# williamleif/GraphSAGE

Hardware: NVIDIA B200
Metric: seed_nodes_per_sec (higher is better)
Workload: dtype f32

## Files before the change

### graphsage_b200/_lib.py

```python
import ctypes
import os

import torch

_HERE = os.path.dirname(os.path.abspath(__file__))
LIB_PATH = os.path.join(_HERE, "csrc", "libgraphsage_b200.so")

ABI_VERSION = 2
GS_F32, GS_BF16 = 0, 1
ACT_NONE, ACT_RELU = 0, 1
COMBINE_ADD, COMBINE_CONCAT = 0, 1
MATH_FP32_SIMT, MATH_TF32X3, MATH_TF32, MATH_BF16 = 0, 1, 2, 3
MAX_SEGMENTS = 4

c_i32, c_i64, c_u64, c_vp = ctypes.c_int32, ctypes.c_int64, ctypes.c_uint64, ctypes.c_void_p


class Segment(ctypes.Structure):
    _fields_ = [("self_ids", c_vp), ("neigh_ids", c_vp), ("self_row0", c_i64), ("neigh_row0", c_i64),
                ("n", c_i64), ("k", c_i32), ("_pad", c_i32), ("out_row0", c_i64)]


MAX_SHARDS = 16


class ShardedTable(ctypes.Structure):
    _fields_ = [("base", c_vp * MAX_SHARDS), ("row_start", c_i64 * (MAX_SHARDS + 1)), ("n_shards", c_i32),
                ("my_shard", c_i32), ("n_global_rows", c_i64), ("zero_row", c_i64), ("remap", c_vp)]


class GemmPart(ctypes.Structure):
    _fields_ = [("A", c_vp), ("lda", c_i64), ("K", c_i32), ("B", c_vp), ("ldb", c_i64), ("N", c_i32)]


_SIGNATURES = {
    "gs_version": (c_i32, []),
    "gs_last_error_string": (ctypes.c_char_p, []),
    "gs_set_tuning": (c_i32, [ctypes.c_char_p, c_i32]),
    "gs_sample_padded": (c_i32, [c_vp, c_i64, c_i32, c_vp, c_i64, c_i32, c_vp, c_u64, c_u64, c_vp, c_vp, c_vp]),
    "gs_sample_padded_khop": (c_i32, [c_vp, c_i64, c_i32, c_vp, c_i64, ctypes.POINTER(c_i32), c_i32, c_u64, c_u64, c_vp,
                                      ctypes.POINTER(c_vp), c_vp]),
    "gs_build_padded_adj": (c_i32, [c_vp, c_vp, c_i64, c_i32, c_vp, c_u64, c_u64, c_vp, c_vp, c_vp]),
    "gs_sample_unigram": (c_i32, [c_vp, c_i64, c_i32, c_u64, c_u64, c_vp, c_vp, c_vp]),
    "gs_sample_csr": (c_i32, [c_vp, c_vp, c_i64, c_vp, c_i64, c_i32, c_i32, c_u64, c_u64, c_vp, c_i32, c_vp, c_vp]),
    "gs_perm_prefix_host": (c_i32, [c_u64, c_u64, c_i32, c_i32, ctypes.POINTER(c_i32)]),
    "gs_gather_rows": (c_i32, [c_vp, c_i32, c_i64, c_i32, c_i64, c_vp, c_i64, c_vp, c_i64, c_vp]),
    "gs_gather_mean": (c_i32, [c_vp, c_i32, c_i64, c_i32, c_i64, ctypes.POINTER(Segment), c_i32, c_i32, c_vp, c_vp,
                               c_i64, c_vp]),
    "gs_gather_mean_sharded": (c_i32, [ctypes.POINTER(ShardedTable), c_i32, c_i32, c_i64, ctypes.POINTER(Segment), c_i32,
                                       c_i32, c_i32, c_vp, c_vp, c_vp, c_i64, c_vp]),
    "gs_halo_begin": (c_i32, [c_vp, c_i64, c_vp, c_vp]),
    "gs_halo_claim": (c_i32, [ctypes.POINTER(ShardedTable), c_vp, c_i64, c_vp, c_vp, c_vp, c_i64, c_vp]),
    "gs_halo_fetch": (c_i32, [ctypes.POINTER(ShardedTable), c_i32, c_i64, c_vp, c_vp, c_i64, c_vp, c_i64, c_vp]),
    "gs_halo_translate": (c_i32, [ctypes.POINTER(ShardedTable), c_vp, c_i64, c_vp, c_vp, c_vp]),
    "gs_translate_ids": (c_i32, [ctypes.POINTER(ShardedTable), c_vp, c_i64, c_vp, c_vp]),
    "gs_gather_rows_sharded": (c_i32, [ctypes.POINTER(ShardedTable), c_i32, c_i32, c_i64, c_vp, c_i64, c_vp, c_i64, c_vp]),
    "gs_shard_alloc": (c_i32, [c_i64, ctypes.POINTER(c_vp)]),
    "gs_shard_free": (c_i32, [c_vp]),
    "gs_ipc_export": (c_i32, [c_vp, ctypes.c_char_p]),
    "gs_ipc_import": (c_i32, [ctypes.c_char_p, ctypes.POINTER(c_vp)]),
    "gs_ipc_close": (c_i32, [c_vp]),
    "gs_gather_rows_f32": (c_i32, [c_vp, c_i32, c_i64, c_i32, c_i64, c_vp, c_i64, c_i64, c_vp, c_i64, c_vp]),
    "gs_cast_rows_bf16": (c_i32, [c_vp, c_i64, c_i32, c_i64, c_vp, c_i64, c_vp]),
    "gs_rmat_degrees": (c_i32, [c_i32, c_i64, ctypes.c_double, ctypes.c_double, ctypes.c_double, ctypes.c_double,
                                ctypes.c_double, c_u64, c_u64, c_u64, c_u64, c_vp, c_vp]),
    "gs_rmat_fill": (c_i32, [c_i32, c_i64, ctypes.c_double, ctypes.c_double, ctypes.c_double, ctypes.c_double, c_u64, c_u64,
                             c_u64, c_u64, c_vp, c_vp, c_vp, c_i64, c_i64, c_vp]),
    "gs_segment_max": (c_i32, [c_vp, c_i64, c_i32, c_i32, c_i64, c_vp, c_i64, c_vp]),
    "gs_sage_gemm_workspace_bytes": (c_i64, [c_i64, ctypes.POINTER(GemmPart), c_i32, c_i32]),
    "gs_sage_gemm": (c_i32, [c_i64, ctypes.POINTER(GemmPart), c_i32, c_i32, c_vp, c_i32, c_i32, c_vp, c_i64, c_vp,
                             c_vp]),
    "gs_sage_gemm_pack": (c_i32, [ctypes.POINTER(GemmPart), c_i32, c_i32, c_vp, c_vp]),
    "gs_sage_gemm_prepacked": (c_i32, [c_i64, ctypes.POINTER(GemmPart), c_i32, c_i32, c_vp, c_i32, c_i32, c_vp, c_i64,
                                       c_vp, c_vp]),
    "gs_gather_mean_img_bytes": (c_i64, [c_i64, c_i32, c_i32]),
    "gs_gather_mean_img": (c_i32, [c_vp, c_i64, ctypes.POINTER(ShardedTable), c_i32, c_vp, c_i32, c_i64, ctypes.POINTER(Segment),
                                   c_i32, c_i32, c_i32, c_vp, c_vp]),
    "gs_sage_gemm_img": (c_i32, [c_i64, ctypes.POINTER(GemmPart), c_i32, c_i32, c_vp, c_i32, c_vp, c_i64, c_vp, c_vp, c_i32,
                                 c_vp]),
    "gs_sage_layer_small": (c_i32, [c_vp, c_i64, c_i32, c_i64, ctypes.POINTER(Segment), c_i32, ctypes.POINTER(GemmPart),
                                    c_i32, c_i32, c_vp, c_i32, c_i32, c_vp, c_i64, c_vp, c_u64, c_vp]),
    "gs_maxpool_mlp_workspace_bytes": (c_i64, [c_i32, c_i32]),
    "gs_maxpool_mlp_pack": (c_i32, [c_vp, c_i64, c_i32, c_i32, c_vp, c_vp]),
    "gs_maxpool_mlp_fused": (c_i32, [c_vp, c_i64, c_i32, c_i64, c_vp, c_i64, c_i64, c_i32, c_vp, c_vp, c_i32, c_vp, c_i64,
                                     c_vp]),
    "gs_meanpool_mlp_fused": (c_i32, [c_vp, c_i64, c_i32, c_i64, c_vp, c_i64, c_i64, c_i32, c_vp, c_vp, c_i32, c_vp, c_i64,
                                      c_vp]),
    "gs_pipeline_step": (c_i32, [c_vp, c_vp, c_i64, ctypes.POINTER(c_vp), c_i32, c_vp, c_vp, c_i64, c_vp, c_vp, c_vp, c_vp,
                                 c_vp, c_vp]),
    "gs_row_used": (c_i32, [c_vp, c_i32, c_i64, c_i32, c_i64, c_vp, c_vp]),
    "gs_lstm_seq": (c_i32, [c_vp, c_i64, c_vp, c_i32, c_vp, c_vp, c_i64, c_i64, c_i32, c_vp, c_i64, c_vp, c_vp, c_vp, c_vp]),
    "gs_l2_normalize_rows": (c_i32, [c_vp, c_i64, c_i32, c_i64, c_vp]),
    "gs_bump_counter": (c_i32, [c_vp, c_u64, c_vp]),
}

_lib = None


def lib():
    global _lib
    if _lib is None:
        if not os.path.exists(LIB_PATH):
            raise ImportError(
                "graphsage_b200: %s is missing - build it with `python -m graphsage_b200.build` "
                "(there is no CPU fallback)" % LIB_PATH)
        _lib = ctypes.CDLL(LIB_PATH)
        for name, (res, args) in _SIGNATURES.items():
            fn = getattr(_lib, name)
            fn.restype, fn.argtypes = res, args
        if _lib.gs_version() != ABI_VERSION:
            raise ImportError("graphsage_b200: %s has ABI version %d, this binding needs %d - rebuild it"
                              % (LIB_PATH, _lib.gs_version(), ABI_VERSION))
        for kv in os.environ.get("GS_TUNING", "").split(","):
            if "=" in kv:
                k, v = kv.split("=", 1)
                _lib.gs_set_tuning(k.strip().encode(), int(v))
    return _lib


def exported_symbols():
    return sorted(_SIGNATURES)


def check(rc):
    if rc != 0:
        msg = lib().gs_last_error_string().decode("utf-8", "replace")
        raise RuntimeError("libgraphsage_b200 error %d: %s" % (rc, msg))


def stream_ptr():
    return torch.cuda.current_stream().cuda_stream


def ptr(t):
    return 0 if t is None else t.data_ptr()


def require_cuda(*tensors):
    for t in tensors:
        if t is not None and not t.is_cuda:
            raise RuntimeError("graphsage_b200: tensor on %s - the hot path is CUDA-only (no CPU fallback)" % t.device)


def set_tuning(key, value):
    return lib().gs_set_tuning(key.encode(), int(value))


def perm_prefix_host(seed, counter, max_deg, k):
    buf = (c_i32 * max(k, 1))()
    check(lib().gs_perm_prefix_host(seed & (2**64 - 1), counter & (2**64 - 1), max_deg, k, buf))
    return list(buf[:k])
```

### graphsage_b200/csrc/api.cu

```cuda
#include <stdarg.h>

#include <map>
#include <set>
#include <utility>
#include <mutex>
#include <string>

#include "common.cuh"

namespace gs {

static thread_local char g_err[512] = "";

void set_error(const char* fmt, ...) {
  va_list ap;
  va_start(ap, fmt);
  vsnprintf(g_err, sizeof(g_err), fmt, ap);
  va_end(ap);
}

int32_t cuda_fail(cudaError_t e, const char* what) {
  set_error("CUDA error %d (%s) at %s", (int)e, cudaGetErrorString(e), what);
  return GS_ERR_CUDA;
}

static std::mutex g_mu;
static std::map<std::string, int32_t>& knobs() {
  static std::map<std::string, int32_t> m;
  return m;
}

int32_t tuning(const char* key, int32_t dflt) {
  std::lock_guard<std::mutex> l(g_mu);
  auto it = knobs().find(key);
  return it == knobs().end() ? dflt : it->second;
}

int sm_count() {
  static int n[64] = {0};
  int dev = 0;
  if (cudaGetDevice(&dev) != cudaSuccess || dev < 0 || dev >= 64) return 148;
  if (n[dev] == 0) {
    int v = 0;
    if (cudaDeviceGetAttribute(&v, cudaDevAttrMultiProcessorCount, dev) != cudaSuccess || v <= 0) v = 148;
    n[dev] = v;
  }
  return n[dev];
}

int32_t ensure_dyn_smem(const void* kernel, int bytes) {
  static std::mutex mu;
  static std::set<std::pair<int, const void*>> done;
  int dev = 0;
  GS_CUDA(cudaGetDevice(&dev));
  std::lock_guard<std::mutex> l(mu);
  if (done.count(std::make_pair(dev, kernel))) return GS_OK;
  GS_CUDA(cudaFuncSetAttribute(kernel, cudaFuncAttributeMaxDynamicSharedMemorySize, bytes));
  done.insert(std::make_pair(dev, kernel));
  return GS_OK;
}

}

extern "C" {

int32_t gs_version(void) { return GS_ABI_VERSION; }

const char* gs_last_error_string(void) { return gs::g_err; }

int32_t gs_set_tuning(const char* key, int32_t value) {
  if (!key) return 0;
  std::lock_guard<std::mutex> l(gs::g_mu);
  int32_t prev = 0;
  auto it = gs::knobs().find(key);
  if (it != gs::knobs().end()) prev = it->second;
  gs::knobs()[key] = value;
  return prev;
}

int32_t gs_perm_prefix_host(uint64_t seed, uint64_t counter, int32_t max_deg, int32_t k, int32_t* out_host) {
  GS_REQUIRE(out_host != nullptr || k == 0, "gs_perm_prefix_host: out_host is NULL");
  GS_REQUIRE(max_deg > 0 && k >= 0 && k <= max_deg, "gs_perm_prefix_host: need 0 <= k <= max_deg (k=%d, max_deg=%d)", k,
             max_deg);
  std::string buf((size_t)max_deg * sizeof(int32_t), '\0');
  int32_t* p = (int32_t*)&buf[0];
  for (int i = 0; i < max_deg; ++i) p[i] = i;
  for (int i = 0; i < k; ++i) {
    uint32_t r = gs::philox_draw(seed, counter, 0u, gs::kStreamPadded, i);
    int j = i + (int)gs::mulhi32(r, (uint32_t)(max_deg - i));
    int32_t t = p[i];
    p[i] = p[j];
    p[j] = t;
  }
  for (int i = 0; i < k; ++i) out_host[i] = p[i];
  return GS_OK;
}

int32_t gs_pipeline_step(const void* ids_host, void* ids_dev, int64_t ids_bytes, void* const* graph_execs_host,
                         int32_t n_graphs, const void* out_dev, void* out_host, int64_t out_bytes, void* h2d_stream,
                         void* compute_stream, void* copy_stream, void* ev_ids, void* ev_done, void* ev_drained) {
  GS_REQUIRE(ids_host && ids_dev && graph_execs_host && out_dev && out_host && ev_ids && ev_done && ev_drained &&
                 n_graphs >= 1,
             "gs_pipeline_step: NULL argument");
  cudaStream_t hs = (cudaStream_t)h2d_stream, cs = (cudaStream_t)compute_stream, ps = (cudaStream_t)copy_stream;
  GS_CUDA(cudaStreamWaitEvent(hs, (cudaEvent_t)ev_done, 0));
  GS_CUDA(cudaMemcpyAsync(ids_dev, ids_host, (size_t)ids_bytes, cudaMemcpyHostToDevice, hs));
  GS_CUDA(cudaEventRecord((cudaEvent_t)ev_ids, hs));
  GS_CUDA(cudaStreamWaitEvent(cs, (cudaEvent_t)ev_ids, 0));
  GS_CUDA(cudaStreamWaitEvent(cs, (cudaEvent_t)ev_drained, 0));
  for (int i = 0; i < n_graphs; ++i) GS_CUDA(cudaGraphLaunch((cudaGraphExec_t)graph_execs_host[i], cs));
  GS_CUDA(cudaEventRecord((cudaEvent_t)ev_done, cs));
  GS_CUDA(cudaStreamWaitEvent(ps, (cudaEvent_t)ev_done, 0));
  GS_CUDA(cudaMemcpyAsync(out_host, out_dev, (size_t)out_bytes, cudaMemcpyDeviceToHost, ps));
  GS_CUDA(cudaEventRecord((cudaEvent_t)ev_drained, ps));
  return GS_OK;
}

}
```

### graphsage_b200/csrc/common.cuh

```cuda
#pragma once
#include <cuda_runtime.h>
#include <stdint.h>
#include <stdio.h>
#include <string.h>

#include "../../include/graphsage_b200.h"

namespace gs {

void set_error(const char* fmt, ...);
int32_t cuda_fail(cudaError_t e, const char* what);
int32_t tuning(const char* key, int32_t dflt);
int32_t ensure_dyn_smem(const void* kernel, int bytes);

#define GS_REQUIRE(cond, ...)            \
  do {                                   \
    if (!(cond)) {                       \
      gs::set_error(__VA_ARGS__);        \
      return GS_ERR_INVALID_ARG;         \
    }                                    \
  } while (0)

#define GS_CUDA(expr)                                        \
  do {                                                       \
    cudaError_t _e = (expr);                                 \
    if (_e != cudaSuccess) return gs::cuda_fail(_e, #expr);  \
  } while (0)

inline int32_t launch_check(const char* what) {
  cudaError_t e = cudaGetLastError();
  if (e != cudaSuccess) return cuda_fail(e, what);
  return GS_OK;
}

int sm_count();

struct u32x4 { uint32_t x, y, z, w; };

__host__ __device__ inline uint32_t mulhi32(uint32_t a, uint32_t b) {
  return (uint32_t)(((uint64_t)a * (uint64_t)b) >> 32);
}

__host__ __device__ inline u32x4 philox4x32_10(u32x4 c, uint32_t k0, uint32_t k1) {
#pragma unroll
  for (int r = 0; r < 10; ++r) {
    uint64_t p0 = (uint64_t)0xD2511F53u * c.x;
    uint64_t p1 = (uint64_t)0xCD9E8D57u * c.z;
    u32x4 n;
    n.x = (uint32_t)(p1 >> 32) ^ c.y ^ k0;
    n.y = (uint32_t)p1;
    n.z = (uint32_t)(p0 >> 32) ^ c.w ^ k1;
    n.w = (uint32_t)p0;
    c = n;
    k0 += 0x9E3779B9u;
    k1 += 0xBB67AE85u;
  }
  return c;
}

__host__ __device__ inline uint32_t pick(const u32x4& v, int i) {
  return i == 0 ? v.x : i == 1 ? v.y : i == 2 ? v.z : v.w;
}

__host__ __device__ inline uint32_t philox_draw(uint64_t seed, uint64_t counter, uint32_t c2, uint32_t tag, int i) {
  u32x4 c{(uint32_t)counter, (uint32_t)(counter >> 32), c2, tag + (uint32_t)(i >> 2)};
  u32x4 r = philox4x32_10(c, (uint32_t)seed, (uint32_t)(seed >> 32));
  return pick(r, i & 3);
}

constexpr uint32_t kStreamPadded = 0u;
constexpr uint32_t kStreamCsr = 0x40000000u;
constexpr uint32_t kStreamUnigram = 0x20000000u;
constexpr uint32_t kStreamBuild = 0x10000000u;

#ifdef __CUDACC__
__device__ __forceinline__ uint32_t smem_u32(const void* p) { return (uint32_t)__cvta_generic_to_shared(p); }

__device__ __forceinline__ void mbar_init(uint64_t* bar, uint32_t count) {
  asm volatile("mbarrier.init.shared::cta.b64 [%0], %1;" ::"r"(smem_u32(bar)), "r"(count));
}
__device__ __forceinline__ void fence_mbar_init() { asm volatile("fence.mbarrier_init.release.cluster;" ::: "memory"); }
__device__ __forceinline__ void fence_proxy_async() { asm volatile("fence.proxy.async.shared::cta;" ::: "memory"); }

__device__ __forceinline__ void mbar_expect_tx(uint64_t* bar, uint32_t bytes) {
  asm volatile("mbarrier.arrive.expect_tx.shared::cta.b64 _, [%0], %1;" ::"r"(smem_u32(bar)), "r"(bytes) : "memory");
}
__device__ __forceinline__ void mbar_arrive(uint64_t* bar) {
  asm volatile("mbarrier.arrive.shared::cta.b64 _, [%0];" ::"r"(smem_u32(bar)) : "memory");
}
__device__ __forceinline__ bool mbar_try_wait(uint64_t* bar, uint32_t parity) {
  uint32_t ok;
  asm volatile(
      "{\n\t.reg .pred p;\n\t"
      "mbarrier.try_wait.parity.shared::cta.b64 p, [%1], %2;\n\t"
      "selp.b32 %0, 1, 0, p;\n\t}"
      : "=r"(ok)
      : "r"(smem_u32(bar)), "r"(parity)
      : "memory");
  return ok != 0;
}
__device__ __forceinline__ void mbar_wait(uint64_t* bar, uint32_t parity) {
  while (!mbar_try_wait(bar, parity)) {
  }
}

__device__ __forceinline__ void bulk_g2s(void* smem_dst, const void* gsrc, uint32_t bytes, uint64_t* bar) {
  asm volatile("cp.async.bulk.shared::cluster.global.mbarrier::complete_tx::bytes [%0], [%1], %2, [%3];" ::"r"(
                   smem_u32(smem_dst)),
               "l"(gsrc), "r"(bytes), "r"(smem_u32(bar))
               : "memory");
}
__device__ __forceinline__ void bulk_s2g(void* gdst, const void* smem_src, uint32_t bytes) {
  asm volatile("cp.async.bulk.global.shared::cta.bulk_group [%0], [%1], %2;" ::"l"(gdst), "r"(smem_u32(smem_src)),
               "r"(bytes)
               : "memory");
}
__device__ __forceinline__ void bulk_commit() { asm volatile("cp.async.bulk.commit_group;" ::: "memory"); }
template <int N>
__device__ __forceinline__ void bulk_wait_read() {
  asm volatile("cp.async.bulk.wait_group.read %0;" ::"n"(N) : "memory");
}
template <int N>
__device__ __forceinline__ void bulk_wait() {
  asm volatile("cp.async.bulk.wait_group %0;" ::"n"(N) : "memory");
}

__device__ __forceinline__ float4 ldg_nc_f4(const float4* p) {
  float4 r;
  asm volatile("ld.global.nc.L1::no_allocate.v4.f32 {%0,%1,%2,%3}, [%4];"
               : "=f"(r.x), "=f"(r.y), "=f"(r.z), "=f"(r.w)
               : "l"(p));
  return r;
}
#endif

}
```

### graphsage_b200/csrc/gather.cu

```cuda
#include "common.cuh"

namespace gs {

struct SegTable {
  gs_segment s[GS_MAX_SEGMENTS];
  int32_t n_segments;
  int64_t total_rows;
};

__device__ __forceinline__ int find_segment(const SegTable& t, int64_t r, int64_t& local) {
  int si = 0;
  int64_t base = 0;
#pragma unroll
  for (int q = 0; q < GS_MAX_SEGMENTS - 1; ++q) {
    if (q < t.n_segments - 1 && r >= base + t.s[q].n) {
      base += t.s[q].n;
      si = q + 1;
    }
  }
  local = r - base;
  return si;
}

__device__ __forceinline__ int64_t clamp_row(int64_t id, int64_t n_rows) {
  return (id < 0 || id >= n_rows) ? n_rows - 1 : id;
}

__device__ __forceinline__ float4 mask_tail(float4 v, int col0, int F) {
  if (col0 + 1 >= F) v.y = 0.f;
  if (col0 + 2 >= F) v.z = 0.f;
  if (col0 + 3 >= F) v.w = 0.f;
  return v;
}

template <int kUnroll>
__global__ void __launch_bounds__(256) gather_mean_ldg_kernel(const float* __restrict__ src, int64_t n_src_rows, int F,
                                                              int64_t pitch, const __grid_constant__ SegTable tab, int include_self,
                                                              float* __restrict__ out_self,
                                                              float* __restrict__ out_mean, int64_t out_pitch) {
  const int ncol4 = (int)(out_pitch >> 2);
  for (int64_t r = blockIdx.x; r < tab.total_rows; r += gridDim.x) {
    int64_t i;
    const gs_segment& sg = tab.s[find_segment(tab, r, i)];
    const int k = sg.k;
    const int64_t orow = sg.out_row0 + i;
    const int64_t srow = clamp_row(sg.self_ids ? (int64_t)sg.self_ids[i] : sg.self_row0 + i, n_src_rows);
    for (int c = threadIdx.x; c < ncol4; c += blockDim.x) {
      const int col0 = c * 4;
      float4 acc = make_float4(0.f, 0.f, 0.f, 0.f);
      float4 sv = acc;
      if (col0 < F) {
        int j = 0;
        for (; j + kUnroll <= k; j += kUnroll) {
          float4 v[kUnroll];
#pragma unroll
          for (int u = 0; u < kUnroll; ++u) {
            int64_t nr = clamp_row(sg.neigh_ids ? (int64_t)sg.neigh_ids[i * k + j + u] : sg.neigh_row0 + i * k + j + u,
                                   n_src_rows);
            v[u] = ldg_nc_f4(reinterpret_cast<const float4*>(src + nr * pitch) + c);
          }
#pragma unroll
          for (int u = 0; u < kUnroll; ++u) {
            acc.x += v[u].x; acc.y += v[u].y; acc.z += v[u].z; acc.w += v[u].w;
          }
        }
        for (; j < k; ++j) {
          int64_t nr = clamp_row(sg.neigh_ids ? (int64_t)sg.neigh_ids[i * k + j] : sg.neigh_row0 + i * k + j, n_src_rows);
          float4 v = ldg_nc_f4(reinterpret_cast<const float4*>(src + nr * pitch) + c);
          acc.x += v.x; acc.y += v.y; acc.z += v.z; acc.w += v.w;
        }
        if (include_self || out_self) sv = ldg_nc_f4(reinterpret_cast<const float4*>(src + srow * pitch) + c);
        float div = (float)(k + (include_self ? 1 : 0));
        if (include_self) { acc.x += sv.x; acc.y += sv.y; acc.z += sv.z; acc.w += sv.w; }
        acc.x /= div; acc.y /= div; acc.z /= div; acc.w /= div;
        acc = mask_tail(acc, col0, F);
        sv = mask_tail(sv, col0, F);
      }
      reinterpret_cast<float4*>(out_mean + orow * out_pitch)[c] = acc;
      if (out_self) reinterpret_cast<float4*>(out_self + orow * out_pitch)[c] = sv;
    }
  }
}

__global__ void __launch_bounds__(256) gather_mean_scalar_kernel(const float* __restrict__ src, int64_t n_src_rows, int F,
                                                                 int64_t pitch, const __grid_constant__ SegTable tab, int include_self,
                                                                 float* __restrict__ out_self,
                                                                 float* __restrict__ out_mean, int64_t out_pitch) {
  for (int64_t r = blockIdx.x; r < tab.total_rows; r += gridDim.x) {
    int64_t i;
    const gs_segment& sg = tab.s[find_segment(tab, r, i)];
    const int k = sg.k;
    const int64_t orow = sg.out_row0 + i;
    const int64_t srow = clamp_row(sg.self_ids ? (int64_t)sg.self_ids[i] : sg.self_row0 + i, n_src_rows);
    for (int c = threadIdx.x; c < (int)out_pitch; c += blockDim.x) {
      float acc = 0.f, sv = 0.f;
      if (c < F) {
        for (int j = 0; j < k; ++j) {
          int64_t nr = clamp_row(sg.neigh_ids ? (int64_t)sg.neigh_ids[i * k + j] : sg.neigh_row0 + i * k + j, n_src_rows);
          acc += src[nr * pitch + c];
        }
        sv = src[srow * pitch + c];
        if (include_self) acc += sv;
        acc /= (float)(k + (include_self ? 1 : 0));
      }
      out_mean[orow * out_pitch + c] = acc;
      if (out_self) out_self[orow * out_pitch + c] = sv;
    }
  }
}

__global__ void __launch_bounds__(192) gather_mean_tma_kernel(const float* __restrict__ src, int64_t n_src_rows, int F,
                                                              int64_t pitch, const __grid_constant__ SegTable tab, int include_self,
                                                              float* __restrict__ out_self,
                                                              float* __restrict__ out_mean, int64_t out_pitch,
                                                              int row_bytes) {
  extern __shared__ __align__(128) unsigned char smem[];
  __shared__ __align__(8) uint64_t bar;
  if (threadIdx.x == 0) {
    mbar_init(&bar, 1);
    fence_mbar_init();
  }
  __syncthreads();
  const int ncol4 = (int)(out_pitch >> 2);
  const int row_f4 = row_bytes >> 4;
  uint32_t phase = 0;
  for (int64_t r = blockIdx.x; r < tab.total_rows; r += gridDim.x) {
    int64_t i;
    const gs_segment& sg = tab.s[find_segment(tab, r, i)];
    const int k = sg.k;
    const int64_t orow = sg.out_row0 + i;
    if (threadIdx.x < 32) {
      if (threadIdx.x == 0) mbar_expect_tx(&bar, (uint32_t)((k + 1) * row_bytes));
      __syncwarp();
      for (int j = threadIdx.x; j <= k; j += 32) {
        int64_t id;
        if (j < k) id = sg.neigh_ids ? (int64_t)sg.neigh_ids[i * k + j] : sg.neigh_row0 + i * k + j;
        else id = sg.self_ids ? (int64_t)sg.self_ids[i] : sg.self_row0 + i;
        id = clamp_row(id, n_src_rows);
        bulk_g2s(smem + (size_t)j * row_bytes, src + id * pitch, (uint32_t)row_bytes, &bar);
      }
    }
    mbar_wait(&bar, phase);
    phase ^= 1u;
    const float4* rows = reinterpret_cast<const float4*>(smem);
    for (int c = threadIdx.x; c < ncol4; c += blockDim.x) {
      const int col0 = c * 4;
      float4 acc = make_float4(0.f, 0.f, 0.f, 0.f);
      float4 sv = acc;
      if (col0 < F) {
#pragma unroll 5
        for (int j = 0; j < k; ++j) {
          float4 v = rows[j * row_f4 + c];
          acc.x += v.x; acc.y += v.y; acc.z += v.z; acc.w += v.w;
        }
        sv = rows[k * row_f4 + c];
        float div = (float)(k + (include_self ? 1 : 0));
        if (include_self) { acc.x += sv.x; acc.y += sv.y; acc.z += sv.z; acc.w += sv.w; }
        acc.x /= div; acc.y /= div; acc.z /= div; acc.w /= div;
        acc = mask_tail(acc, col0, F);
        sv = mask_tail(sv, col0, F);
      }
      reinterpret_cast<float4*>(out_mean + orow * out_pitch)[c] = acc;
      if (out_self) reinterpret_cast<float4*>(out_self + orow * out_pitch)[c] = sv;
    }
    __syncthreads();
  }
}

struct DenseRows {
  const float* src;
  int64_t n_rows, pitch;
  __device__ __forceinline__ const float* row(int64_t id) const { return src + clamp_row(id, n_rows) * pitch; }
};

struct ShardTab {
  const float* base[GS_MAX_SHARDS];
  int64_t row_start[GS_MAX_SHARDS + 1];
  int32_t n_shards, my_shard;
  int64_t n_global_rows;
  int64_t zero_row;
  const int32_t* remap;
};

struct ShardRows {
  ShardTab t;
  int64_t pitch;
  int32_t locators;
  const float* staging;
  __device__ __forceinline__ const float* row(int64_t id) const {
    const float* mine = t.base[t.my_shard];
    if (locators) {
      if (id >= 0) return mine + id * pitch;
      if (locators == 2) return staging + (-id - 1) * pitch;
      id = -id - 1;
    } else if (id < 0 || id >= t.n_global_rows - 1) {
      return mine + t.zero_row * pitch;
    } else if (t.remap) {
      const int32_t s = __ldg(t.remap + id);
      if (s >= 0) return mine + (int64_t)s * pitch;
    } else if (id >= t.row_start[t.my_shard] && id < t.row_start[t.my_shard + 1]) {
      return mine + (id - t.row_start[t.my_shard]) * pitch;
    }
    int o = 0;
#pragma unroll
    for (int q = 1; q < GS_MAX_SHARDS; ++q)
      if (q < t.n_shards && id >= t.row_start[q]) o = q;
    return t.base[o] + (id - t.row_start[o]) * pitch;
  }
};

constexpr int kGroupRows = 13;

struct GatherImg {
  unsigned char* base;
  int32_t kblocks, n_mtiles;
  int32_t want_self;
};

__device__ __forceinline__ void gather_img_store(const GatherImg& im, int part, int64_t orow, int c, float4 v) {
  const int kb = c >> 3, chunk = c & 7;
  const int64_t mt = orow >> 7;
  const int r = (int)(orow & 127);
  unsigned char* dst = im.base + ((((int64_t)part * im.n_mtiles + mt) * im.kblocks + kb) * 2) * 16384 +
                       (uint32_t)(r * 128 + ((chunk ^ (r & 7)) << 4));
  uint4 hi, lo;
  hi.x = __float_as_uint(v.x) & 0xFFFFE000u; hi.y = __float_as_uint(v.y) & 0xFFFFE000u;
  hi.z = __float_as_uint(v.z) & 0xFFFFE000u; hi.w = __float_as_uint(v.w) & 0xFFFFE000u;
  lo.x = __float_as_uint(v.x - __uint_as_float(hi.x)) & 0xFFFFE000u; lo.y = __float_as_uint(v.y - __uint_as_float(hi.y)) & 0xFFFFE000u;
  lo.z = __float_as_uint(v.z - __uint_as_float(hi.z)) & 0xFFFFE000u; lo.w = __float_as_uint(v.w - __uint_as_float(hi.w)) & 0xFFFFE000u;
  *reinterpret_cast<uint4*>(dst) = hi;
  *reinterpret_cast<uint4*>(dst + 16384) = lo;
}

template <class Rows>
__global__ void __launch_bounds__(192) gather_mean_tma2_kernel(const __grid_constant__ Rows rows_of, int F,
                                                               const __grid_constant__ SegTable tab,
                                                               int include_self, float* __restrict__ out_self,
                                                               float* __restrict__ out_mean, int64_t out_pitch,
                                                               int row_bytes, const __grid_constant__ GatherImg img) {
  extern __shared__ __align__(128) unsigned char smem[];
  __shared__ __align__(8) uint64_t bar[2];
  if (threadIdx.x == 0) {
    mbar_init(&bar[0], 1);
    mbar_init(&bar[1], 1);
    fence_mbar_init();
  }
  __syncthreads();
  const int ncol4 = (int)(out_pitch >> 2);
  const int row_f4 = row_bytes >> 4;
  const size_t buf_bytes = (size_t)kGroupRows * row_bytes;

  int64_t r_issue = blockIdx.x;
  int g_issue = 0;
  auto issue = [&](int buf) -> bool {
    if (r_issue >= tab.total_rows) return false;
    int64_t i;
    const gs_segment& sg = tab.s[find_segment(tab, r_issue, i)];
    const int k = sg.k;
    const int rows_total = k + 1;
    const int first = g_issue * kGroupRows;
    const int cnt = min(kGroupRows, rows_total - first);
    if (threadIdx.x < 32) {
      if (threadIdx.x == 0) mbar_expect_tx(&bar[buf], (uint32_t)(cnt * row_bytes));
      __syncwarp();
      for (int j = threadIdx.x; j < cnt; j += 32) {
        const int jj = first + j;
        int64_t id;
        if (jj < k) id = sg.neigh_ids ? (int64_t)sg.neigh_ids[i * k + jj] : sg.neigh_row0 + i * k + jj;
        else id = sg.self_ids ? (int64_t)sg.self_ids[i] : sg.self_row0 + i;
        bulk_g2s(smem + buf * buf_bytes + (size_t)j * row_bytes, rows_of.row(id), (uint32_t)row_bytes, &bar[buf]);
      }
    }
    if (first + cnt >= rows_total) { r_issue += gridDim.x; g_issue = 0; } else { ++g_issue; }
    return true;
  };

  uint32_t phase[2] = {0u, 0u};
  int buf = 0;
  bool have = issue(0);
  int64_t r = blockIdx.x;
  int g = 0;
  float4 acc[2];
  acc[0] = acc[1] = make_float4(0.f, 0.f, 0.f, 0.f);
  while (have) {
    const bool have_next = issue(buf ^ 1);
    int64_t i;
    const gs_segment& sg = tab.s[find_segment(tab, r, i)];
    const int k = sg.k;
    const int rows_total = k + 1;
    const int first = g * kGroupRows;
    const int cnt = min(kGroupRows, rows_total - first);
    const bool last = first + cnt >= rows_total;
    mbar_wait(&bar[buf], phase[buf]);
    phase[buf] ^= 1u;
    const float4* rows = reinterpret_cast<const float4*>(smem + buf * buf_bytes);
    const int nn = last ? cnt - 1 : cnt;
#pragma unroll
    for (int q = 0; q < 2; ++q) {
      const int c = threadIdx.x + q * blockDim.x;
      if (c < ncol4 && c * 4 < F) {
        float4 a = acc[q];
        for (int j = 0; j < nn; ++j) {
          float4 v = rows[j * row_f4 + c];
          a.x += v.x; a.y += v.y; a.z += v.z; a.w += v.w;
        }
        acc[q] = a;
      }
    }
    if (last) {
      const int64_t orow = sg.out_row0 + i;
      const int ncol_img = img.base ? img.kblocks * 8 : 0;
#pragma unroll
      for (int q = 0; q < 2; ++q) {
        const int c = threadIdx.x + q * blockDim.x;
        if (c < ncol4 || c < ncol_img) {
          float4 a = make_float4(0.f, 0.f, 0.f, 0.f), sv = a;
          if (c < ncol4 && c * 4 < F) {
            a = acc[q];
            sv = rows[(cnt - 1) * row_f4 + c];
            const float div = (float)(k + (include_self ? 1 : 0));
            if (include_self) { a.x += sv.x; a.y += sv.y; a.z += sv.z; a.w += sv.w; }
            a.x /= div; a.y /= div; a.z /= div; a.w /= div;
            a = mask_tail(a, c * 4, F);
            sv = mask_tail(sv, c * 4, F);
          }
          if (c < ncol4) {
            if (out_mean) reinterpret_cast<float4*>(out_mean + orow * out_pitch)[c] = a;
            if (out_self) reinterpret_cast<float4*>(out_self + orow * out_pitch)[c] = sv;
          }
          if (c < ncol_img) {
            if (img.want_self) gather_img_store(img, 0, orow, c, sv);
            gather_img_store(img, img.want_self ? 1 : 0, orow, c, a);
          }
          if (c < ncol4) acc[q] = make_float4(0.f, 0.f, 0.f, 0.f);
        }
      }
      r += gridDim.x;
      g = 0;
    } else {
      ++g;
    }
    __syncthreads();
    buf ^= 1;
    have = have_next;
  }
}

__global__ void __launch_bounds__(192) gather_mean_bf16_tma2_kernel(const uint16_t* __restrict__ src, int64_t n_src_rows, int F,
                                                                    int64_t pitch, const __grid_constant__ SegTable tab,
                                                                    int include_self, float* __restrict__ out_self,
                                                                    float* __restrict__ out_mean, int64_t out_pitch,
                                                                    int row_bytes) {
  extern __shared__ __align__(128) unsigned char smem[];
  __shared__ __align__(8) uint64_t bar[2];
  if (threadIdx.x == 0) {
    mbar_init(&bar[0], 1);
    mbar_init(&bar[1], 1);
    fence_mbar_init();
  }
  __syncthreads();
  const int ncol8 = (int)(out_pitch >> 3);
  const int row_u4 = row_bytes >> 4;
  const size_t buf_bytes = (size_t)kGroupRows * row_bytes;
  int64_t r_issue = blockIdx.x;
  int g_issue = 0;
  auto issue = [&](int buf) -> bool {
    if (r_issue >= tab.total_rows) return false;
    int64_t i;
    const gs_segment& sg = tab.s[find_segment(tab, r_issue, i)];
    const int k = sg.k;
    const int rows_total = k + 1;
    const int first = g_issue * kGroupRows;
    const int cnt = min(kGroupRows, rows_total - first);
    if (threadIdx.x < 32) {
      if (threadIdx.x == 0) mbar_expect_tx(&bar[buf], (uint32_t)(cnt * row_bytes));
      __syncwarp();
      for (int j = threadIdx.x; j < cnt; j += 32) {
        const int jj = first + j;
        int64_t id;
        if (jj < k) id = sg.neigh_ids ? (int64_t)sg.neigh_ids[i * k + jj] : sg.neigh_row0 + i * k + jj;
        else id = sg.self_ids ? (int64_t)sg.self_ids[i] : sg.self_row0 + i;
        id = clamp_row(id, n_src_rows);
        bulk_g2s(smem + buf * buf_bytes + (size_t)j * row_bytes, src + id * pitch, (uint32_t)row_bytes, &bar[buf]);
      }
    }
    if (first + cnt >= rows_total) { r_issue += gridDim.x; g_issue = 0; } else { ++g_issue; }
    return true;
  };
  auto widen = [](uint4 u, float (&v)[8]) {
    const uint32_t w[4] = {u.x, u.y, u.z, u.w};
#pragma unroll
    for (int e = 0; e < 4; ++e) {
      v[2 * e] = __uint_as_float(w[e] << 16);
      v[2 * e + 1] = __uint_as_float(w[e] & 0xffff0000u);
    }
  };
  uint32_t phase[2] = {0u, 0u};
  int buf = 0;
  bool have = issue(0);
  int64_t r = blockIdx.x;
  int g = 0;
  float acc[8];
#pragma unroll
  for (int e = 0; e < 8; ++e) acc[e] = 0.f;
  const int c = threadIdx.x;
  while (have) {
    const bool have_next = issue(buf ^ 1);
    int64_t i;
    const gs_segment& sg = tab.s[find_segment(tab, r, i)];
    const int k = sg.k;
    const int rows_total = k + 1;
    const int first = g * kGroupRows;
    const int cnt = min(kGroupRows, rows_total - first);
    const bool last = first + cnt >= rows_total;
    mbar_wait(&bar[buf], phase[buf]);
    phase[buf] ^= 1u;
    const uint4* rows = reinterpret_cast<const uint4*>(smem + buf * buf_bytes);
    const int nn = last ? cnt - 1 : cnt;
    if (c < ncol8 && c * 8 < F) {
      for (int j = 0; j < nn; ++j) {
        float v[8];
        widen(rows[j * row_u4 + c], v);
#pragma unroll
        for (int e = 0; e < 8; ++e) acc[e] += v[e];
      }
    }
    if (last) {
      const int64_t orow = sg.out_row0 + i;
      if (c < ncol8) {
        float a[8], sv[8];
#pragma unroll
        for (int e = 0; e < 8; ++e) { a[e] = 0.f; sv[e] = 0.f; }
        if (c * 8 < F) {
          widen(rows[(cnt - 1) * row_u4 + c], sv);
          const float div = (float)(k + (include_self ? 1 : 0));
#pragma unroll
          for (int e = 0; e < 8; ++e) {
            float t = acc[e];
            if (include_self) t += sv[e];
            a[e] = (c * 8 + e < F) ? t / div : 0.f;
            if (c * 8 + e >= F) sv[e] = 0.f;
          }
        }
        float4* om = reinterpret_cast<float4*>(out_mean + orow * out_pitch) + 2 * c;
        om[0] = make_float4(a[0], a[1], a[2], a[3]);
        om[1] = make_float4(a[4], a[5], a[6], a[7]);
        if (out_self) {
          float4* os = reinterpret_cast<float4*>(out_self + orow * out_pitch) + 2 * c;
          os[0] = make_float4(sv[0], sv[1], sv[2], sv[3]);
          os[1] = make_float4(sv[4], sv[5], sv[6], sv[7]);
        }
#pragma unroll
        for (int e = 0; e < 8; ++e) acc[e] = 0.f;
      }
      r += gridDim.x;
      g = 0;
    } else {
      ++g;
    }
    __syncthreads();
    buf ^= 1;
    have = have_next;
  }
}

__global__ void __launch_bounds__(32) gather_rows_tma_kernel(const unsigned char* __restrict__ src, int64_t n_rows,
                                                             int64_t pitch_bytes, const int32_t* __restrict__ ids,
                                                             int64_t n, unsigned char* __restrict__ out,
                                                             int64_t out_pitch_bytes, int row_bytes) {
  extern __shared__ __align__(128) unsigned char smem[];
  __shared__ __align__(8) uint64_t bar;
  const int lane = threadIdx.x;
  if (lane == 0) {
    mbar_init(&bar, 1);
    fence_mbar_init();
  }
  __syncwarp();
  uint32_t phase = 0;
  for (int64_t base = (int64_t)blockIdx.x * 32; base < n; base += (int64_t)gridDim.x * 32) {
    int cnt = (int)((n - base) < 32 ? (n - base) : 32);
    if (lane == 0) mbar_expect_tx(&bar, (uint32_t)(cnt * row_bytes));
    __syncwarp();
    if (lane < cnt) {
      int64_t id = clamp_row(ids[base + lane], n_rows);
      bulk_g2s(smem + (size_t)lane * row_bytes, src + id * pitch_bytes, (uint32_t)row_bytes, &bar);
    }
    mbar_wait(&bar, phase);
    phase ^= 1u;
    if (lane < cnt) bulk_s2g(out + (base + lane) * out_pitch_bytes, smem + (size_t)lane * row_bytes, (uint32_t)row_bytes);
    bulk_commit();
    bulk_wait_read<0>();
    __syncwarp();
  }
  bulk_wait<0>();
}

template <typename T>
__global__ void __launch_bounds__(256) gather_rows_simple_kernel(const T* __restrict__ src, int64_t n_rows, int F,
                                                                 int64_t pitch, const int32_t* __restrict__ ids,
                                                                 int64_t n, T* __restrict__ out, int64_t out_pitch) {
  const int lane = threadIdx.x & 31;
  const int64_t warp = ((int64_t)blockIdx.x * blockDim.x + threadIdx.x) >> 5;
  const int64_t nwarps = ((int64_t)gridDim.x * blockDim.x) >> 5;
  for (int64_t i = warp; i < n; i += nwarps) {
    int64_t id = clamp_row(ids[i], n_rows);
    for (int c = lane; c < F; c += 32) out[i * out_pitch + c] = src[id * pitch + c];
  }
}

template <typename T>
__global__ void __launch_bounds__(256) gather_rows_to_f32_kernel(const T* __restrict__ src, int64_t n_rows, int F,
                                                                 int64_t pitch, const int32_t* __restrict__ ids, int64_t row0,
                                                                 int64_t n, float* __restrict__ out, int64_t out_pitch) {
  const int lane = threadIdx.x & 31;
  const int64_t warp = ((int64_t)blockIdx.x * blockDim.x + threadIdx.x) >> 5;
  const int64_t nwarps = ((int64_t)gridDim.x * blockDim.x) >> 5;
  for (int64_t i = warp; i < n; i += nwarps) {
    const int64_t id = clamp_row(ids ? (int64_t)ids[i] : row0 + i, n_rows);
    for (int c = lane; c < (int)out_pitch; c += 32) {
      float v = 0.f;
      if (c < F) {
        if constexpr (sizeof(T) == 2) v = __uint_as_float(((uint32_t)src[id * pitch + c]) << 16);
        else v = src[id * pitch + c];
      }
      out[i * out_pitch + c] = v;
    }
  }
}

__global__ void __launch_bounds__(256) gather_rows_bf16_to_f32_vec_kernel(const uint16_t* __restrict__ src, int64_t n_rows, int F,
                                                                          int64_t pitch, const int32_t* __restrict__ ids,
                                                                          int64_t row0, int64_t n, float* __restrict__ out,
                                                                          int64_t out_pitch) {
  const int lane = threadIdx.x & 31;
  const int64_t warp = ((int64_t)blockIdx.x * blockDim.x + threadIdx.x) >> 5;
  const int64_t nwarps = ((int64_t)gridDim.x * blockDim.x) >> 5;
  const int chunks = (int)(out_pitch >> 3);
  for (int64_t i = warp; i < n; i += nwarps) {
    const int64_t id = clamp_row(ids ? (int64_t)ids[i] : row0 + i, n_rows);
    const uint4* rp = reinterpret_cast<const uint4*>(src + id * pitch);
    float4* op = reinterpret_cast<float4*>(out + i * out_pitch);
    for (int c = lane; c < chunks; c += 32) {
      uint4 u = make_uint4(0u, 0u, 0u, 0u);
      if (c * 8 < F) u = __ldg(rp + c);
      const uint32_t w[4] = {u.x, u.y, u.z, u.w};
      float v[8];
#pragma unroll
      for (int e = 0; e < 4; ++e) {
        v[2 * e] = (c * 8 + 2 * e < F) ? __uint_as_float(w[e] << 16) : 0.f;
        v[2 * e + 1] = (c * 8 + 2 * e + 1 < F) ? __uint_as_float(w[e] & 0xffff0000u) : 0.f;
      }
      op[2 * c] = make_float4(v[0], v[1], v[2], v[3]);
      op[2 * c + 1] = make_float4(v[4], v[5], v[6], v[7]);
    }
  }
}

__device__ __forceinline__ uint32_t f32_to_bf16_rne(float x) {
  const uint32_t u = __float_as_uint(x);
  if ((u & 0x7fffffffu) > 0x7f800000u) return (u >> 16) | 0x40u;
  return (u + 0x7fffu + ((u >> 16) & 1u)) >> 16;
}

__global__ void __launch_bounds__(256) cast_rows_bf16_kernel(const float* __restrict__ x, int64_t n, int F, int64_t ldx,
                                                             uint16_t* __restrict__ out, int64_t out_pitch) {
  const int chunks = (int)(out_pitch >> 3);
  const int64_t total = n * chunks;
  for (int64_t q = (int64_t)blockIdx.x * blockDim.x + threadIdx.x; q < total; q += (int64_t)gridDim.x * blockDim.x) {
    const int64_t i = q / chunks;
    const int c = (int)(q - i * chunks) * 8;
    const float* xp = x + i * ldx + c;
    uint32_t h[8];
#pragma unroll
    for (int e = 0; e < 8; ++e) h[e] = (c + e < F) ? f32_to_bf16_rne(xp[e]) : 0u;
    uint4 o;
    o.x = h[0] | (h[1] << 16); o.y = h[2] | (h[3] << 16); o.z = h[4] | (h[5] << 16); o.w = h[6] | (h[7] << 16);
    *reinterpret_cast<uint4*>(out + i * out_pitch + c) = o;
  }
}

__global__ void __launch_bounds__(256) cast_rows_bf16_scalar_kernel(const float* __restrict__ x, int64_t n, int F, int64_t ldx,
                                                                    uint16_t* __restrict__ out, int64_t out_pitch) {
  const int64_t total = n * out_pitch;
  for (int64_t q = (int64_t)blockIdx.x * blockDim.x + threadIdx.x; q < total; q += (int64_t)gridDim.x * blockDim.x) {
    const int64_t i = q / out_pitch;
    const int c = (int)(q - i * out_pitch);
    out[q] = c < F ? (uint16_t)f32_to_bf16_rne(x[i * ldx + c]) : (uint16_t)0;
  }
}

__global__ void bump_counter_kernel(unsigned long long* counter, unsigned long long inc) { *counter += inc; }

__global__ void __launch_bounds__(256) segment_max_kernel(const float* __restrict__ x, int64_t n, int k, int C,
                                                          int64_t ldx, float* __restrict__ out, int64_t ldo) {
  for (int64_t i = blockIdx.x; i < n; i += gridDim.x) {
    for (int c = threadIdx.x; c < C; c += blockDim.x) {
      float m = x[(i * k) * ldx + c];
      for (int j = 1; j < k; ++j) m = fmaxf(m, x[(i * k + j) * ldx + c]);
      out[i * ldo + c] = m;
    }
  }
}

__global__ void __launch_bounds__(256) l2_normalize_kernel(float* __restrict__ x, int64_t n, int C, int64_t ldx) {
  const int lane = threadIdx.x & 31;
  const int64_t warp = ((int64_t)blockIdx.x * blockDim.x + threadIdx.x) >> 5;
  const int64_t nwarps = ((int64_t)gridDim.x * blockDim.x) >> 5;
  for (int64_t i = warp; i < n; i += nwarps) {
    float ss = 0.f;
    for (int c = lane; c < C; c += 32) {
      float v = x[i * ldx + c];
      ss += v * v;
    }
#pragma unroll
    for (int o = 16; o > 0; o >>= 1) ss += __shfl_xor_sync(0xffffffffu, ss, o);
    float inv = 1.0f / sqrtf(fmaxf(ss, 1e-12f));
    for (int c = lane; c < C; c += 32) x[i * ldx + c] *= inv;
  }
}

__global__ void __launch_bounds__(256) translate_ids_kernel(const int32_t* __restrict__ remap, int64_t n_global_rows,
                                                            int32_t zero_row, const int32_t* __restrict__ ids, int64_t n,
                                                            int32_t* __restrict__ out) {
  for (int64_t i = (int64_t)blockIdx.x * blockDim.x + threadIdx.x; i < n; i += (int64_t)gridDim.x * blockDim.x) {
    const int32_t id = ids[i];
    int32_t loc;
    if (id < 0 || id >= n_global_rows - 1) loc = zero_row;
    else {
      loc = __ldg(remap + id);
      if (loc < 0) loc = -id - 1;
    }
    out[i] = loc;
  }
}

__device__ __forceinline__ bool halo_is_local(const ShardTab& t, int32_t id, int32_t& loc) {
  if (id < 0 || id >= t.n_global_rows - 1) { loc = (int32_t)t.zero_row; return true; }
  if (t.remap) {
    loc = __ldg(t.remap + id);
    return loc >= 0;
  }
  if (id >= t.row_start[t.my_shard] && id < t.row_start[t.my_shard + 1]) { loc = (int32_t)(id - t.row_start[t.my_shard]); return true; }
  return false;
}

__global__ void __launch_bounds__(256) halo_claim_kernel(const __grid_constant__ ShardTab t, const int32_t* __restrict__ ids,
                                                         int64_t n, int32_t* __restrict__ claim, int32_t* __restrict__ count,
                                                         int32_t* __restrict__ stage_ids, int64_t capacity) {
  for (int64_t i = (int64_t)blockIdx.x * blockDim.x + threadIdx.x; i < n; i += (int64_t)gridDim.x * blockDim.x) {
    const int32_t id = ids[i];
    int32_t loc;
    if (halo_is_local(t, id, loc)) continue;
    if (atomicCAS(claim + id, -1, -2) == -1) {
      const int32_t idx = atomicAdd(count, 1);
      if (idx < capacity) stage_ids[idx] = id;
      claim[id] = idx;
    }
  }
}

__global__ void __launch_bounds__(256) halo_translate_kernel(const __grid_constant__ ShardTab t, const int32_t* __restrict__ ids,
                                                             int64_t n, const int32_t* __restrict__ claim,
                                                             int32_t* __restrict__ out) {
  for (int64_t i = (int64_t)blockIdx.x * blockDim.x + threadIdx.x; i < n; i += (int64_t)gridDim.x * blockDim.x) {
    const int32_t id = ids[i];
    int32_t loc;
    if (!halo_is_local(t, id, loc)) loc = -claim[id] - 1;
    out[i] = loc;
  }
}

constexpr int kHaloLoads = 5;
__global__ void __launch_bounds__(256) halo_fetch_kernel(const __grid_constant__ ShardRows sr, int row_f4,
                                                         const int32_t* __restrict__ stage_ids, const int32_t* __restrict__ count,
                                                         int64_t capacity, float* __restrict__ staging, int64_t staging_pitch) {
  const int lane = threadIdx.x & 31;
  const int64_t warp = ((int64_t)blockIdx.x * blockDim.x + threadIdx.x) >> 5;
  const int64_t nwarps = ((int64_t)gridDim.x * blockDim.x) >> 5;
  int64_t n = *count;
  if (n > capacity) n = capacity;
  for (int64_t i = warp; i < n; i += nwarps) {
    const float4* src = reinterpret_cast<const float4*>(sr.row(stage_ids[i]));
    float4* dst = reinterpret_cast<float4*>(staging + i * staging_pitch);
    for (int c0 = lane; c0 < row_f4; c0 += 32 * kHaloLoads) {
      float4 v[kHaloLoads];
#pragma unroll
      for (int u = 0; u < kHaloLoads; ++u)
        if (c0 + 32 * u < row_f4) v[u] = ldg_nc_f4(src + c0 + 32 * u);
#pragma unroll
      for (int u = 0; u < kHaloLoads; ++u)
        if (c0 + 32 * u < row_f4) dst[c0 + 32 * u] = v[u];
    }
  }
}

template <int kUnroll>
__global__ void __launch_bounds__(256) gather_mean_sharded_kernel(const __grid_constant__ ShardRows st, int F,
                                                                  const __grid_constant__ SegTable tab, int include_self,
                                                                  float* __restrict__ out_self,
                                                                  float* __restrict__ out_mean, int64_t out_pitch) {
  const int ncol4 = (int)(out_pitch >> 2);
  for (int64_t r = blockIdx.x; r < tab.total_rows; r += gridDim.x) {
    int64_t i;
    const gs_segment& sg = tab.s[find_segment(tab, r, i)];
    const int k = sg.k;
    const int64_t orow = sg.out_row0 + i;
    const float* srow = st.row(sg.self_ids ? (int64_t)sg.self_ids[i] : sg.self_row0 + i);
    for (int c = threadIdx.x; c < ncol4; c += blockDim.x) {
      const int col0 = c * 4;
      float4 acc = make_float4(0.f, 0.f, 0.f, 0.f);
      float4 sv = acc;
      if (col0 < F) {
        int j = 0;
        for (; j + kUnroll <= k; j += kUnroll) {
          float4 v[kUnroll];
#pragma unroll
          for (int u = 0; u < kUnroll; ++u) {
            const float* p = st.row(sg.neigh_ids ? (int64_t)sg.neigh_ids[i * k + j + u] : sg.neigh_row0 + i * k + j + u);
            v[u] = ldg_nc_f4(reinterpret_cast<const float4*>(p) + c);
          }
#pragma unroll
          for (int u = 0; u < kUnroll; ++u) {
            acc.x += v[u].x; acc.y += v[u].y; acc.z += v[u].z; acc.w += v[u].w;
          }
        }
        for (; j < k; ++j) {
          const float* p = st.row(sg.neigh_ids ? (int64_t)sg.neigh_ids[i * k + j] : sg.neigh_row0 + i * k + j);
          float4 v = ldg_nc_f4(reinterpret_cast<const float4*>(p) + c);
          acc.x += v.x; acc.y += v.y; acc.z += v.z; acc.w += v.w;
        }
        if (include_self || out_self) sv = ldg_nc_f4(reinterpret_cast<const float4*>(srow) + c);
        float div = (float)(k + (include_self ? 1 : 0));
        if (include_self) { acc.x += sv.x; acc.y += sv.y; acc.z += sv.z; acc.w += sv.w; }
        acc.x /= div; acc.y /= div; acc.z /= div; acc.w /= div;
        acc = mask_tail(acc, col0, F);
        sv = mask_tail(sv, col0, F);
      }
      reinterpret_cast<float4*>(out_mean + orow * out_pitch)[c] = acc;
      if (out_self) reinterpret_cast<float4*>(out_self + orow * out_pitch)[c] = sv;
    }
  }
}

__global__ void __launch_bounds__(256) gather_rows_sharded_kernel(const __grid_constant__ ShardRows st, int F,
                                                                  const int32_t* __restrict__ ids, int64_t n,
                                                                  float* __restrict__ out, int64_t out_pitch) {
  const int lane = threadIdx.x & 31;
  const int64_t warp = ((int64_t)blockIdx.x * blockDim.x + threadIdx.x) >> 5;
  const int64_t nwarps = ((int64_t)gridDim.x * blockDim.x) >> 5;
  const int ncol4 = (int)(out_pitch >> 2);
  for (int64_t i = warp; i < n; i += nwarps) {
    const float* p = st.row(ids[i]);
    for (int c = lane; c < ncol4; c += 32) {
      float4 v = make_float4(0.f, 0.f, 0.f, 0.f);
      if (c * 4 < F) v = mask_tail(ldg_nc_f4(reinterpret_cast<const float4*>(p) + c), c * 4, F);
      reinterpret_cast<float4*>(out + i * out_pitch)[c] = v;
    }
  }
}

static inline bool aligned16(const void* p) { return (reinterpret_cast<uintptr_t>(p) & 15u) == 0; }

}


namespace gs {
template <class Rows>
static int32_t launch_gather_tma2(const Rows& rows_of, int F, const SegTable& tab, int include_self, float* out_self, float* out_mean,
                                  int64_t out_pitch, const GatherImg& img, cudaStream_t st) {
  const int32_t rc_attr = ensure_dyn_smem((const void*)gather_mean_tma2_kernel<Rows>, 200 * 1024);
  if (rc_attr != GS_OK) return rc_attr;
  const int ncol4 = (int)(out_pitch / 4);
  const int row_bytes = ((F + 3) / 4) * 16;
  const size_t smem2 = (size_t)2 * kGroupRows * row_bytes;
  int threads = ((ncol4 + 31) / 32) * 32;
  if (threads > 160) threads = 160;
  if (threads < 32) threads = 32;
  int per_sm = (int)((224 * 1024) / (smem2 + 1024));
  if (per_sm < 1) per_sm = 1;
  int lim = tuning("gather_ctas_per_sm", 8);
  if (per_sm > lim) per_sm = lim;
  int64_t blocks = tab.total_rows;
  int64_t cap = (int64_t)sm_count() * per_sm;
  if (blocks > cap) blocks = cap;
  gather_mean_tma2_kernel<Rows><<<(unsigned)blocks, threads, smem2, st>>>(rows_of, F, tab, include_self, out_self, out_mean,
                                                                          out_pitch, row_bytes, img);
  return launch_check("gather_mean_tma2_kernel");
}
}

extern "C" {

int32_t gs_gather_rows(const void* feats, int32_t dtype, int64_t n_rows, int32_t F, int64_t pitch, const int32_t* ids,
                       int64_t n, void* out, int64_t out_pitch, void* stream) {
  GS_REQUIRE(n >= 0 && F >= 0, "gs_gather_rows: negative size");
  if (n == 0 || F == 0) return GS_OK;
  GS_REQUIRE(feats && ids && out, "gs_gather_rows: NULL pointer");
  GS_REQUIRE(dtype == GS_F32 || dtype == GS_BF16, "gs_gather_rows: dtype %d", dtype);
  GS_REQUIRE(n_rows > 0 && pitch >= F && out_pitch >= F, "gs_gather_rows: pitch < F");
  const int es = dtype == GS_F32 ? 4 : 2;
  cudaStream_t st = (cudaStream_t)stream;
  const int row_bytes = ((F * es + 15) / 16) * 16;
  const bool tma_ok = gs::aligned16(feats) && gs::aligned16(out) && (pitch * es) % 16 == 0 && (out_pitch * es) % 16 == 0 &&
                      row_bytes <= pitch * es && row_bytes <= out_pitch * es && row_bytes * 32 <= 200 * 1024;
  if (tma_ok && gs::tuning("gather_variant", 2) != 0) {
    size_t smem = (size_t)row_bytes * 32;
    {
      const int32_t rc_attr = gs::ensure_dyn_smem((const void*)gs::gather_rows_tma_kernel, 200 * 1024);
      if (rc_attr != GS_OK) return rc_attr;
    }
    int per_sm = (int)((220 * 1024) / (smem + 1024));
    if (per_sm < 1) per_sm = 1;
    if (per_sm > 16) per_sm = 16;
    int64_t blocks = (n + 31) / 32;
    int64_t cap = (int64_t)gs::sm_count() * per_sm;
    if (blocks > cap) blocks = cap;
    gs::gather_rows_tma_kernel<<<(unsigned)blocks, 32, smem, st>>>((const unsigned char*)feats, n_rows, pitch * es, ids, n,
                                                                   (unsigned char*)out, out_pitch * es, row_bytes);
    return gs::launch_check("gather_rows_tma_kernel");
  }
  int64_t blocks = (n + 7) / 8;
  int64_t cap = (int64_t)gs::sm_count() * 8;
  if (blocks > cap) blocks = cap;
  if (dtype == GS_F32)
    gs::gather_rows_simple_kernel<float><<<(unsigned)blocks, 256, 0, st>>>((const float*)feats, n_rows, F, pitch, ids, n,
                                                                           (float*)out, out_pitch);
  else
    gs::gather_rows_simple_kernel<uint16_t><<<(unsigned)blocks, 256, 0, st>>>((const uint16_t*)feats, n_rows, F, pitch, ids,
                                                                              n, (uint16_t*)out, out_pitch);
  return gs::launch_check("gather_rows_simple_kernel");
}

int32_t gs_gather_mean(const void* src, int32_t dtype, int64_t n_src_rows, int32_t F, int64_t pitch,
                       const gs_segment* segments_host, int32_t n_segments, int32_t include_self, void* out_self,
                       void* out_mean, int64_t out_pitch, void* stream) {
  GS_REQUIRE(dtype == GS_F32 || dtype == GS_BF16, "gs_gather_mean: dtype %d (GS_F32 or GS_BF16)", dtype);
  GS_REQUIRE(n_segments >= 0 && n_segments <= GS_MAX_SEGMENTS, "gs_gather_mean: n_segments=%d (max %d)", n_segments,
             GS_MAX_SEGMENTS);
  GS_REQUIRE(segments_host || n_segments == 0, "gs_gather_mean: segments_host is NULL");
  gs::SegTable tab;
  memset(&tab, 0, sizeof(tab));
  tab.n_segments = n_segments;
  int kmax = 0;
  for (int s = 0; s < n_segments; ++s) {
    tab.s[s] = segments_host[s];
    GS_REQUIRE(tab.s[s].n >= 0 && tab.s[s].k >= 1, "gs_gather_mean: segment %d has n=%lld k=%d", s, (long long)tab.s[s].n,
               tab.s[s].k);
    tab.total_rows += tab.s[s].n;
    if (tab.s[s].k > kmax) kmax = tab.s[s].k;
  }
  if (tab.total_rows == 0) return GS_OK;
  GS_REQUIRE(src && out_mean, "gs_gather_mean: NULL pointer");
  GS_REQUIRE(F > 0 && pitch >= F && out_pitch >= F && n_src_rows > 0, "gs_gather_mean: bad F/pitch");
  cudaStream_t st = (cudaStream_t)stream;
  if (dtype == GS_BF16) {
    const int64_t f8 = ((int64_t)F + 7) / 8 * 8;
    if (!(gs::aligned16(src) && gs::aligned16(out_mean) && (!out_self || gs::aligned16(out_self)) && pitch % 8 == 0 &&
          out_pitch % 8 == 0 && f8 <= pitch && f8 <= out_pitch && f8 / 8 <= 192)) {
      gs::set_error("gs_gather_mean(GS_BF16): needs 16-byte aligned rows (pitch %% 8 == 0), out_pitch %% 8 == 0 and F <= 1536");
      return GS_ERR_UNSUPPORTED;
    }
    const int32_t rc_attr = gs::ensure_dyn_smem((const void*)gs::gather_mean_bf16_tma2_kernel, 200 * 1024);
    if (rc_attr != GS_OK) return rc_attr;
    const int row_bytes = (int)(f8 * 2);
    const size_t smem2 = (size_t)2 * gs::kGroupRows * row_bytes;
    const int ncol8 = (int)(out_pitch / 8);
    int threads = ((ncol8 + 31) / 32) * 32;
    if (threads < 32) threads = 32;
    GS_REQUIRE(threads <= 192, "gs_gather_mean(GS_BF16): out_pitch too wide");
    int per_sm = (int)((224 * 1024) / (smem2 + 1024));
    if (per_sm < 1) per_sm = 1;
    int lim = gs::tuning("gather_ctas_per_sm", 8);
    if (per_sm > lim) per_sm = lim;
    int64_t blocks = tab.total_rows;
    int64_t cap = (int64_t)gs::sm_count() * per_sm;
    if (blocks > cap) blocks = cap;
    gs::gather_mean_bf16_tma2_kernel<<<(unsigned)blocks, threads, smem2, st>>>((const uint16_t*)src, n_src_rows, F, pitch, tab,
                                                                              include_self, (float*)out_self, (float*)out_mean,
                                                                              out_pitch, row_bytes);
    return gs::launch_check("gather_mean_bf16_tma2_kernel");
  }
  const float* fsrc = (const float*)src;
  const bool vec_ok = gs::aligned16(src) && gs::aligned16(out_mean) && (!out_self || gs::aligned16(out_self)) &&
                      pitch % 4 == 0 && out_pitch % 4 == 0 && ((F + 3) / 4) * 4 <= pitch;
  if (!vec_ok) {
    int64_t blocks = tab.total_rows;
    int64_t cap = (int64_t)gs::sm_count() * 8;
    if (blocks > cap) blocks = cap;
    gs::gather_mean_scalar_kernel<<<(unsigned)blocks, 256, 0, st>>>(fsrc, n_src_rows, F, pitch, tab, include_self,
                                                                    (float*)out_self, (float*)out_mean, out_pitch);
    return gs::launch_check("gather_mean_scalar_kernel");
  }
  const int ncol4 = (int)(out_pitch / 4);
  const int row_bytes = ((F + 3) / 4) * 16;
  const size_t smem = (size_t)row_bytes * (kmax + 1);
  const int variant = gs::tuning("gather_variant", 2);
  if (variant == 2 && ncol4 <= 2 * 160) {
    const gs::DenseRows rows_of{fsrc, n_src_rows, pitch};
    gs::GatherImg img;
    memset(&img, 0, sizeof(img));
    return gs::launch_gather_tma2(rows_of, F, tab, include_self, (float*)out_self, (float*)out_mean, out_pitch, img, st);
  }
  if (variant >= 1 && smem <= 200 * 1024) {
    {
      const int32_t rc_attr = gs::ensure_dyn_smem((const void*)gs::gather_mean_tma_kernel, 200 * 1024);
      if (rc_attr != GS_OK) return rc_attr;
    }
    int threads = ((ncol4 + 31) / 32) * 32;
    if (threads > 192) threads = 192;
    if (threads < 32) threads = 32;
    int per_sm = (int)((224 * 1024) / (smem + 1024));
    if (per_sm < 1) per_sm = 1;
    int lim = gs::tuning("gather_ctas_per_sm", 8);
    if (per_sm > lim) per_sm = lim;
    int64_t blocks = tab.total_rows;
    int64_t cap = (int64_t)gs::sm_count() * per_sm;
    if (blocks > cap) blocks = cap;
    gs::gather_mean_tma_kernel<<<(unsigned)blocks, threads, smem, st>>>(fsrc, n_src_rows, F, pitch, tab, include_self,
                                                                        (float*)out_self, (float*)out_mean, out_pitch,
                                                                        row_bytes);
    return gs::launch_check("gather_mean_tma_kernel");
  }
  int threads = ((ncol4 + 31) / 32) * 32;
  if (threads > 256) threads = 256;
  int64_t blocks = tab.total_rows;
  int64_t cap = (int64_t)gs::sm_count() * gs::tuning("gather_ctas_per_sm", 8);
  if (blocks > cap) blocks = cap;
  gs::gather_mean_ldg_kernel<5><<<(unsigned)blocks, threads, 0, st>>>(fsrc, n_src_rows, F, pitch, tab, include_self,
                                                                      (float*)out_self, (float*)out_mean, out_pitch);
  return gs::launch_check("gather_mean_ldg_kernel");
}

int32_t gs_gather_rows_f32(const void* feats, int32_t dtype, int64_t n_rows, int32_t F, int64_t pitch, const int32_t* ids,
                           int64_t row0, int64_t n, float* out, int64_t out_pitch, void* stream) {
  GS_REQUIRE(n >= 0 && F >= 0, "gs_gather_rows_f32: negative size");
  if (n == 0 || out_pitch == 0) return GS_OK;
  GS_REQUIRE(feats && out, "gs_gather_rows_f32: NULL pointer");
  GS_REQUIRE(dtype == GS_F32 || dtype == GS_BF16, "gs_gather_rows_f32: dtype %d", dtype);
  GS_REQUIRE(n_rows > 0 && pitch >= F && out_pitch >= F, "gs_gather_rows_f32: pitch < F");
  int64_t blocks = (n + 7) / 8;
  int64_t cap = (int64_t)gs::sm_count() * 8;
  if (blocks > cap) blocks = cap;
  if (dtype == GS_F32)
    gs::gather_rows_to_f32_kernel<float><<<(unsigned)blocks, 256, 0, (cudaStream_t)stream>>>(
        (const float*)feats, n_rows, F, pitch, ids, row0, n, out, out_pitch);
  else if (pitch % 8 == 0 && out_pitch % 8 == 0 && gs::aligned16(feats) && gs::aligned16(out) && out_pitch <= pitch)
    gs::gather_rows_bf16_to_f32_vec_kernel<<<(unsigned)blocks, 256, 0, (cudaStream_t)stream>>>(
        (const uint16_t*)feats, n_rows, F, pitch, ids, row0, n, out, out_pitch);
  else
    gs::gather_rows_to_f32_kernel<uint16_t><<<(unsigned)blocks, 256, 0, (cudaStream_t)stream>>>(
        (const uint16_t*)feats, n_rows, F, pitch, ids, row0, n, out, out_pitch);
  return gs::launch_check("gather_rows_to_f32_kernel");
}

int32_t gs_cast_rows_bf16(const float* x, int64_t n, int32_t F, int64_t ldx, void* out_bf16, int64_t out_pitch,
                          void* stream) {
  GS_REQUIRE(n >= 0 && F >= 0 && ldx >= F && out_pitch >= F, "gs_cast_rows_bf16: bad sizes");
  if (n == 0 || out_pitch == 0) return GS_OK;
  GS_REQUIRE(x && out_bf16, "gs_cast_rows_bf16: NULL pointer");
  const bool vec = out_pitch % 8 == 0 && gs::aligned16(out_bf16) && ldx >= ((F + 7) / 8) * 8;
  int64_t blocks = ((vec ? n * (out_pitch / 8) : n * out_pitch) + 255) / 256;
  int64_t cap = (int64_t)gs::sm_count() * 8;
  if (blocks > cap) blocks = cap;
  if (vec)
    gs::cast_rows_bf16_kernel<<<(unsigned)blocks, 256, 0, (cudaStream_t)stream>>>(x, n, F, ldx, (uint16_t*)out_bf16, out_pitch);
  else
    gs::cast_rows_bf16_scalar_kernel<<<(unsigned)blocks, 256, 0, (cudaStream_t)stream>>>(x, n, F, ldx, (uint16_t*)out_bf16,
                                                                                         out_pitch);
  return gs::launch_check("cast_rows_bf16_kernel");
}

int32_t gs_bump_counter(uint64_t* counter_dev, uint64_t inc, void* stream) {
  GS_REQUIRE(counter_dev != nullptr, "gs_bump_counter: NULL counter");
  gs::bump_counter_kernel<<<1, 1, 0, (cudaStream_t)stream>>>((unsigned long long*)counter_dev, (unsigned long long)inc);
  return gs::launch_check("bump_counter_kernel");
}

int32_t gs_segment_max(const float* x, int64_t n, int32_t k, int32_t C, int64_t ldx, float* out, int64_t ldo,
                       void* stream) {
  GS_REQUIRE(n >= 0 && k >= 1 && C >= 0, "gs_segment_max: bad sizes");
  if (n == 0 || C == 0) return GS_OK;
  GS_REQUIRE(x && out, "gs_segment_max: NULL pointer");
  int64_t blocks = n;
  int64_t cap = (int64_t)gs::sm_count() * 8;
  if (blocks > cap) blocks = cap;
  gs::segment_max_kernel<<<(unsigned)blocks, 256, 0, (cudaStream_t)stream>>>(x, n, k, C, ldx, out, ldo);
  return gs::launch_check("segment_max_kernel");
}

int32_t gs_l2_normalize_rows(float* x, int64_t n, int32_t C, int64_t ldx, void* stream) {
  GS_REQUIRE(n >= 0 && C >= 0, "gs_l2_normalize_rows: bad sizes");
  if (n == 0 || C == 0) return GS_OK;
  GS_REQUIRE(x, "gs_l2_normalize_rows: NULL pointer");
  int64_t blocks = (n + 7) / 8;
  int64_t cap = (int64_t)gs::sm_count() * 8;
  if (blocks > cap) blocks = cap;
  gs::l2_normalize_kernel<<<(unsigned)blocks, 256, 0, (cudaStream_t)stream>>>(x, n, C, ldx);
  return gs::launch_check("l2_normalize_kernel");
}

}

static int32_t fill_shard_tab(const gs_sharded_table* t, gs::ShardRows& sr, int64_t pitch, const char* who) {
  GS_REQUIRE(t != nullptr, "%s: table is NULL", who);
  GS_REQUIRE(t->n_shards >= 1 && t->n_shards <= GS_MAX_SHARDS, "%s: n_shards=%d (max %d)", who, t->n_shards, GS_MAX_SHARDS);
  GS_REQUIRE(t->my_shard >= 0 && t->my_shard < t->n_shards, "%s: my_shard=%d", who, t->my_shard);
  GS_REQUIRE(t->n_global_rows > 0 && t->row_start[0] == 0 && t->row_start[t->n_shards] == t->n_global_rows - 1,
             "%s: row_start must run from 0 to n_global_rows - 1", who);
  for (int i = 0; i < t->n_shards; ++i)
    GS_REQUIRE(t->row_start[i] <= t->row_start[i + 1], "%s: row_start must be non-decreasing (shard %d)", who, i);
  GS_REQUIRE(t->zero_row >= 0, "%s: zero_row < 0", who);
  GS_REQUIRE(pitch % 4 == 0, "%s: pitch must be a multiple of 4 floats", who);
  memset(&sr, 0, sizeof(sr));
  gs::ShardTab& st = sr.t;
  for (int i = 0; i < t->n_shards; ++i) {
    GS_REQUIRE(t->base[i] != nullptr && gs::aligned16(t->base[i]), "%s: shard %d pointer NULL or not 16-byte aligned", who, i);
    st.base[i] = (const float*)t->base[i];
  }
  for (int i = 0; i <= t->n_shards; ++i) st.row_start[i] = t->row_start[i];
  for (int i = t->n_shards + 1; i <= GS_MAX_SHARDS; ++i) st.row_start[i] = t->row_start[t->n_shards];
  st.n_shards = t->n_shards;
  st.my_shard = t->my_shard;
  st.n_global_rows = t->n_global_rows;
  st.zero_row = t->zero_row;
  st.remap = t->remap;
  sr.pitch = pitch;
  return GS_OK;
}

extern "C" {

int32_t gs_translate_ids(const gs_sharded_table* table_host, const int32_t* ids, int64_t n, int32_t* out, void* stream) {
  GS_REQUIRE(table_host && table_host->remap, "gs_translate_ids: the table has no remap (no replicas)");
  GS_REQUIRE(n >= 0, "gs_translate_ids: n < 0");
  if (n == 0) return GS_OK;
  GS_REQUIRE(ids && out, "gs_translate_ids: NULL pointer");
  GS_REQUIRE(table_host->zero_row >= 0 && table_host->zero_row < 0x7fffffffLL, "gs_translate_ids: zero_row out of range");
  int64_t blocks = (n + 255) / 256;
  int64_t cap = (int64_t)gs::sm_count() * 8;
  if (blocks > cap) blocks = cap;
  gs::translate_ids_kernel<<<(unsigned)blocks, 256, 0, (cudaStream_t)stream>>>(table_host->remap, table_host->n_global_rows,
                                                                                (int32_t)table_host->zero_row, ids, n, out);
  return gs::launch_check("translate_ids_kernel");
}

int64_t gs_gather_mean_img_bytes(int64_t rows, int32_t F, int32_t want_self) {
  if (rows < 0 || F < 1) return -1;
  const int64_t n_mtiles = (rows + 127) / 128, kblocks = (F + 31) / 32;
  return (want_self ? 2 : 1) * n_mtiles * kblocks * 2 * 16384;
}

int32_t gs_gather_mean_img(const void* src, int64_t n_src_rows, const gs_sharded_table* table_host, int32_t ids_are_locators,
                           const void* staging, int32_t F, int64_t pitch, const gs_segment* segments_host, int32_t n_segments,
                           int32_t include_self, int32_t want_self, void* images, void* stream) {
  GS_REQUIRE((src != nullptr) != (table_host != nullptr), "gs_gather_mean_img: pass either a dense table or a sharded one");
  GS_REQUIRE(n_segments >= 0 && n_segments <= GS_MAX_SEGMENTS && (segments_host || n_segments == 0),
             "gs_gather_mean_img: bad segments");
  gs::SegTable tab;
  memset(&tab, 0, sizeof(tab));
  tab.n_segments = n_segments;
  int64_t rows = 0;
  for (int s = 0; s < n_segments; ++s) {
    tab.s[s] = segments_host[s];
    GS_REQUIRE(tab.s[s].n >= 0 && tab.s[s].k >= 1, "gs_gather_mean_img: segment %d has n=%lld k=%d", s, (long long)tab.s[s].n,
               tab.s[s].k);
    tab.total_rows += tab.s[s].n;
    if (tab.s[s].out_row0 + tab.s[s].n > rows) rows = tab.s[s].out_row0 + tab.s[s].n;
  }
  if (tab.total_rows == 0) return GS_OK;
  GS_REQUIRE(images && (reinterpret_cast<uintptr_t>(images) & 1023u) == 0, "gs_gather_mean_img: images must be 1024-byte aligned");
  const int64_t out_pitch = ((int64_t)F + 7) / 8 * 8;
  const int ncol4 = (int)(out_pitch / 4);
  if (ncol4 > 2 * 160 || F < 1 || pitch % 4 != 0 || pitch < ((F + 3) / 4) * 4 || gs::tuning("gather_variant", 2) != 2) {
    gs::set_error("gs_gather_mean_img: needs F <= 1280, 16-byte row pitch and the bulk-copy gather (F=%d pitch=%lld)", F, (long long)pitch);
    return GS_ERR_UNSUPPORTED;
  }
  gs::GatherImg img;
  img.base = (unsigned char*)images;
  img.kblocks = (F + 31) / 32;
  img.n_mtiles = (int32_t)((rows + 127) / 128);
  img.want_self = want_self ? 1 : 0;
  if (src) {
    GS_REQUIRE(gs::aligned16(src) && n_src_rows > 0, "gs_gather_mean_img: table must be 16-byte aligned");
    const gs::DenseRows rows_of{(const float*)src, n_src_rows, pitch};
    return gs::launch_gather_tma2(rows_of, F, tab, include_self, nullptr, nullptr, out_pitch, img, (cudaStream_t)stream);
  }
  gs::ShardRows sr;
  int32_t rc = fill_shard_tab(table_host, sr, pitch, "gs_gather_mean_img");
  if (rc != GS_OK) return rc;
  GS_REQUIRE(ids_are_locators >= 0 && ids_are_locators <= 2 && (ids_are_locators != 2 || staging != nullptr),
             "gs_gather_mean_img: ids_are_locators = 2 needs the staging buffer");
  sr.locators = ids_are_locators;
  sr.staging = (const float*)staging;
  return gs::launch_gather_tma2(sr, F, tab, include_self, nullptr, nullptr, out_pitch, img, (cudaStream_t)stream);
}

int32_t gs_halo_begin(int32_t* claim, int64_t n_global_rows, int32_t* count, void* stream) {
  GS_REQUIRE(claim && count && n_global_rows > 0, "gs_halo_begin: bad arguments");
  GS_CUDA(cudaMemsetAsync(claim, 0xff, (size_t)n_global_rows * 4, (cudaStream_t)stream));
  GS_CUDA(cudaMemsetAsync(count, 0, 4, (cudaStream_t)stream));
  return GS_OK;
}

int32_t gs_halo_claim(const gs_sharded_table* table_host, const int32_t* ids, int64_t n, int32_t* claim, int32_t* count,
                      int32_t* stage_ids, int64_t capacity, void* stream) {
  gs::ShardRows sr;
  int32_t rc = fill_shard_tab(table_host, sr, 4, "gs_halo_claim");
  if (rc != GS_OK) return rc;
  GS_REQUIRE(n >= 0 && capacity >= 0, "gs_halo_claim: negative size");
  if (n == 0) return GS_OK;
  GS_REQUIRE(ids && claim && count && stage_ids, "gs_halo_claim: NULL pointer");
  int64_t blocks = (n + 255) / 256;
  int64_t cap = (int64_t)gs::sm_count() * 8;
  if (blocks > cap) blocks = cap;
  gs::halo_claim_kernel<<<(unsigned)blocks, 256, 0, (cudaStream_t)stream>>>(sr.t, ids, n, claim, count, stage_ids, capacity);
  return gs::launch_check("halo_claim_kernel");
}

int32_t gs_halo_translate(const gs_sharded_table* table_host, const int32_t* ids, int64_t n, const int32_t* claim, int32_t* out,
                          void* stream) {
  gs::ShardRows sr;
  int32_t rc = fill_shard_tab(table_host, sr, 4, "gs_halo_translate");
  if (rc != GS_OK) return rc;
  GS_REQUIRE(n >= 0, "gs_halo_translate: n < 0");
  if (n == 0) return GS_OK;
  GS_REQUIRE(ids && claim && out, "gs_halo_translate: NULL pointer");
  int64_t blocks = (n + 255) / 256;
  int64_t cap = (int64_t)gs::sm_count() * 8;
  if (blocks > cap) blocks = cap;
  gs::halo_translate_kernel<<<(unsigned)blocks, 256, 0, (cudaStream_t)stream>>>(sr.t, ids, n, claim, out);
  return gs::launch_check("halo_translate_kernel");
}

int32_t gs_halo_fetch(const gs_sharded_table* table_host, int32_t F, int64_t pitch, const int32_t* stage_ids,
                      const int32_t* count, int64_t capacity, float* staging, int64_t staging_pitch, void* stream) {
  gs::ShardRows sr;
  int32_t rc = fill_shard_tab(table_host, sr, pitch, "gs_halo_fetch");
  if (rc != GS_OK) return rc;
  if (capacity == 0) return GS_OK;
  GS_REQUIRE(stage_ids && count && staging && gs::aligned16(staging) && staging_pitch % 4 == 0 && F > 0 &&
                 pitch >= ((F + 3) / 4) * 4 && staging_pitch >= ((F + 3) / 4) * 4,
             "gs_halo_fetch: bad arguments");
  sr.locators = 0;
  sr.staging = nullptr;
  sr.t.remap = nullptr;
  const int blocks = gs::sm_count() * gs::tuning("halo_fetch_ctas_per_sm", 2);
  gs::halo_fetch_kernel<<<(unsigned)blocks, 256, 0, (cudaStream_t)stream>>>(sr, (F + 3) / 4, stage_ids, count, capacity, staging,
                                                                            staging_pitch);
  return gs::launch_check("halo_fetch_kernel");
}

int32_t gs_gather_mean_sharded(const gs_sharded_table* table_host, int32_t dtype, int32_t F, int64_t pitch,
                               const gs_segment* segments_host, int32_t n_segments, int32_t include_self,
                               int32_t ids_are_locators, const void* staging, void* out_self, void* out_mean,
                               int64_t out_pitch, void* stream) {
  GS_REQUIRE(dtype == GS_F32, "gs_gather_mean_sharded: only GS_F32 (dtype=%d)", dtype);
  GS_REQUIRE(n_segments >= 0 && n_segments <= GS_MAX_SEGMENTS && (segments_host || n_segments == 0),
             "gs_gather_mean_sharded: bad segments");
  gs::ShardRows sr;
  int32_t rc = fill_shard_tab(table_host, sr, pitch, "gs_gather_mean_sharded");
  if (rc != GS_OK) return rc;
  GS_REQUIRE(ids_are_locators >= 0 && ids_are_locators <= 2 && (ids_are_locators != 2 || staging != nullptr),
             "gs_gather_mean_sharded: ids_are_locators = 2 needs the staging buffer");
  sr.locators = ids_are_locators;
  sr.staging = (const float*)staging;
  gs::SegTable tab;
  memset(&tab, 0, sizeof(tab));
  tab.n_segments = n_segments;
  for (int s = 0; s < n_segments; ++s) {
    tab.s[s] = segments_host[s];
    GS_REQUIRE(tab.s[s].n >= 0 && tab.s[s].k >= 1, "gs_gather_mean_sharded: segment %d has n=%lld k=%d", s,
               (long long)tab.s[s].n, tab.s[s].k);
    tab.total_rows += tab.s[s].n;
  }
  if (tab.total_rows == 0) return GS_OK;
  GS_REQUIRE(out_mean && gs::aligned16(out_mean) && (!out_self || gs::aligned16(out_self)) && out_pitch % 4 == 0 &&
                 F > 0 && pitch >= ((F + 3) / 4) * 4 && out_pitch >= F,
             "gs_gather_mean_sharded: bad output / pitch");
  const int ncol4 = (int)(out_pitch / 4);
  if (gs::tuning("gather_variant", 2) != 0 && ncol4 <= 2 * 160) {
    gs::GatherImg img;
    memset(&img, 0, sizeof(img));
    return gs::launch_gather_tma2(sr, F, tab, include_self, (float*)out_self, (float*)out_mean, out_pitch, img,
                                  (cudaStream_t)stream);
  }
  int threads = ((ncol4 + 31) / 32) * 32;
  if (threads > 256) threads = 256;
  int64_t blocks = tab.total_rows;
  int64_t cap = (int64_t)gs::sm_count() * gs::tuning("gather_ctas_per_sm", 8);
  if (blocks > cap) blocks = cap;
  gs::gather_mean_sharded_kernel<5><<<(unsigned)blocks, threads, 0, (cudaStream_t)stream>>>(
      sr, F, tab, include_self, (float*)out_self, (float*)out_mean, out_pitch);
  return gs::launch_check("gather_mean_sharded_kernel");
}

int32_t gs_gather_rows_sharded(const gs_sharded_table* table_host, int32_t dtype, int32_t F, int64_t pitch,
                               const int32_t* ids, int64_t n, void* out, int64_t out_pitch, void* stream) {
  GS_REQUIRE(dtype == GS_F32, "gs_gather_rows_sharded: only GS_F32 (dtype=%d)", dtype);
  gs::ShardRows sr;
  int32_t rc = fill_shard_tab(table_host, sr, pitch, "gs_gather_rows_sharded");
  if (rc != GS_OK) return rc;
  if (n == 0) return GS_OK;
  GS_REQUIRE(ids && out && gs::aligned16(out) && out_pitch % 4 == 0 && F > 0 && pitch >= ((F + 3) / 4) * 4 && out_pitch >= F,
             "gs_gather_rows_sharded: bad arguments");
  int64_t blocks = (n + 7) / 8;
  int64_t cap = (int64_t)gs::sm_count() * 8;
  if (blocks > cap) blocks = cap;
  gs::gather_rows_sharded_kernel<<<(unsigned)blocks, 256, 0, (cudaStream_t)stream>>>(sr, F, ids, n, (float*)out, out_pitch);
  return gs::launch_check("gather_rows_sharded_kernel");
}

int32_t gs_shard_alloc(int64_t bytes, void** dev_ptr_out) {
  GS_REQUIRE(bytes > 0 && dev_ptr_out, "gs_shard_alloc: bad arguments");
  GS_CUDA(cudaMalloc(dev_ptr_out, (size_t)bytes));
  return GS_OK;
}

int32_t gs_shard_free(void* dev_ptr) {
  if (dev_ptr) GS_CUDA(cudaFree(dev_ptr));
  return GS_OK;
}

int32_t gs_ipc_export(const void* dev_ptr, uint8_t* handle64_out_host) {
  GS_REQUIRE(dev_ptr && handle64_out_host, "gs_ipc_export: NULL argument");
  static_assert(sizeof(cudaIpcMemHandle_t) == 64, "cudaIpcMemHandle_t is 64 bytes");
  cudaIpcMemHandle_t h;
  GS_CUDA(cudaIpcGetMemHandle(&h, const_cast<void*>(dev_ptr)));
  memcpy(handle64_out_host, &h, 64);
  return GS_OK;
}

int32_t gs_ipc_import(const uint8_t* handle64_host, void** dev_ptr_out) {
  GS_REQUIRE(handle64_host && dev_ptr_out, "gs_ipc_import: NULL argument");
  cudaIpcMemHandle_t h;
  memcpy(&h, handle64_host, 64);
  GS_CUDA(cudaIpcOpenMemHandle(dev_ptr_out, h, cudaIpcMemLazyEnablePeerAccess));
  return GS_OK;
}

int32_t gs_ipc_close(void* dev_ptr) {
  if (dev_ptr) GS_CUDA(cudaIpcCloseMemHandle(dev_ptr));
  return GS_OK;
}

}
```

### graphsage_b200/csrc/gemm_tc.cu

```cuda
#include "tc_common.cuh"

namespace gs {

constexpr int TC_PRODUCER_WARPS = 8;
constexpr int TC_THREADS = (TC_PRODUCER_WARPS + 2) * 32;

struct TcPart {
  const float* A;
  int64_t lda;
  int32_t K;
  int32_t N;
  int32_t kblocks;
  int32_t ntiles;
  int64_t img_off;
  const float* B;
  int64_t ldb;
};

struct TcParams {
  TcPart p[2];
  int32_t n_parts;
  int32_t combine;
  int64_t M;
  const float* bias;
  int32_t act;
  float* out;
  int64_t ldo;
  int32_t tiles_n0;
  int32_t issue_elect;
  const unsigned char* a_img;
  int32_t a_mtiles;
  int32_t a_part0;
};

template <int MODE>
__global__ void __launch_bounds__(256) pack_b_kernel(TcParams prm, unsigned char* __restrict__ ws) {
  constexpr int BK = MODE == 2 ? 64 : 32;
  constexpr int EPC = MODE == 2 ? 8 : 4;
  constexpr int NIMG = MODE == 0 ? 2 : 1;
  int unit = blockIdx.x;
  int pi = 0;
  if (prm.n_parts == 2 && unit >= prm.p[0].ntiles * prm.p[0].kblocks) {
    unit -= prm.p[0].ntiles * prm.p[0].kblocks;
    pi = 1;
  }
  const TcPart& P = prm.p[pi];
  const int nt = unit / P.kblocks, kb = unit % P.kblocks;
  unsigned char* img = ws + P.img_off + ((int64_t)(nt * P.kblocks + kb) * NIMG) * TC_TILE_BYTES;
  for (int q = threadIdx.x; q < 128 * 8; q += blockDim.x) {
    const int c = q >> 7, n = q & 127;
    const int gn = nt * TC_BN + n;
    const int k0 = kb * BK + c * EPC;
    float w[EPC];
#pragma unroll
    for (int e = 0; e < EPC; ++e) w[e] = (gn < P.N && k0 + e < P.K) ? P.B[(int64_t)(k0 + e) * P.ldb + gn] : 0.f;
    const uint32_t off = sw128_off(n, c);
    if constexpr (MODE == 2) {
      __nv_bfloat162 h[4];
#pragma unroll
      for (int e = 0; e < 4; ++e) h[e] = __floats2bfloat162_rn(w[2 * e], w[2 * e + 1]);
      *reinterpret_cast<uint4*>(img + off) = *reinterpret_cast<uint4*>(h);
    } else {
      uint4 hi;
      hi.x = tf32_mask(w[0]); hi.y = tf32_mask(w[1]); hi.z = tf32_mask(w[2]); hi.w = tf32_mask(w[3]);
      *reinterpret_cast<uint4*>(img + off) = hi;
      if constexpr (MODE == 0) {
        uint4 lo;
        lo.x = tf32_mask(w[0] - __uint_as_float(hi.x)); lo.y = tf32_mask(w[1] - __uint_as_float(hi.y));
        lo.z = tf32_mask(w[2] - __uint_as_float(hi.z)); lo.w = tf32_mask(w[3] - __uint_as_float(hi.w));
        *reinterpret_cast<uint4*>(img + TC_TILE_BYTES + off) = lo;
      }
    }
  }
}

__device__ unsigned long long g_tc_dbg[32];
__device__ __forceinline__ void dbg_stamp(int slot) {
  if (blockIdx.x == 0 && blockIdx.y == 0) {
    unsigned long long t;
    asm volatile("mov.u64 %0, %%globaltimer;" : "=l"(t));
    g_tc_dbg[slot] = t;
  }
}

template <int MODE, bool ASYNC = false>
struct TcCfg {
  static constexpr int BK = MODE == 2 ? 64 : 32;
  static constexpr int UK = MODE == 2 ? 16 : 8;
  static constexpr int NIMG = MODE == 0 ? 2 : 1;
  static constexpr int IMG_BYTES = NIMG * TC_TILE_BYTES;
  static constexpr int SA = MODE == 0 ? 2 : 3;
  static constexpr int NB = ASYNC ? (MODE == 0 ? 2 : 4) : (MODE == 0 ? 4 : 8);
  static constexpr int RAW_BYTES = TC_BM * BK * 4;
  static constexpr int RAW_SLOTS = ASYNC ? (MODE == 2 ? 3 : 4) : 0;
  static constexpr int B_OFF = SA * IMG_BYTES;
  static constexpr int RAW_OFF = B_OFF + NB * IMG_BYTES;
  static constexpr int SMEM_BYTES = RAW_OFF + RAW_SLOTS * RAW_BYTES + 1024;
};


template <int MODE>
__device__ __forceinline__ void load_a_chunk(const TcPart& P, int64_t M, int64_t grow, int gcol, bool vec, float (&v)[8]) {
  constexpr int EPC = MODE == 2 ? 8 : 4;
#pragma unroll
  for (int e = 0; e < 8; ++e) v[e] = 0.f;
  if (grow >= M) return;
  const float* src = P.A + grow * P.lda + gcol;
  if (vec && gcol + EPC <= P.K) {
    float4 a = ldg_nc_f4(reinterpret_cast<const float4*>(src));
    v[0] = a.x; v[1] = a.y; v[2] = a.z; v[3] = a.w;
    if constexpr (EPC == 8) {
      float4 b = ldg_nc_f4(reinterpret_cast<const float4*>(src) + 1);
      v[4] = b.x; v[5] = b.y; v[6] = b.z; v[7] = b.w;
    }
  } else {
#pragma unroll
    for (int e = 0; e < EPC; ++e)
      if (gcol + e < P.K) v[e] = __ldg(src + e);
  }
}

template <int MODE>
__device__ __forceinline__ void store_a_chunk(unsigned char* a_img, int row, int c, const float (&v)[8]) {
  const uint32_t off = sw128_off(row, c);
  if constexpr (MODE == 2) {
    __nv_bfloat162 h[4];
#pragma unroll
    for (int e = 0; e < 4; ++e) h[e] = __floats2bfloat162_rn(v[2 * e], v[2 * e + 1]);
    *reinterpret_cast<uint4*>(a_img + off) = *reinterpret_cast<uint4*>(h);
  } else {
    uint4 hi;
    hi.x = tf32_mask(v[0]); hi.y = tf32_mask(v[1]); hi.z = tf32_mask(v[2]); hi.w = tf32_mask(v[3]);
    *reinterpret_cast<uint4*>(a_img + off) = hi;
    if constexpr (MODE == 0) {
      uint4 lo;
      lo.x = tf32_mask(v[0] - __uint_as_float(hi.x)); lo.y = tf32_mask(v[1] - __uint_as_float(hi.y));
      lo.z = tf32_mask(v[2] - __uint_as_float(hi.z)); lo.w = tf32_mask(v[3] - __uint_as_float(hi.w));
      *reinterpret_cast<uint4*>(a_img + TC_TILE_BYTES + off) = lo;
    }
  }
}

template <int MODE, bool ASYNC>
__global__ void __launch_bounds__(TC_THREADS, 1) sage_gemm_tc_kernel(const __grid_constant__ TcParams prm,
                                                                     const unsigned char* __restrict__ ws) {
  using C = TcCfg<MODE, ASYNC>;
  extern __shared__ unsigned char smem_raw[];
  __shared__ __align__(8) uint64_t full_a[C::SA], empty_a[C::SA], full_b[C::NB], empty_b[C::NB], accum_bar;
  __shared__ uint32_t tmem_base_smem;

  unsigned char* smem = reinterpret_cast<unsigned char*>((reinterpret_cast<uintptr_t>(smem_raw) + 1023) & ~(uintptr_t)1023);
  const int warp = threadIdx.x >> 5, lane = threadIdx.x & 31;
  if (threadIdx.x == 0) dbg_stamp(0);

  const int64_t m0 = (int64_t)blockIdx.x * TC_BM;
  int part_lo = 0, part_hi = prm.n_parts, ntile = blockIdx.y, col_off = 0;
  if (prm.combine == GS_COMBINE_CONCAT && prm.n_parts == 2) {
    if ((int)blockIdx.y < prm.tiles_n0) part_hi = 1;
    else { part_lo = 1; ntile = blockIdx.y - prm.tiles_n0; col_off = prm.p[0].N; }
  }
  const int N = prm.p[part_lo].N;
  int total_it = 0;
  for (int pi = part_lo; pi < part_hi; ++pi) total_it += prm.p[pi].kblocks;

  if (threadIdx.x == 0) {
    for (int s = 0; s < C::SA; ++s) {
      mbar_init(&full_a[s], ASYNC ? TC_PRODUCER_WARPS : TC_PRODUCER_WARPS / 2);
      mbar_init(&empty_a[s], 1);
    }
    for (int s = 0; s < C::NB; ++s) {
      mbar_init(&full_b[s], 1);
      mbar_init(&empty_b[s], 1);
    }
    mbar_init(&accum_bar, 1);
    fence_mbar_init();
  }
  if (warp == TC_PRODUCER_WARPS) {
    tmem_alloc(&tmem_base_smem, TC_BN);
    tmem_relinquish();
  }
  tc_fence_before();
  __syncthreads();
  tc_fence_after();
  const uint32_t tmem_acc = tmem_base_smem;
  if (threadIdx.x == 0) dbg_stamp(1);

  if (warp < TC_PRODUCER_WARPS) {
    if constexpr (ASYNC) {
      constexpr int EPC = MODE == 2 ? 8 : 4;
      constexpr int CPT = 4;
      constexpr int RAW_PER_CHUNK = EPC / 4;
      unsigned char* raw = smem + C::RAW_OFF;
      const int tid = threadIdx.x;
      auto locate = [&](int it, int& pi, int& kb) {
        pi = part_lo; kb = it;
        while (kb >= prm.p[pi].kblocks) { kb -= prm.p[pi].kblocks; ++pi; }
      };
      auto issue = [&](int it) {
        if (it < total_it) {
          int pi, kb;
          locate(it, pi, kb);
          const TcPart& P = prm.p[pi];
          unsigned char* slot = raw + (size_t)(it % C::RAW_SLOTS) * C::RAW_BYTES;
#pragma unroll
          for (int i = 0; i < CPT; ++i) {
            const int q = tid + 256 * i;
            const int row = q >> 3, c = q & 7;
            const int64_t grow = m0 + row;
#pragma unroll
            for (int h = 0; h < RAW_PER_CHUNK; ++h) {
              const int gcol = kb * C::BK + c * EPC + h * 4;
              int nbytes = 0;
              if (grow < prm.M && gcol < P.K) nbytes = min(4, P.K - gcol) * 4;
              const float* src = nbytes ? (P.A + grow * P.lda + gcol) : P.A;
              cp_async16(slot + (size_t)(q * RAW_PER_CHUNK + h) * 16, src, nbytes);
            }
          }
        }
        cp_async_commit();
      };
#pragma unroll
      for (int j = 0; j < C::RAW_SLOTS - 1; ++j) issue(j);
      for (int it = 0; it < total_it; ++it) {
        issue(it + C::RAW_SLOTS - 1);
        cp_async_wait<C::RAW_SLOTS - 1>();
        const unsigned char* slot = raw + (size_t)(it % C::RAW_SLOTS) * C::RAW_BYTES;
        float v[CPT][8];
#pragma unroll
        for (int i = 0; i < CPT; ++i) {
          const int q = tid + 256 * i;
#pragma unroll
          for (int h = 0; h < RAW_PER_CHUNK; ++h) {
            const float4 f = *reinterpret_cast<const float4*>(slot + (size_t)(q * RAW_PER_CHUNK + h) * 16);
            v[i][h * 4 + 0] = f.x; v[i][h * 4 + 1] = f.y; v[i][h * 4 + 2] = f.z; v[i][h * 4 + 3] = f.w;
          }
        }
        const int s = it % C::SA;
        const uint32_t ph = (uint32_t)(it / C::SA) & 1u;
        mbar_wait(&empty_a[s], ph ^ 1u);
        unsigned char* a_img = smem + (size_t)s * C::IMG_BYTES;
#pragma unroll
        for (int i = 0; i < CPT; ++i) {
          const int q = tid + 256 * i;
          store_a_chunk<MODE>(a_img, q >> 3, q & 7, v[i]);
        }
        fence_proxy_async();
        __syncwarp();
        if (lane == 0) mbar_arrive(&full_a[s]);
      }
    } else {
    const int group = warp >> 2;
    const int tg = threadIdx.x & 127;
    const int c = tg & 7, r0 = tg >> 3;
    float cur[8][8];
    auto locate = [&](int it, int& pi, int& kb) {
      pi = part_lo; kb = it;
      while (kb >= prm.p[pi].kblocks) { kb -= prm.p[pi].kblocks; ++pi; }
    };
    auto fetch = [&](int it, float (&dst)[8][8]) {
      int pi, kb;
      locate(it, pi, kb);
      const TcPart& P = prm.p[pi];
      const bool vec = ((P.lda & 3) == 0) && ((reinterpret_cast<uintptr_t>(P.A) & 15u) == 0);
      const int gcol = kb * C::BK + c * (MODE == 2 ? 8 : 4);
#pragma unroll
      for (int i = 0; i < 8; ++i) load_a_chunk<MODE>(P, prm.M, m0 + r0 + 16 * i, gcol, vec, dst[i]);
    };
    int it = group;
    if (it < total_it) fetch(it, cur);
    for (; it < total_it; it += 2) {
      const int s = it % C::SA;
      const uint32_t ph = (uint32_t)(it / C::SA) & 1u;
      float nxt[8][8];
      const bool more = it + 2 < total_it;
      if (more) fetch(it + 2, nxt);
      mbar_wait(&empty_a[s], ph ^ 1u);
      unsigned char* a_img = smem + (size_t)s * C::IMG_BYTES;
#pragma unroll
      for (int i = 0; i < 8; ++i) store_a_chunk<MODE>(a_img, r0 + 16 * i, c, cur[i]);
      fence_proxy_async();
      __syncwarp();
      if (lane == 0) mbar_arrive(&full_a[s]);
      if (threadIdx.x == 0 && it == 0) dbg_stamp(2);
      if (threadIdx.x == 0 && it + 2 >= total_it) dbg_stamp(3);
      if (more) {
#pragma unroll
        for (int i = 0; i < 8; ++i)
#pragma unroll
          for (int e = 0; e < 8; ++e) cur[i][e] = nxt[i][e];
      }
    }
    }
    if (threadIdx.x == 0) dbg_stamp(4);
    mbar_wait(&accum_bar, 0);
    tc_fence_after();
    if (threadIdx.x == 0) dbg_stamp(5);
    const int q = warp & 3;
    const int half = warp >> 2;
    const int64_t grow = m0 + q * 32 + lane;
#pragma unroll
    for (int cb = 0; cb < 2; ++cb) {
      const int col0 = half * 64 + cb * 32;
      uint32_t r[32];
      tmem_ld_32x32(tmem_acc + ((uint32_t)(q * 32) << 16) + (uint32_t)col0, r);
      tmem_ld_wait();
      if (grow < prm.M) {
        const int gn0 = ntile * TC_BN + col0;
        float* dst = prm.out + grow * prm.ldo + col_off + gn0;
        const bool vec = ((reinterpret_cast<uintptr_t>(dst) & 15u) == 0) && gn0 + 32 <= N;
#pragma unroll
        for (int j = 0; j < 32; j += 4) {
          float v[4];
#pragma unroll
          for (int e = 0; e < 4; ++e) {
            v[e] = __uint_as_float(r[j + e]);
            if (prm.bias && gn0 + j + e < N) v[e] += prm.bias[col_off + gn0 + j + e];
            if (prm.act == GS_ACT_RELU) v[e] = fmaxf(v[e], 0.f);
          }
          if (vec) {
            *reinterpret_cast<float4*>(dst + j) = make_float4(v[0], v[1], v[2], v[3]);
          } else {
#pragma unroll
            for (int e = 0; e < 4; ++e)
              if (gn0 + j + e < N) dst[j + e] = v[e];
          }
        }
      }
    }
    tc_fence_before();
    if (threadIdx.x == 0) dbg_stamp(6);
  } else if (warp == TC_PRODUCER_WARPS) {
    constexpr uint32_t idesc = make_idesc(MODE == 2 ? 1u : 2u, TC_BM, TC_BN);
    for (int it = 0; it < total_it; ++it) {
      const int s = it % C::SA, sb = it % C::NB;
      mbar_wait(&full_a[s], (uint32_t)(it / C::SA) & 1u);
      if (lane == 0 && it == 0) dbg_stamp(8);
      mbar_wait(&full_b[sb], (uint32_t)(it / C::NB) & 1u);
      tc_fence_after();
      if (lane == 0 && it == 0) dbg_stamp(9);
      if (lane == 0 && it == 1) dbg_stamp(10);
      if (lane == 0 && it == 8) dbg_stamp(11);
      if (lane == 0 && it == total_it - 1) dbg_stamp(12);
      const uint32_t a_base = smem_u32(smem + (size_t)s * C::IMG_BYTES);
      const uint32_t b_base = smem_u32(smem + C::B_OFF + (size_t)sb * C::IMG_BYTES);
      const uint64_t a_hi = make_smem_desc(a_base), b_hi = make_smem_desc(b_base);
      if (prm.issue_elect) {
#pragma unroll
        for (int k = 0; k < C::BK / C::UK; ++k) {
          const uint64_t koff = (uint64_t)((k * 32) >> 4);
          const uint32_t acc = (it > 0 || k > 0) ? 1u : 0u;
          umma_ss_elect<MODE == 2>(tmem_acc, a_hi + koff, b_hi + koff, idesc, acc);
          if constexpr (MODE == 0) {
            const uint64_t a_lo = make_smem_desc(a_base + TC_TILE_BYTES), b_lo = make_smem_desc(b_base + TC_TILE_BYTES);
            umma_ss_elect<false>(tmem_acc, a_hi + koff, b_lo + koff, idesc, 1u);
            umma_ss_elect<false>(tmem_acc, a_lo + koff, b_hi + koff, idesc, 1u);
          }
        }
        umma_commit_elect(&empty_a[s]);
        umma_commit_elect(&empty_b[sb]);
        if (it == total_it - 1) umma_commit_elect(&accum_bar);
        if (lane == 0 && it == total_it - 1) dbg_stamp(13);
      } else if (lane == 0) {
#pragma unroll
        for (int k = 0; k < C::BK / C::UK; ++k) {
          const uint64_t koff = (uint64_t)((k * 32) >> 4);
          const uint32_t acc = (it > 0 || k > 0) ? 1u : 0u;
          umma_ss<MODE == 2>(tmem_acc, a_hi + koff, b_hi + koff, idesc, acc);
          if constexpr (MODE == 0) {
            const uint64_t a_lo = make_smem_desc(a_base + TC_TILE_BYTES), b_lo = make_smem_desc(b_base + TC_TILE_BYTES);
            umma_ss<false>(tmem_acc, a_hi + koff, b_lo + koff, idesc, 1u);
            umma_ss<false>(tmem_acc, a_lo + koff, b_hi + koff, idesc, 1u);
          }
        }
        umma_commit(&empty_a[s]);
        umma_commit(&empty_b[sb]);
        if (it == total_it - 1) umma_commit(&accum_bar);
        if (it == total_it - 1) dbg_stamp(13);
      }
      __syncwarp();
    }
  } else {
    if (lane == 0) {
      int it = 0;
      for (int pi = part_lo; pi < part_hi; ++pi) {
        const TcPart& P = prm.p[pi];
        const unsigned char* base = ws + P.img_off + (int64_t)ntile * P.kblocks * C::NIMG * TC_TILE_BYTES;
        for (int kb = 0; kb < P.kblocks; ++kb, ++it) {
          const int sb = it % C::NB;
          const uint32_t ph = (uint32_t)(it / C::NB) & 1u;
          mbar_wait(&empty_b[sb], ph ^ 1u);
          mbar_expect_tx(&full_b[sb], C::IMG_BYTES);
          bulk_g2s(smem + C::B_OFF + (size_t)sb * C::IMG_BYTES, base + (int64_t)kb * C::IMG_BYTES, C::IMG_BYTES,
                   &full_b[sb]);
        }
      }
    }
    __syncwarp();
  }
  __syncthreads();
  if (threadIdx.x == 0) dbg_stamp(7);
  if (warp == TC_PRODUCER_WARPS) {
    tc_fence_after();
    tmem_dealloc(tmem_acc, TC_BN);
  }
}

constexpr int TCI_THREADS = 256;
constexpr int TCI_IMG = 2 * TC_TILE_BYTES;
constexpr int TCI_SA = 3, TCI_NB = 3;
constexpr int TCI_SMEM = (TCI_SA + TCI_NB) * TCI_IMG + 1024;

__global__ void __launch_bounds__(TCI_THREADS, 1) sage_gemm_tc_img_kernel(const __grid_constant__ TcParams prm,
                                                                          const unsigned char* __restrict__ ws) {
  extern __shared__ unsigned char smem_raw[];
  __shared__ __align__(8) uint64_t full_a[TCI_SA], empty_a[TCI_SA], full_b[TCI_NB], empty_b[TCI_NB], accum_bar;
  __shared__ uint32_t tmem_base_smem;
  unsigned char* smem = reinterpret_cast<unsigned char*>((reinterpret_cast<uintptr_t>(smem_raw) + 1023) & ~(uintptr_t)1023);
  unsigned char* a_ring = smem;
  unsigned char* b_ring = smem + TCI_SA * TCI_IMG;
  const int warp = threadIdx.x >> 5, lane = threadIdx.x & 31;

  const int64_t m0 = (int64_t)blockIdx.x * TC_BM;
  int part_lo = 0, part_hi = prm.n_parts, ntile = blockIdx.y, col_off = 0;
  if (prm.combine == GS_COMBINE_CONCAT && prm.n_parts == 2) {
    if ((int)blockIdx.y < prm.tiles_n0) part_hi = 1;
    else { part_lo = 1; ntile = blockIdx.y - prm.tiles_n0; col_off = prm.p[0].N; }
  }
  const int N = prm.p[part_lo].N;
  int total_it = 0;
  for (int pi = part_lo; pi < part_hi; ++pi) total_it += prm.p[pi].kblocks;

  if (threadIdx.x == 0) {
    for (int s = 0; s < TCI_SA; ++s) { mbar_init(&full_a[s], 1); mbar_init(&empty_a[s], 1); }
    for (int s = 0; s < TCI_NB; ++s) { mbar_init(&full_b[s], 1); mbar_init(&empty_b[s], 1); }
    mbar_init(&accum_bar, 1);
    fence_mbar_init();
  }
  if (warp == 2) {
    tmem_alloc(&tmem_base_smem, TC_BN);
    tmem_relinquish();
  }
  tc_fence_before();
  __syncthreads();
  tc_fence_after();
  const uint32_t tmem_acc = tmem_base_smem;

  if (warp == 0) {
    if (lane == 0) {
      int it = 0;
      for (int pi = part_lo; pi < part_hi; ++pi) {
        const TcPart& P = prm.p[pi];
        const unsigned char* base = prm.a_img + (((int64_t)(prm.a_part0 + pi) * prm.a_mtiles + blockIdx.x) * P.kblocks) * TCI_IMG;
        for (int kb = 0; kb < P.kblocks; ++kb, ++it) {
          const int sa = it % TCI_SA;
          mbar_wait(&empty_a[sa], ((uint32_t)(it / TCI_SA) & 1u) ^ 1u);
          mbar_expect_tx(&full_a[sa], TCI_IMG);
          bulk_g2s(a_ring + (size_t)sa * TCI_IMG, base + (int64_t)kb * TCI_IMG, TCI_IMG, &full_a[sa]);
        }
      }
    }
    __syncwarp();
  } else if (warp == 1) {
    if (lane == 0) {
      int it = 0;
      for (int pi = part_lo; pi < part_hi; ++pi) {
        const TcPart& P = prm.p[pi];
        const unsigned char* base = ws + P.img_off + (int64_t)ntile * P.kblocks * TCI_IMG;
        for (int kb = 0; kb < P.kblocks; ++kb, ++it) {
          const int sb = it % TCI_NB;
          mbar_wait(&empty_b[sb], ((uint32_t)(it / TCI_NB) & 1u) ^ 1u);
          mbar_expect_tx(&full_b[sb], TCI_IMG);
          bulk_g2s(b_ring + (size_t)sb * TCI_IMG, base + (int64_t)kb * TCI_IMG, TCI_IMG, &full_b[sb]);
        }
      }
    }
    __syncwarp();
  } else if (warp == 2) {
    constexpr uint32_t idesc = make_idesc(2u, TC_BM, TC_BN);
    for (int it = 0; it < total_it; ++it) {
      const int sa = it % TCI_SA, sb = it % TCI_NB;
      mbar_wait_uniform(&full_a[sa], (uint32_t)(it / TCI_SA) & 1u);
      mbar_wait_uniform(&full_b[sb], (uint32_t)(it / TCI_NB) & 1u);
      tc_fence_after();
      const uint32_t a_base = smem_u32(a_ring + (size_t)sa * TCI_IMG), b_base = smem_u32(b_ring + (size_t)sb * TCI_IMG);
      const uint64_t a_hi = make_smem_desc(a_base), b_hi = make_smem_desc(b_base);
      const uint64_t a_lo = make_smem_desc(a_base + TC_TILE_BYTES), b_lo = make_smem_desc(b_base + TC_TILE_BYTES);
#pragma unroll
      for (int k = 0; k < 4; ++k) {
        const uint64_t koff = (uint64_t)((k * 32) >> 4);
        umma_ss_elect<false>(tmem_acc, a_hi + koff, b_hi + koff, idesc, (it > 0 || k > 0) ? 1u : 0u);
        umma_ss_elect<false>(tmem_acc, a_hi + koff, b_lo + koff, idesc, 1u);
        umma_ss_elect<false>(tmem_acc, a_lo + koff, b_hi + koff, idesc, 1u);
      }
      umma_commit_elect(&empty_a[sa]);
      umma_commit_elect(&empty_b[sb]);
      if (it == total_it - 1) umma_commit_elect(&accum_bar);
    }
  } else if (warp >= 4) {
    mbar_wait(&accum_bar, 0);
    tc_fence_after();
    const int q = warp & 3;
    const int64_t grow = m0 + q * 32 + lane;
#pragma unroll 1
    for (int cb = 0; cb < 4; ++cb) {
      const int col0 = cb * 32;
      uint32_t r[32];
      tmem_ld_32x32(tmem_acc + ((uint32_t)(q * 32) << 16) + (uint32_t)col0, r);
      tmem_ld_wait();
      if (grow < prm.M) {
        const int gn0 = ntile * TC_BN + col0;
        float* dst = prm.out + grow * prm.ldo + col_off + gn0;
        const bool vec = ((reinterpret_cast<uintptr_t>(dst) & 15u) == 0) && gn0 + 32 <= N;
#pragma unroll
        for (int j = 0; j < 32; j += 4) {
          float v[4];
#pragma unroll
          for (int e = 0; e < 4; ++e) {
            v[e] = __uint_as_float(r[j + e]);
            if (prm.bias && gn0 + j + e < N) v[e] += prm.bias[col_off + gn0 + j + e];
            if (prm.act == GS_ACT_RELU) v[e] = fmaxf(v[e], 0.f);
          }
          if (vec) {
            *reinterpret_cast<float4*>(dst + j) = make_float4(v[0], v[1], v[2], v[3]);
          } else {
#pragma unroll
            for (int e = 0; e < 4; ++e)
              if (gn0 + j + e < N) dst[j + e] = v[e];
          }
        }
      }
    }
    tc_fence_before();
  }
  __syncthreads();
  if (warp == 2) {
    tc_fence_after();
    tmem_dealloc(tmem_acc, TC_BN);
  }
}

static int mode_of(int32_t math) { return math == GS_MATH_TF32X3 ? 0 : math == GS_MATH_TF32 ? 1 : 2; }

static void fill_parts(TcParams& prm, int64_t M, const gs_gemm_part* parts, int32_t n_parts, int mode) {
  const int BK = mode == 2 ? 64 : 32;
  const int nimg = mode == 0 ? 2 : 1;
  memset(&prm, 0, sizeof(prm));
  prm.n_parts = n_parts;
  prm.M = M;
  int64_t off = 0;
  for (int i = 0; i < n_parts; ++i) {
    TcPart& P = prm.p[i];
    P.A = parts[i].A; P.lda = parts[i].lda; P.K = parts[i].K; P.N = parts[i].N;
    P.B = parts[i].B; P.ldb = parts[i].ldb;
    P.kblocks = (P.K + BK - 1) / BK;
    P.ntiles = (P.N + TC_BN - 1) / TC_BN;
    P.img_off = off;
    off += (int64_t)P.kblocks * P.ntiles * nimg * TC_TILE_BYTES;
  }
  prm.tiles_n0 = prm.p[0].ntiles;
  prm.issue_elect = tuning("mma_issue", 1) != 0;
}

int64_t sage_gemm_tc_workspace(int64_t M, const gs_gemm_part* parts, int32_t n_parts, int32_t math) {
  TcParams prm;
  fill_parts(prm, M, parts, n_parts, mode_of(math));
  const TcPart& L = prm.p[n_parts - 1];
  const int nimg = mode_of(math) == 0 ? 2 : 1;
  return L.img_off + (int64_t)L.kblocks * L.ntiles * nimg * TC_TILE_BYTES;
}

template <int MODE>
static int32_t launch_pack(const TcParams& prm, unsigned char* ws, cudaStream_t st) {
  int units = prm.p[0].ntiles * prm.p[0].kblocks + (prm.n_parts == 2 ? prm.p[1].ntiles * prm.p[1].kblocks : 0);
  pack_b_kernel<MODE><<<units, 256, 0, st>>>(prm, ws);
  return launch_check("pack_b_kernel");
}

template <int MODE, bool ASYNC>
static int32_t launch_tc_impl(const TcParams& prm, const unsigned char* ws, cudaStream_t st) {
  using C = TcCfg<MODE, ASYNC>;
  {
    const int32_t rc_attr = ensure_dyn_smem((const void*)sage_gemm_tc_kernel<MODE, ASYNC>, C::SMEM_BYTES);
    if (rc_attr != GS_OK) return rc_attr;
  }
  int tiles_n = prm.p[0].ntiles;
  if (prm.combine == GS_COMBINE_CONCAT && prm.n_parts == 2) tiles_n += prm.p[1].ntiles;
  dim3 grid((unsigned)((prm.M + TC_BM - 1) / TC_BM), (unsigned)tiles_n);
  sage_gemm_tc_kernel<MODE, ASYNC><<<grid, TC_THREADS, C::SMEM_BYTES, st>>>(prm, ws);
  return launch_check("sage_gemm_tc_kernel");
}

template <int MODE>
static int32_t launch_tc(const TcParams& prm, const unsigned char* ws, cudaStream_t st) {
  bool aligned = true;
  for (int i = 0; i < prm.n_parts; ++i)
    aligned = aligned && (prm.p[i].lda % 4 == 0) && ((reinterpret_cast<uintptr_t>(prm.p[i].A) & 15u) == 0);
  if (aligned && tuning("gemm_async", 0)) return launch_tc_impl<MODE, true>(prm, ws, st);
  return launch_tc_impl<MODE, false>(prm, ws, st);
}

int32_t tc_debug_read(unsigned long long* out_host, int n) {
  if (n > 32) n = 32;
  GS_CUDA(cudaDeviceSynchronize());
  GS_CUDA(cudaMemcpyFromSymbol(out_host, g_tc_dbg, sizeof(unsigned long long) * n));
  return GS_OK;
}

int32_t sage_gemm_tc_pack(const gs_gemm_part* parts, int32_t n_parts, int32_t math, void* workspace, cudaStream_t st) {
  GS_REQUIRE(workspace != nullptr && (reinterpret_cast<uintptr_t>(workspace) & 127u) == 0,
             "gs_sage_gemm_pack: workspace must be non-NULL and 128-byte aligned");
  const int mode = mode_of(math);
  TcParams prm;
  fill_parts(prm, 0, parts, n_parts, mode);
  unsigned char* ws = (unsigned char*)workspace;
  if (mode == 0) return launch_pack<0>(prm, ws, st);
  if (mode == 1) return launch_pack<1>(prm, ws, st);
  return launch_pack<2>(prm, ws, st);
}

int32_t sage_gemm_tc_img(int64_t M, const gs_gemm_part* parts, int32_t n_parts, int32_t combine, const float* bias, int32_t act,
                         float* out, int64_t ldo, const void* workspace, const void* a_images, int32_t a_part0,
                         cudaStream_t st) {
  GS_REQUIRE(workspace != nullptr && (reinterpret_cast<uintptr_t>(workspace) & 127u) == 0,
             "gs_sage_gemm_img: packed weights missing or not 128-byte aligned");
  GS_REQUIRE(a_images != nullptr && (reinterpret_cast<uintptr_t>(a_images) & 1023u) == 0,
             "gs_sage_gemm_img: A images missing or not 1024-byte aligned");
  TcParams prm;
  fill_parts(prm, M, parts, n_parts, 0);
  for (int i = 1; i < n_parts; ++i)
    GS_REQUIRE(prm.p[i].K == prm.p[0].K, "gs_sage_gemm_img: every part must have the K of the gathered rows");
  prm.combine = combine; prm.bias = bias; prm.act = act; prm.out = out; prm.ldo = ldo;
  prm.a_img = (const unsigned char*)a_images;
  prm.a_mtiles = (int32_t)((M + TC_BM - 1) / TC_BM);
  prm.a_part0 = a_part0;
  const int32_t rc_attr = ensure_dyn_smem((const void*)sage_gemm_tc_img_kernel, TCI_SMEM);
  if (rc_attr != GS_OK) return rc_attr;
  int tiles_n = prm.p[0].ntiles;
  if (combine == GS_COMBINE_CONCAT && n_parts == 2) tiles_n += prm.p[1].ntiles;
  dim3 grid((unsigned)prm.a_mtiles, (unsigned)tiles_n);
  sage_gemm_tc_img_kernel<<<grid, TCI_THREADS, TCI_SMEM, st>>>(prm, (const unsigned char*)workspace);
  return launch_check("sage_gemm_tc_img_kernel");
}

int32_t sage_gemm_tc(int64_t M, const gs_gemm_part* parts, int32_t n_parts, int32_t combine, const float* bias,
                     int32_t act, int32_t math, float* out, int64_t ldo, const void* workspace, cudaStream_t st) {
  GS_REQUIRE(workspace != nullptr, "gs_sage_gemm: tensor-core math modes need the workspace (gs_sage_gemm_workspace_bytes)");
  GS_REQUIRE((reinterpret_cast<uintptr_t>(workspace) & 127u) == 0, "gs_sage_gemm: workspace must be 128-byte aligned");
  const int mode = mode_of(math);
  TcParams prm;
  fill_parts(prm, M, parts, n_parts, mode);
  prm.combine = combine;
  prm.bias = bias;
  prm.act = act;
  prm.out = out;
  prm.ldo = ldo;
  const unsigned char* ws = (const unsigned char*)workspace;
  if (mode == 0) return launch_tc<0>(prm, ws, st);
  if (mode == 1) return launch_tc<1>(prm, ws, st);
  return launch_tc<2>(prm, ws, st);
}

}
```

### graphsage_b200/csrc/layer_small.cu

```cuda
#include "common.cuh"

namespace gs {

constexpr int LS_ROWS = 4;
constexpr int LS_THREADS = 512;

struct LsParams {
  const float* src;
  int64_t n_src_rows, pitch;
  int32_t F;
  gs_segment seg;
  int32_t include_self;
  gs_gemm_part p[2];
  int32_t n_parts, combine;
  const float* bias;
  int32_t act, l2norm;
  float* out;
  int64_t ldo;
  uint64_t* counter_dev;
  uint64_t counter_inc;
  int32_t vec;
};

__device__ __forceinline__ int64_t ls_clamp(int64_t id, int64_t n) { return (id < 0 || id >= n) ? n - 1 : id; }

__global__ void __launch_bounds__(LS_THREADS) sage_layer_small_kernel(const __grid_constant__ LsParams prm) {
  extern __shared__ float sm[];
  const int F = prm.F;
  float* xs = sm;
  float* xm = sm + LS_ROWS * F;
  const gs_segment& sg = prm.seg;
  const int k = sg.k;
  const int64_t row0 = (int64_t)blockIdx.x * LS_ROWS;
  if (prm.vec) {
    const int f4 = F >> 2;
    for (int p = threadIdx.x; p < f4 * LS_ROWS; p += LS_THREADS) {
      const int r = p / f4, c4 = p - r * f4;
      const int64_t i = row0 + r;
      float4 acc = make_float4(0.f, 0.f, 0.f, 0.f), sv = acc;
      if (i < sg.n) {
        const int64_t srow = ls_clamp(sg.self_ids ? (int64_t)sg.self_ids[i] : sg.self_row0 + i, prm.n_src_rows);
        sv = ldg_nc_f4(reinterpret_cast<const float4*>(prm.src + srow * prm.pitch) + c4);
        for (int j0 = 0; j0 < k; j0 += 5) {
          float4 v[5];
#pragma unroll
          for (int u = 0; u < 5; ++u) {
            v[u] = make_float4(0.f, 0.f, 0.f, 0.f);
            if (j0 + u < k) {
              const int64_t nr = ls_clamp(sg.neigh_ids ? (int64_t)sg.neigh_ids[i * k + j0 + u] : sg.neigh_row0 + i * k + j0 + u,
                                          prm.n_src_rows);
              v[u] = ldg_nc_f4(reinterpret_cast<const float4*>(prm.src + nr * prm.pitch) + c4);
            }
          }
#pragma unroll
          for (int u = 0; u < 5; ++u) { acc.x += v[u].x; acc.y += v[u].y; acc.z += v[u].z; acc.w += v[u].w; }
        }
        const float div = (float)(k + (prm.include_self ? 1 : 0));
        if (prm.include_self) { acc.x += sv.x; acc.y += sv.y; acc.z += sv.z; acc.w += sv.w; }
        acc.x /= div; acc.y /= div; acc.z /= div; acc.w /= div;
      }
      reinterpret_cast<float4*>(xs + r * F)[c4] = sv;
      reinterpret_cast<float4*>(xm + r * F)[c4] = acc;
    }
  } else
  for (int c = threadIdx.x; c < F; c += LS_THREADS) {
    float acc[LS_ROWS], sv[LS_ROWS];
#pragma unroll
    for (int r = 0; r < LS_ROWS; ++r) {
      acc[r] = 0.f;
      const int64_t i = row0 + r;
      sv[r] = 0.f;
      if (i < sg.n) {
        const int64_t srow = ls_clamp(sg.self_ids ? (int64_t)sg.self_ids[i] : sg.self_row0 + i, prm.n_src_rows);
        sv[r] = prm.src[srow * prm.pitch + c];
      }
    }
    for (int j0 = 0; j0 < k; j0 += 5) {
      float v[LS_ROWS][5];
#pragma unroll
      for (int r = 0; r < LS_ROWS; ++r) {
        const int64_t i = row0 + r;
#pragma unroll
        for (int u = 0; u < 5; ++u) {
          v[r][u] = 0.f;
          if (i < sg.n && j0 + u < k) {
            const int64_t nr = ls_clamp(sg.neigh_ids ? (int64_t)sg.neigh_ids[i * k + j0 + u] : sg.neigh_row0 + i * k + j0 + u,
                                        prm.n_src_rows);
            v[r][u] = prm.src[nr * prm.pitch + c];
          }
        }
      }
#pragma unroll
      for (int r = 0; r < LS_ROWS; ++r)
#pragma unroll
        for (int u = 0; u < 5; ++u) acc[r] += v[r][u];
    }
#pragma unroll
    for (int r = 0; r < LS_ROWS; ++r) {
      float a = acc[r];
      if (prm.include_self) a += sv[r];
      a /= (float)(k + (prm.include_self ? 1 : 0));
      xs[r * F + c] = sv[r];
      xm[r * F + c] = (row0 + r < sg.n) ? a : 0.f;
    }
  }
  __syncthreads();
  const int N0 = prm.p[0].N;
  const int ntot = (prm.n_parts == 2 && prm.combine == GS_COMBINE_CONCAT) ? N0 + prm.p[1].N : N0;
  const int ncolp = (ntot + 31) & ~31;
  const int ncgp = prm.vec ? ((((ntot + 3) >> 2) + 31) & ~31) : 0;
  const int nslices = prm.vec ? (ncgp <= LS_THREADS ? LS_THREADS / ncgp : 1) : (ncolp <= LS_THREADS ? LS_THREADS / ncolp : 1);
  float* part = xm + LS_ROWS * F;
  float* red = part + nslices * LS_ROWS * ncolp;
  if (prm.vec) {
    const int ncg = ntot >> 2;
    const int sl = threadIdx.x / ncgp;
    const int cg0 = threadIdx.x - sl * ncgp;
    for (int cg = cg0; cg < ncg && sl < nslices; cg += (nslices == 1 ? LS_THREADS : ncgp)) {
      const int col = cg * 4;
      float4 acc[LS_ROWS];
#pragma unroll
      for (int r = 0; r < LS_ROWS; ++r) acc[r] = make_float4(0.f, 0.f, 0.f, 0.f);
      for (int pi = 0; pi < prm.n_parts; ++pi) {
        int c = col;
        if (prm.n_parts == 2 && prm.combine == GS_COMBINE_CONCAT) {
          if ((pi == 0) != (col < N0)) continue;
          if (pi == 1) c = col - N0;
        }
        const gs_gemm_part& P = prm.p[pi];
        const float* x = (prm.n_parts == 1 || pi == 1) ? xm : xs;
        const float* w = P.B + c;
        const int kchunk = (((P.K + nslices - 1) / nslices) + 3) & ~3;
        const int kbeg = sl * kchunk, kend = min(P.K, kbeg + kchunk);
        float4 wn[4];
        if (kbeg < kend) {
#pragma unroll
          for (int u = 0; u < 4; ++u) wn[u] = __ldg(reinterpret_cast<const float4*>(w + (int64_t)(kbeg + u) * P.ldb));
        }
        for (int kk = kbeg; kk < kend; kk += 4) {
          float4 wv[4];
#pragma unroll
          for (int u = 0; u < 4; ++u) wv[u] = wn[u];
          if (kk + 4 < kend) {
#pragma unroll
            for (int u = 0; u < 4; ++u) wn[u] = __ldg(reinterpret_cast<const float4*>(w + (int64_t)(kk + 4 + u) * P.ldb));
          }
#pragma unroll
          for (int r = 0; r < LS_ROWS; ++r) {
            const float4 xv = *reinterpret_cast<const float4*>(x + r * F + kk);
            acc[r].x = fmaf(xv.x, wv[0].x, acc[r].x); acc[r].y = fmaf(xv.x, wv[0].y, acc[r].y);
            acc[r].z = fmaf(xv.x, wv[0].z, acc[r].z); acc[r].w = fmaf(xv.x, wv[0].w, acc[r].w);
            acc[r].x = fmaf(xv.y, wv[1].x, acc[r].x); acc[r].y = fmaf(xv.y, wv[1].y, acc[r].y);
            acc[r].z = fmaf(xv.y, wv[1].z, acc[r].z); acc[r].w = fmaf(xv.y, wv[1].w, acc[r].w);
            acc[r].x = fmaf(xv.z, wv[2].x, acc[r].x); acc[r].y = fmaf(xv.z, wv[2].y, acc[r].y);
            acc[r].z = fmaf(xv.z, wv[2].z, acc[r].z); acc[r].w = fmaf(xv.z, wv[2].w, acc[r].w);
            acc[r].x = fmaf(xv.w, wv[3].x, acc[r].x); acc[r].y = fmaf(xv.w, wv[3].y, acc[r].y);
            acc[r].z = fmaf(xv.w, wv[3].z, acc[r].z); acc[r].w = fmaf(xv.w, wv[3].w, acc[r].w);
          }
        }
      }
#pragma unroll
      for (int r = 0; r < LS_ROWS; ++r) *reinterpret_cast<float4*>(part + (sl * LS_ROWS + r) * ncolp + col) = acc[r];
      if (nslices > 1) break;
    }
  }
  const int slice = prm.vec ? nslices : (nslices == 1 ? 0 : threadIdx.x / ncolp);
  const int col_step = nslices == 1 ? LS_THREADS : ncolp;
  for (int col = (nslices == 1 ? threadIdx.x : threadIdx.x % ncolp); col < ntot && slice < nslices; col += col_step) {
    float acc[LS_ROWS];
#pragma unroll
    for (int r = 0; r < LS_ROWS; ++r) acc[r] = 0.f;
    for (int pi = 0; pi < prm.n_parts; ++pi) {
      int c = col;
      if (prm.n_parts == 2 && prm.combine == GS_COMBINE_CONCAT) {
        if ((pi == 0) != (col < N0)) continue;
        if (pi == 1) c = col - N0;
      }
      const gs_gemm_part& P = prm.p[pi];
      const float* x = (prm.n_parts == 1 || pi == 1) ? xm : xs;
      const float* w = P.B + c;
      const int kchunk = (((P.K + nslices - 1) / nslices) + 7) & ~7;
      const int kbeg = slice * kchunk, kend = min(P.K, kbeg + kchunk);
      int kk = kbeg;
      for (; kk + 8 <= kend; kk += 8) {
        float wv[8];
#pragma unroll
        for (int u = 0; u < 8; ++u) wv[u] = __ldg(w + (int64_t)(kk + u) * P.ldb);
#pragma unroll
        for (int u = 0; u < 8; ++u)
#pragma unroll
          for (int r = 0; r < LS_ROWS; ++r) acc[r] = fmaf(x[r * F + kk + u], wv[u], acc[r]);
      }
      for (; kk < kend; ++kk) {
        const float wv = __ldg(w + (int64_t)kk * P.ldb);
#pragma unroll
        for (int r = 0; r < LS_ROWS; ++r) acc[r] = fmaf(x[r * F + kk], wv, acc[r]);
      }
    }
#pragma unroll
    for (int r = 0; r < LS_ROWS; ++r) part[(slice * LS_ROWS + r) * ncolp + col] = acc[r];
    if (nslices > 1) break;
  }
  __syncthreads();
  float ss[LS_ROWS];
#pragma unroll
  for (int r = 0; r < LS_ROWS; ++r) ss[r] = 0.f;
  for (int col = threadIdx.x; col < ntot; col += LS_THREADS) {
#pragma unroll
    for (int r = 0; r < LS_ROWS; ++r) {
      float v = 0.f;
      for (int s2 = 0; s2 < nslices; ++s2) v += part[(s2 * LS_ROWS + r) * ncolp + col];
      if (prm.bias) v += prm.bias[col];
      if (prm.act == GS_ACT_RELU) v = fmaxf(v, 0.f);
      ss[r] += v * v;
      part[r * ncolp + col] = v;
    }
  }
  float inv[LS_ROWS];
#pragma unroll
  for (int r = 0; r < LS_ROWS; ++r) inv[r] = 1.f;
  if (prm.l2norm) {
#pragma unroll
    for (int r = 0; r < LS_ROWS; ++r) {
      float t = ss[r];
#pragma unroll
      for (int o = 16; o > 0; o >>= 1) t += __shfl_xor_sync(0xffffffffu, t, o);
      if ((threadIdx.x & 31) == 0) red[r * 16 + (threadIdx.x >> 5)] = t;
    }
    __syncthreads();
#pragma unroll
    for (int r = 0; r < LS_ROWS; ++r) {
      float tot = 0.f;
#pragma unroll
      for (int w = 0; w < LS_THREADS / 32; ++w) tot += red[r * 16 + w];
      inv[r] = 1.0f / sqrtf(fmaxf(tot, 1e-12f));
    }
  }
  for (int col = threadIdx.x; col < ntot; col += LS_THREADS) {
#pragma unroll
    for (int r = 0; r < LS_ROWS; ++r)
      if (row0 + r < sg.n) prm.out[(sg.out_row0 + row0 + r) * prm.ldo + col] = part[r * ncolp + col] * inv[r];
  }
  if (prm.counter_dev != nullptr && blockIdx.x == 0 && threadIdx.x == 0) *prm.counter_dev += prm.counter_inc;
}

}

extern "C" int32_t gs_sage_layer_small(const float* src, int64_t n_src_rows, int32_t F, int64_t pitch,
                                       const gs_segment* segment_host, int32_t include_self,
                                       const gs_gemm_part* parts_host, int32_t n_parts, int32_t combine, const float* bias,
                                       int32_t act, int32_t l2_normalize, float* out, int64_t ldo, uint64_t* counter_dev,
                                       uint64_t counter_inc, void* stream) {
  GS_REQUIRE(src && segment_host && parts_host && out, "gs_sage_layer_small: NULL pointer");
  GS_REQUIRE(n_parts == 1 || n_parts == 2, "gs_sage_layer_small: n_parts=%d", n_parts);
  GS_REQUIRE(F >= 1 && F <= 2048 && pitch >= F && n_src_rows > 0, "gs_sage_layer_small: F=%d (max 2048) / pitch", F);
  GS_REQUIRE(segment_host->k >= 1 && segment_host->n >= 0, "gs_sage_layer_small: bad segment");
  GS_REQUIRE(combine == GS_COMBINE_ADD || combine == GS_COMBINE_CONCAT, "gs_sage_layer_small: combine=%d", combine);
  GS_REQUIRE(act == GS_ACT_NONE || act == GS_ACT_RELU, "gs_sage_layer_small: act=%d", act);
  gs::LsParams prm;
  memset(&prm, 0, sizeof(prm));
  int ntot = 0;
  for (int i = 0; i < n_parts; ++i) {
    GS_REQUIRE(parts_host[i].B && parts_host[i].K == F && parts_host[i].N >= 1 && parts_host[i].ldb >= parts_host[i].N,
               "gs_sage_layer_small: part %d must have K == F (%d) and a valid B", i, F);
    prm.p[i] = parts_host[i];
  }
  if (n_parts == 2 && combine == GS_COMBINE_ADD)
    GS_REQUIRE(parts_host[0].N == parts_host[1].N, "gs_sage_layer_small: ADD needs equal N");
  ntot = parts_host[0].N + ((n_parts == 2 && combine == GS_COMBINE_CONCAT) ? parts_host[1].N : 0);
  GS_REQUIRE(ntot <= 1024 && ldo >= ntot, "gs_sage_layer_small: output width %d (max 1024) / ldo", ntot);
  if (segment_host->n == 0) return GS_OK;
  prm.src = src; prm.n_src_rows = n_src_rows; prm.pitch = pitch; prm.F = F;
  prm.seg = *segment_host; prm.include_self = include_self;
  prm.n_parts = n_parts; prm.combine = combine; prm.bias = bias; prm.act = act; prm.l2norm = l2_normalize;
  prm.out = out; prm.ldo = ldo; prm.counter_dev = counter_dev; prm.counter_inc = counter_inc;
  bool vec = (F % 4 == 0) && (pitch % 4 == 0) && ((reinterpret_cast<uintptr_t>(src) & 15u) == 0) && (ntot % 4 == 0) &&
             (parts_host[0].N % 4 == 0);
  for (int i = 0; i < n_parts; ++i)
    vec = vec && (parts_host[i].ldb % 4 == 0) && ((reinterpret_cast<uintptr_t>(parts_host[i].B) & 15u) == 0);
  prm.vec = vec ? 1 : 0;
  const int ncolp = (ntot + 31) & ~31;
  const int ncgp = (((ntot + 3) / 4) + 31) & ~31;
  const int nslices = vec ? (ncgp <= gs::LS_THREADS ? gs::LS_THREADS / ncgp : 1)
                          : (ncolp <= gs::LS_THREADS ? gs::LS_THREADS / ncolp : 1);
  const size_t smem = (size_t)(2 * gs::LS_ROWS * F + nslices * gs::LS_ROWS * ncolp + gs::LS_ROWS * 16) * sizeof(float);
  GS_REQUIRE(smem <= 200 * 1024, "gs_sage_layer_small: needs %zu bytes of shared memory", smem);
  {
    const int32_t rc_attr = gs::ensure_dyn_smem((const void*)gs::sage_layer_small_kernel, 200 * 1024);
    if (rc_attr != GS_OK) return rc_attr;
  }
  unsigned blocks = (unsigned)((segment_host->n + gs::LS_ROWS - 1) / gs::LS_ROWS);
  gs::sage_layer_small_kernel<<<blocks, gs::LS_THREADS, smem, (cudaStream_t)stream>>>(prm);
  return gs::launch_check("sage_layer_small_kernel");
}
```

### graphsage_b200/csrc/maxpool_tc.cu

```cuda
#include <cuda.h>

#include "tc_common.cuh"

namespace gs {

constexpr int MP_KCOLS = 32;
constexpr int MP_IMG = TC_BM * 64;
constexpr int MP_MAX_KB = 20;
constexpr int MP_RING = 26;
constexpr int MP_PROD_WARPS = 4;
constexpr int MP_THREADS = (MP_PROD_WARPS + 6) * 32;
constexpr int MP_STAGE_LD = 129;
constexpr int MP_SMEM = MP_RING * MP_IMG + 32 * MP_STAGE_LD * 4 + 1024;

struct MpParams {
  const __nv_bfloat16* table;
  int64_t n_rows, pitch;
  int32_t K, kblocks;
  const int32_t* row_ids;
  int64_t row0;
  int64_t n_groups;
  int32_t k, G;
  int64_t n_tiles;
  int32_t hidden, n_slices;
  const unsigned char* wimg;
  const float* bias;
  int32_t pool_mean;
  float* out;
  int64_t ldo;
  int32_t issue_elect;
  int32_t n_stages;
  int32_t kb_t;
  const uint32_t* wrows;
  int32_t dbg;
};

__host__ __device__ __forceinline__ uint32_t sw64_off(int r, int c) { return (uint32_t)(r * 64 + ((c ^ ((r >> 1) & 3)) << 4)); }

__device__ __forceinline__ uint64_t make_smem_desc64(uint32_t saddr) {
  uint64_t d = 0;
  d |= (uint64_t)((saddr & 0x3FFFFu) >> 4);
  d |= (uint64_t)1 << 16;
  d |= (uint64_t)(512 >> 4) << 32;
  d |= (uint64_t)1 << 46;
  d |= (uint64_t)4 << 61;
  return d;
}

__global__ void __launch_bounds__(256) maxpool_pack_kernel(const float* __restrict__ W, int64_t ldw, int K, int hidden,
                                                           int kblocks, unsigned char* __restrict__ img) {
  const int slice = blockIdx.x / kblocks, kb = blockIdx.x % kblocks;
  unsigned char* dst = img + ((int64_t)slice * kblocks + kb) * MP_IMG;
  for (int q = threadIdx.x; q < 128 * 4; q += blockDim.x) {
    const int c = q >> 7, n = q & 127;
    const int gn = slice * 128 + n, k0 = kb * MP_KCOLS + c * 8;
    __nv_bfloat162 h[4];
#pragma unroll
    for (int e = 0; e < 4; ++e) {
      float a = (gn < hidden && k0 + 2 * e < K) ? W[(int64_t)(k0 + 2 * e) * ldw + gn] : 0.f;
      float b = (gn < hidden && k0 + 2 * e + 1 < K) ? W[(int64_t)(k0 + 2 * e + 1) * ldw + gn] : 0.f;
      h[e] = __floats2bfloat162_rn(a, b);
    }
    *reinterpret_cast<uint4*>(dst + sw64_off(n, c)) = *reinterpret_cast<uint4*>(h);
  }
}

__device__ unsigned long long g_mp_dbg[128];
__device__ __forceinline__ void mp_stamp(uint32_t tcount, int slot) {
  if (blockIdx.x == 0 && tcount < 12) {
    unsigned long long t;
    asm volatile("mov.u64 %0, %%globaltimer;" : "=l"(t));
    g_mp_dbg[tcount * 8 + slot] = t;
  }
}

#ifdef GS_K4_EPI_PROBE
#define MP_EPI_T(var) const long long var = clock64()
#define MP_EPI_ACC(slot, a, b) \
  do {                         \
    if (blockIdx.x == 0 && et == 0) g_mp_dbg[100 + (slot)] += (unsigned long long)((b) - (a)); \
  } while (0)
#else
#define MP_EPI_T(var) \
  do {                \
  } while (0)
#define MP_EPI_ACC(slot, a, b) \
  do {                         \
  } while (0)
#endif


template <int MP_SA, int CL = 1>
__device__ __forceinline__ void mp_mma_role(const MpParams& prm, int lane, int kblocks, int64_t tile0, int64_t tile_step,
                                            uint32_t tmem_base, uint64_t* full_a, uint64_t* empty_a, uint64_t* acc_full,
                                            uint64_t* acc_empty, uint64_t& b_full, unsigned char* a_ring,
                                            unsigned char* b_res) {
  constexpr uint32_t idesc = make_idesc(1u, TC_BM, TC_BN);
  mbar_wait(&b_full, 0);
  uint32_t it = 0, tcount = 0;
  for (int64_t t = tile0; t < prm.n_tiles; t += tile_step, ++tcount) {
    const uint32_t buf = tcount & 1u;
    if (lane == 0) mp_stamp(tcount, 2);
    mbar_wait(&acc_empty[buf], ((tcount >> 1) & 1u) ^ 1u);
    tc_fence_after();
    if (lane == 0) mp_stamp(tcount, 3);
    const uint32_t tmem_acc = tmem_base + buf * 128u;
    for (int kb = 0; kb < kblocks; ++kb, ++it) {
      const int s = it % MP_SA;
      mbar_wait(&full_a[s], (it / MP_SA) & 1u);
      tc_fence_after();
      const uint64_t adesc = make_smem_desc64(smem_u32(a_ring + (size_t)s * MP_IMG));
      const uint64_t bdesc = make_smem_desc64(smem_u32(b_res + (size_t)kb * MP_IMG));
      if (prm.issue_elect) {
#pragma unroll
        for (int k2 = 0; k2 < 2; ++k2)
          umma_ss_elect<true>(tmem_acc, adesc + (uint64_t)(k2 * 2), bdesc + (uint64_t)(k2 * 2), idesc,
                              (kb > 0 || k2 > 0) ? 1u : 0u);
        if constexpr (CL > 1)
          umma_commit_elect_multicast(&empty_a[s], (uint16_t)((1u << CL) - 1u));
        else
          umma_commit_elect(&empty_a[s]);
        if (kb == kblocks - 1) umma_commit_elect(&acc_full[buf]);
        if (lane == 0 && kb == kblocks - 1) mp_stamp(tcount, 4);
      } else if (lane == 0) {
#pragma unroll
        for (int k2 = 0; k2 < 2; ++k2)
          umma_ss<true>(tmem_acc, adesc + (uint64_t)(k2 * 2), bdesc + (uint64_t)(k2 * 2), idesc, (kb > 0 || k2 > 0) ? 1u : 0u);
        umma_commit(&empty_a[s]);
        if (kb == kblocks - 1) umma_commit(&acc_full[buf]);
        if (kb == kblocks - 1) mp_stamp(tcount, 4);
      }
      __syncwarp();
    }
  }
}

__device__ __forceinline__ void mp_weights_role(const MpParams& prm, int lane, int slice, int kblocks, uint64_t& b_full,
                                                unsigned char* b_res) {
  if (lane == 0) {
    mbar_expect_tx(&b_full, (uint32_t)(kblocks * MP_IMG));
    const unsigned char* src = prm.wimg + (int64_t)slice * kblocks * MP_IMG;
    for (int kb = 0; kb < kblocks; ++kb)
      bulk_g2s(b_res + (size_t)kb * MP_IMG, src + (int64_t)kb * MP_IMG, MP_IMG, &b_full);
  }
  __syncwarp();
}

__device__ __forceinline__ void mp_epilogue_role(const MpParams& prm, int et, int warp, int lane, int slice, int64_t tile0,
                                                 int64_t tile_step, uint32_t tmem_base, uint64_t* acc_full,
                                                 uint64_t* acc_empty, float* stage, float* bias_s) {
  const int q = warp & 3;
  const int row = q * 32 + lane;
  const int k = prm.k, G = prm.G;
  bias_s[et] = prm.bias ? prm.bias[slice * 128 + et] : 0.f;
  named_bar_sync(1, 128);
  uint32_t tcount = 0;
  for (int64_t t = tile0; t < prm.n_tiles; t += tile_step, ++tcount) {
    const uint32_t buf = tcount & 1u;
    if (et == 0) mp_stamp(tcount, 5);
    mbar_wait(&acc_full[buf], (tcount >> 1) & 1u);
    tc_fence_after();
    if (et == 0) mp_stamp(tcount, 6);
    const uint32_t tmem_acc = tmem_base + buf * 128u + ((uint32_t)(q * 32) << 16);
#pragma unroll 1
    for (int cb = 0; cb < 4; ++cb) {
      uint32_t r[32];
      MP_EPI_T(e0);
      tmem_ld_32x32(tmem_acc + (uint32_t)(cb * 32), r);
      tmem_ld_wait();
      MP_EPI_T(e1);
      const int hcol0 = slice * 128 + cb * 32;
#pragma unroll
      for (int j = 0; j < 32; ++j) stage[j * MP_STAGE_LD + row] = __uint_as_float(r[j]);
      MP_EPI_T(e2);
      named_bar_sync(1, 128);
      MP_EPI_T(e3);
      {
        const int cc = et & 31;
        for (int g = et >> 5; g < G; g += 4) {
          const int64_t gg = t * G + g;
          if (gg < prm.n_groups) {
            const float* p = stage + cc * MP_STAGE_LD + g * k;
            const float b = bias_s[cb * 32 + cc];
            float res;
            if (prm.pool_mean) {
              float sacc = 0.f;
              for (int j = 0; j < k; ++j) sacc += fmaxf(p[j] + b, 0.f);
              res = sacc / (float)k;
            } else {
              float m = -3.0e38f;
              int j = 0;
              for (; j + 8 <= k; j += 8) {
                float v[8];
#pragma unroll
                for (int u = 0; u < 8; ++u) v[u] = p[j + u];
                m = fmaxf(m, fmaxf(fmaxf(fmaxf(v[0], v[1]), fmaxf(v[2], v[3])), fmaxf(fmaxf(v[4], v[5]), fmaxf(v[6], v[7]))));
              }
              for (; j < k; ++j) m = fmaxf(m, p[j]);
              res = fmaxf(m + b, 0.f);
            }
            prm.out[gg * prm.ldo + hcol0 + cc] = res;
          }
        }
      }
      MP_EPI_T(e4);
      named_bar_sync(1, 128);
      MP_EPI_T(e5);
      MP_EPI_ACC(0, e0, e1);
      MP_EPI_ACC(1, e1, e2);
      MP_EPI_ACC(2, e2, e3);
      MP_EPI_ACC(3, e3, e4);
      MP_EPI_ACC(4, e4, e5);
      MP_EPI_ACC(5, 0, 1);
    }
    tc_fence_before();
    __syncwarp();
    if (lane == 0) mbar_arrive(&acc_empty[buf]);
    if (et == 0) mp_stamp(tcount, 7);
  }
}

template <int MP_SA, int MP_INFLIGHT, bool kAsyncArrive = false>
__global__ void __launch_bounds__(MP_THREADS, 1) maxpool_mlp_kernel(const __grid_constant__ MpParams prm) {
  static_assert(MP_INFLIGHT + 2 <= MP_SA, "a stage must be free while MP_INFLIGHT copies fly and one is consumed");
  extern __shared__ unsigned char smem_raw[];
  __shared__ __align__(8) uint64_t full_a[MP_SA], empty_a[MP_SA], acc_full[2], acc_empty[2], b_full;
  __shared__ uint32_t tmem_base_smem;
  __shared__ float bias_s[128];
  unsigned char* smem = reinterpret_cast<unsigned char*>((reinterpret_cast<uintptr_t>(smem_raw) + 1023) & ~(uintptr_t)1023);
  unsigned char* b_res = smem;
  unsigned char* a_ring = smem + (MP_RING - MP_SA) * MP_IMG;
  float* stage = reinterpret_cast<float*>(smem + MP_RING * MP_IMG);

  const int warp = threadIdx.x >> 5, lane = threadIdx.x & 31;
  const int slice = blockIdx.x % prm.n_slices;
  const int64_t tile0 = blockIdx.x / prm.n_slices, tile_step = gridDim.x / prm.n_slices;
  const int kblocks = prm.kblocks;

  if (threadIdx.x == 0) {
    for (int s = 0; s < MP_SA; ++s) {
      mbar_init(&full_a[s], kAsyncArrive ? MP_PROD_WARPS * 32 : MP_PROD_WARPS);
      mbar_init(&empty_a[s], 1);
    }
    for (int b = 0; b < 2; ++b) {
      mbar_init(&acc_full[b], 1);
      mbar_init(&acc_empty[b], 4);
    }
    mbar_init(&b_full, 1);
    fence_mbar_init();
  }
  if (warp == MP_PROD_WARPS) {
    tmem_alloc(&tmem_base_smem, 256);
    tmem_relinquish();
  }
  tc_fence_before();
  __syncthreads();
  tc_fence_after();
  const uint32_t tmem_base = tmem_base_smem;

  if (warp < MP_PROD_WARPS) {
    const int tid = threadIdx.x;
    const int c = tid & 3, r0 = tid >> 2;
    const int rows_valid = prm.G * prm.k;
    uint32_t it = 0;
    int pending = 0;
    auto publish = [&](uint32_t which) {
      const int s = which % MP_SA;
      fence_proxy_async();
      __syncwarp();
      if (lane == 0) mbar_arrive(&full_a[s]);
    };
    uint32_t ptile = 0;
    for (int64_t t = tile0; t < prm.n_tiles; t += tile_step, ++ptile) {
      if (threadIdx.x == 0) mp_stamp(ptile, 0);
      const __nv_bfloat16* rowp[4];
#pragma unroll
      for (int i = 0; i < 4; ++i) {
        const int r = r0 + 32 * i;
        const int64_t flat = t * rows_valid + r;
        rowp[i] = nullptr;
        if (r < rows_valid && flat < prm.n_groups * prm.k) {
          int64_t id = prm.row_ids ? (int64_t)prm.row_ids[flat] : prm.row0 + flat;
          if (id < 0 || id >= prm.n_rows) id = prm.n_rows - 1;
          rowp[i] = prm.table + id * prm.pitch;
        }
      }
      for (int kb = 0; kb < kblocks; ++kb, ++it) {
        const int s = it % MP_SA;
        mbar_wait(&empty_a[s], ((it / MP_SA) & 1u) ^ 1u);
        unsigned char* a_img = a_ring + (size_t)s * MP_IMG;
        const int col = kb * MP_KCOLS + c * 8;
#pragma unroll
        for (int i = 0; i < 4; ++i) {
          int nbytes = 0;
          if (rowp[i] != nullptr && col < prm.K) nbytes = min(8, prm.K - col) * 2;
          const void* src = nbytes ? (const void*)(rowp[i] + col) : (const void*)prm.table;
          cp_async16(a_img + sw64_off(r0 + 32 * i, c), src, nbytes);
        }
        if constexpr (kAsyncArrive) {
          cp_async_mbar_arrive_noinc(&full_a[s]);
          continue;
        }
        cp_async_commit();
        ++pending;
        if (pending == MP_INFLIGHT + 1) {
          cp_async_wait<MP_INFLIGHT>();
          publish(it - MP_INFLIGHT);
          --pending;
        }
      }
      if (threadIdx.x == 0) mp_stamp(ptile, 1);
    }
    while (pending > 0) {
      if (pending >= 5) cp_async_wait<4>();
      else if (pending == 4) cp_async_wait<3>();
      else if (pending == 3) cp_async_wait<2>();
      else if (pending == 2) cp_async_wait<1>();
      else cp_async_wait<0>();
      publish(it - pending);
      --pending;
    }
  } else if (warp == MP_PROD_WARPS) {
    mp_mma_role<MP_SA>(prm, lane, kblocks, tile0, tile_step, tmem_base, full_a, empty_a, acc_full, acc_empty, b_full, a_ring,
                       b_res);
  } else if (warp == MP_PROD_WARPS + 1) {
    mp_weights_role(prm, lane, slice, kblocks, b_full, b_res);
  } else {
    mp_epilogue_role(prm, (int)threadIdx.x - (MP_PROD_WARPS + 2) * 32, warp, lane, slice, tile0, tile_step, tmem_base, acc_full,
                     acc_empty, stage, bias_s);
  }
  __syncthreads();
  if (warp == MP_PROD_WARPS) {
    tc_fence_after();
    tmem_dealloc(tmem_base, 256);
  }
}

constexpr int MPW_SMEM_BYTES = 28 * MP_IMG;
constexpr int MPW_MAX_STAGES = 8;
constexpr int MPW_SMEM = MPW_SMEM_BYTES + 1024;

template <int KC>
__host__ __device__ __forceinline__ uint32_t mpw_off(int r, int c) {
  if constexpr (KC == 32) return sw64_off(r, c);
  else return sw128_off(r, c);
}
template <int KC>
__device__ __forceinline__ uint64_t mpw_desc(uint32_t saddr) {
  if constexpr (KC == 32) return make_smem_desc64(saddr);
  else return make_smem_desc(saddr);
// ... 1589 lines not shown
```

### graphsage_b200/csrc/sampler.cu

```cuda
#include "common.cuh"

namespace gs {

constexpr int kMaxDegSmem = 1024;

__global__ void __launch_bounds__(256) sample_padded_kernel(const int32_t* __restrict__ adj, int64_t n_rows,
                                                            int32_t max_deg, const int32_t* __restrict__ ids,
                                                            int64_t n, int32_t k,
                                                            const int32_t* __restrict__ col_perm, uint64_t seed,
                                                            uint64_t counter, const uint64_t* __restrict__ counter_dev,
                                                            int32_t* __restrict__ out) {
  __shared__ int16_t perm[kMaxDegSmem];
  __shared__ int32_t pi[kMaxDegSmem];
  if (col_perm != nullptr) {
    for (int j = threadIdx.x; j < k; j += blockDim.x) pi[j] = col_perm[j];
  } else {
    for (int j = threadIdx.x; j < max_deg; j += blockDim.x) perm[j] = (int16_t)j;
    __syncthreads();
    if (threadIdx.x == 0) {
      uint64_t ctr = counter + (counter_dev ? *counter_dev : 0ull);
      u32x4 r{0, 0, 0, 0};
      for (int i = 0; i < k; ++i) {
        if ((i & 3) == 0) {
          u32x4 c{(uint32_t)ctr, (uint32_t)(ctr >> 32), 0u, kStreamPadded + (uint32_t)(i >> 2)};
          r = philox4x32_10(c, (uint32_t)seed, (uint32_t)(seed >> 32));
        }
        int j = i + (int)mulhi32(pick(r, i & 3), (uint32_t)(max_deg - i));
        int16_t t = perm[i];
        perm[i] = perm[j];
        perm[j] = t;
        pi[i] = perm[i];
      }
    }
  }
  __syncthreads();
  const int64_t total = n * (int64_t)k;
  for (int64_t e = (int64_t)blockIdx.x * blockDim.x + threadIdx.x; e < total; e += (int64_t)gridDim.x * blockDim.x) {
    int64_t i = e / k;
    int j = (int)(e - i * k);
    int64_t id = ids[i];
    if (id < 0 || id >= n_rows) id = n_rows - 1;
    out[e] = adj[id * max_deg + pi[j]];
  }
}

struct KhopParams {
  int32_t* out[GS_MAX_HOPS];
  int32_t fanout[GS_MAX_HOPS];
  int64_t count[GS_MAX_HOPS];
  int32_t n_hops;
};

__global__ void __launch_bounds__(512) sample_padded_khop_kernel(const int32_t* __restrict__ adj, int64_t n_rows,
                                                                 int32_t max_deg, const int32_t* __restrict__ seeds,
                                                                 const __grid_constant__ KhopParams kp, uint64_t seed,
                                                                 uint64_t counter,
                                                                 const uint64_t* __restrict__ counter_dev) {
  __shared__ int16_t perm[GS_MAX_HOPS][kMaxDegSmem];
  __shared__ int32_t pi[GS_MAX_HOPS][64];
  const int warp = threadIdx.x >> 5, lane = threadIdx.x & 31;
  if (warp < kp.n_hops) {
    for (int j = lane; j < max_deg; j += 32) perm[warp][j] = (int16_t)j;
    __syncwarp();
    const uint64_t ctr = counter + (counter_dev ? *counter_dev : 0ull) + (uint64_t)warp;
    const int k = kp.fanout[warp];
    for (int blk = lane; blk * 4 < k; blk += 32) {
      u32x4 c{(uint32_t)ctr, (uint32_t)(ctr >> 32), 0u, kStreamPadded + (uint32_t)blk};
      u32x4 r = philox4x32_10(c, (uint32_t)seed, (uint32_t)(seed >> 32));
      pi[warp][blk * 4 + 0] = (int32_t)r.x;
      if (blk * 4 + 1 < 64) pi[warp][blk * 4 + 1] = (int32_t)r.y;
      if (blk * 4 + 2 < 64) pi[warp][blk * 4 + 2] = (int32_t)r.z;
      if (blk * 4 + 3 < 64) pi[warp][blk * 4 + 3] = (int32_t)r.w;
    }
    __syncwarp();
    if (lane == 0) {
      for (int i = 0; i < k; ++i) {
        int j = i + (int)mulhi32((uint32_t)pi[warp][i], (uint32_t)(max_deg - i));
        int16_t t = perm[warp][i];
        perm[warp][i] = perm[warp][j];
        perm[warp][j] = t;
        pi[warp][i] = perm[warp][i];
      }
    }
  }
  __syncthreads();
  int64_t total = 0;
  for (int t = 0; t < kp.n_hops; ++t) total += kp.count[t];
  for (int64_t e = (int64_t)blockIdx.x * blockDim.x + threadIdx.x; e < total; e += (int64_t)gridDim.x * blockDim.x) {
    int hop = 0;
    int64_t local = e;
    while (local >= kp.count[hop]) { local -= kp.count[hop]; ++hop; }
    int64_t sup = 1;
    for (int t = 0; t <= hop; ++t) sup *= kp.fanout[t];
    int64_t id = seeds[local / sup];
    int64_t rem = local % sup;
    for (int t = 0; t <= hop; ++t) {
      sup /= kp.fanout[t];
      const int j = (int)(rem / sup);
      rem -= (int64_t)j * sup;
      if (id < 0 || id >= n_rows) id = n_rows - 1;
      id = adj[id * max_deg + pi[t][j]];
    }
    kp.out[hop][local] = (int32_t)id;
  }
}

__global__ void __launch_bounds__(256) sample_csr_kernel(const int64_t* __restrict__ indptr,
                                                         const int32_t* __restrict__ indices, int64_t n_nodes,
                                                         const int32_t* __restrict__ ids, int64_t n, int32_t k,
                                                         int32_t replace_if_short, uint64_t seed, uint64_t counter,
                                                         const uint64_t* __restrict__ counter_dev, int32_t pad_id,
                                                         int32_t* __restrict__ out) {
  const int lane = threadIdx.x & 31;
  const int64_t warp = ((int64_t)blockIdx.x * blockDim.x + threadIdx.x) >> 5;
  const int64_t nwarps = ((int64_t)gridDim.x * blockDim.x) >> 5;
  const uint64_t ctr = counter + (counter_dev ? *counter_dev : 0ull);
  for (int64_t t = warp; t < n; t += nwarps) {
    int64_t id = ids[t];
    int64_t start = 0, deg = 0;
    if (id >= 0 && id < n_nodes) {
      start = indptr[id];
      deg = indptr[id + 1] - start;
    }
    int32_t res = pad_id;
    uint32_t r = 0;
    if (lane < k && deg > 0) r = philox_draw(seed, ctr, (uint32_t)t, kStreamCsr, lane);
    if (deg >= k) {
      int64_t mine = -1;
      for (int j = 0; j < k; ++j) {
        uint32_t rj = __shfl_sync(0xffffffffu, r, j);
        int64_t m = deg - k + j;
        int64_t tpos = (int64_t)mulhi32(rj, (uint32_t)(m + 1));
        unsigned dup = __ballot_sync(0xffffffffu, lane < j && mine == tpos);
        if (lane == j) mine = dup ? m : tpos;
      }
      if (lane < k) res = indices[start + mine];
    } else if (deg > 0) {
      if (replace_if_short) {
        if (lane < k) res = indices[start + (int64_t)mulhi32(r, (uint32_t)deg)];
      } else {
        if (lane < deg) res = indices[start + lane];
      }
    }
    if (lane < k) out[t * k + lane] = res;
  }
}

__global__ void __launch_bounds__(128) sample_unigram_kernel(const double* __restrict__ cdf, int64_t n, int32_t num,
                                                             uint64_t seed, uint64_t counter,
                                                             const uint64_t* __restrict__ counter_dev,
                                                             int32_t* __restrict__ out) {
  const int j = blockIdx.x * blockDim.x + threadIdx.x;
  if (j >= num) return;
  const uint64_t ctr = counter + (counter_dev ? *counter_dev : 0ull);
  const uint32_t r = philox_draw(seed, ctr, 0u, kStreamUnigram, j);
  const double u = ((double)r + 0.5) * (1.0 / 4294967296.0) * cdf[n - 1];
  int64_t lo = 0, hi = n - 1;
  while (lo < hi) {
    const int64_t mid = (lo + hi) >> 1;
    if (cdf[mid] > u) hi = mid; else lo = mid + 1;
  }
  out[j] = (int32_t)lo;
}

__global__ void __launch_bounds__(256) build_padded_adj_kernel(const int64_t* __restrict__ indptr,
                                                               const int32_t* __restrict__ indices, int64_t n_nodes,
                                                               int32_t max_deg, const uint8_t* __restrict__ skip,
                                                               uint64_t seed, uint64_t counter, int32_t* __restrict__ adj,
                                                               float* __restrict__ deg_out) {
  __shared__ int32_t sel[8][kMaxDegSmem];
  const int lane = threadIdx.x & 31, w = threadIdx.x >> 5;
  const int64_t warp = (int64_t)blockIdx.x * 8 + w;
  const int64_t nwarps = (int64_t)gridDim.x * 8;
  for (int64_t u = warp; u <= n_nodes; u += nwarps) {
    int32_t* row = adj + u * max_deg;
    int64_t start = 0, deg = 0;
    if (u < n_nodes && !(skip && skip[u])) {
      start = indptr[u];
      deg = indptr[u + 1] - start;
    }
    if (u < n_nodes && deg_out && lane == 0) deg_out[u] = (float)deg;
    if (deg == 0) {
      for (int j = lane; j < max_deg; j += 32) row[j] = (int32_t)n_nodes;
    } else if (deg == max_deg) {
      for (int j = lane; j < max_deg; j += 32) row[j] = indices[start + j];
    } else if (deg < max_deg) {
      for (int j = lane; j < max_deg; j += 32) {
        const uint32_t r = philox_draw(seed, counter, (uint32_t)u, kStreamBuild, j);
        row[j] = indices[start + (int64_t)mulhi32(r, (uint32_t)deg)];
      }
    } else {
      for (int j = 0; j < max_deg; ++j) {
        const int64_t m = deg - max_deg + j;
        const uint32_t r = philox_draw(seed, counter, (uint32_t)u, kStreamBuild, j);
        const int32_t t = (int32_t)mulhi32(r, (uint32_t)(m + 1));
        bool dup = false;
        for (int q = lane; q < j; q += 32) dup |= (sel[w][q] == t);
        dup = __any_sync(0xffffffffu, dup);
        if (lane == 0) sel[w][j] = dup ? (int32_t)m : t;
        __syncwarp();
      }
      for (int j = lane; j < max_deg; j += 32) row[j] = indices[start + sel[w][j]];
      __syncwarp();
    }
  }
}

}

extern "C" {

int32_t gs_sample_padded(const int32_t* adj, int64_t n_rows, int32_t max_deg, const int32_t* ids, int64_t n, int32_t k,
                         const int32_t* col_perm, uint64_t seed, uint64_t counter, const uint64_t* counter_dev,
                         int32_t* out, void* stream) {
  GS_REQUIRE(n >= 0 && k >= 0, "gs_sample_padded: negative size (n=%lld, k=%d)", (long long)n, k);
  if (n == 0 || k == 0) return GS_OK;
  GS_REQUIRE(adj && ids && out, "gs_sample_padded: NULL pointer");
  GS_REQUIRE(n_rows > 0 && max_deg > 0 && max_deg <= gs::kMaxDegSmem, "gs_sample_padded: need 0 < max_deg <= %d (got %d)",
             gs::kMaxDegSmem, max_deg);
  GS_REQUIRE(k <= max_deg, "gs_sample_padded: num_samples %d > max_degree %d", k, max_deg);
  int64_t total = n * (int64_t)k;
  int64_t blocks = (total + 255) / 256;
  int64_t cap = (int64_t)gs::sm_count() * 8;
  if (blocks > cap) blocks = cap;
  gs::sample_padded_kernel<<<(unsigned)blocks, 256, 0, (cudaStream_t)stream>>>(adj, n_rows, max_deg, ids, n, k, col_perm,
                                                                               seed, counter, counter_dev, out);
  return gs::launch_check("sample_padded_kernel");
}

int32_t gs_sample_padded_khop(const int32_t* adj, int64_t n_rows, int32_t max_deg, const int32_t* seeds, int64_t n_seeds,
                              const int32_t* fanout_host, int32_t n_hops, uint64_t seed, uint64_t counter,
                              const uint64_t* counter_dev, int32_t* const* out_host, void* stream) {
  GS_REQUIRE(n_hops >= 1 && n_hops <= GS_MAX_HOPS, "gs_sample_padded_khop: n_hops=%d (max %d)", n_hops, GS_MAX_HOPS);
  GS_REQUIRE(fanout_host && out_host, "gs_sample_padded_khop: NULL host array");
  GS_REQUIRE(n_seeds >= 0, "gs_sample_padded_khop: n_seeds < 0");
  if (n_seeds == 0) return GS_OK;
  GS_REQUIRE(adj && seeds, "gs_sample_padded_khop: NULL pointer");
  GS_REQUIRE(n_rows > 0 && max_deg > 0 && max_deg <= gs::kMaxDegSmem, "gs_sample_padded_khop: need 0 < max_deg <= %d",
             gs::kMaxDegSmem);
  gs::KhopParams kp;
  memset(&kp, 0, sizeof(kp));
  kp.n_hops = n_hops;
  int64_t cnt = n_seeds, total = 0;
  for (int t = 0; t < n_hops; ++t) {
    GS_REQUIRE(fanout_host[t] >= 1 && fanout_host[t] <= max_deg && fanout_host[t] <= 64,
               "gs_sample_padded_khop: fanout[%d]=%d (need 1..min(64, max_degree))", t, fanout_host[t]);
    GS_REQUIRE(out_host[t] != nullptr, "gs_sample_padded_khop: out[%d] is NULL", t);
    cnt *= fanout_host[t];
    kp.fanout[t] = fanout_host[t];
    kp.count[t] = cnt;
    kp.out[t] = out_host[t];
    total += cnt;
  }
  int64_t blocks = (total + 511) / 512;
  int64_t cap = (int64_t)gs::sm_count() * 2;
  if (blocks > cap) blocks = cap;
  gs::sample_padded_khop_kernel<<<(unsigned)blocks, 512, 0, (cudaStream_t)stream>>>(adj, n_rows, max_deg, seeds, kp, seed,
                                                                                    counter, counter_dev);
  return gs::launch_check("sample_padded_khop_kernel");
}

int32_t gs_build_padded_adj(const int64_t* indptr, const int32_t* indices, int64_t n_nodes, int32_t max_deg,
                            const uint8_t* skip, uint64_t seed, uint64_t counter, int32_t* adj, float* deg, void* stream) {
  GS_REQUIRE(indptr && indices && adj && n_nodes >= 0, "gs_build_padded_adj: NULL pointer / bad size");
  GS_REQUIRE(max_deg >= 1 && max_deg <= gs::kMaxDegSmem, "gs_build_padded_adj: need 1 <= max_deg <= %d", gs::kMaxDegSmem);
  int64_t blocks = (n_nodes + 1 + 7) / 8;
  int64_t cap = (int64_t)gs::sm_count() * 4;
  if (blocks > cap) blocks = cap;
  gs::build_padded_adj_kernel<<<(unsigned)blocks, 256, 0, (cudaStream_t)stream>>>(indptr, indices, n_nodes, max_deg, skip,
                                                                                   seed, counter, adj, deg);
  return gs::launch_check("build_padded_adj_kernel");
}

int32_t gs_sample_unigram(const double* cdf, int64_t n, int32_t num_sampled, uint64_t seed, uint64_t counter,
                          const uint64_t* counter_dev, int32_t* out, void* stream) {
  GS_REQUIRE(num_sampled >= 0 && n >= 1, "gs_sample_unigram: bad sizes");
  if (num_sampled == 0) return GS_OK;
  GS_REQUIRE(cdf && out, "gs_sample_unigram: NULL pointer");
  gs::sample_unigram_kernel<<<(num_sampled + 127) / 128, 128, 0, (cudaStream_t)stream>>>(cdf, n, num_sampled, seed, counter,
                                                                                       counter_dev, out);
  return gs::launch_check("sample_unigram_kernel");
}

int32_t gs_sample_csr(const int64_t* indptr, const int32_t* indices, int64_t n_nodes, const int32_t* ids, int64_t n,
                      int32_t k, int32_t replace_if_short, uint64_t seed, uint64_t counter, const uint64_t* counter_dev,
                      int32_t pad_id, int32_t* out, void* stream) {
  GS_REQUIRE(n >= 0 && k >= 0, "gs_sample_csr: negative size");
  if (n == 0 || k == 0) return GS_OK;
  GS_REQUIRE(indptr && indices && ids && out, "gs_sample_csr: NULL pointer");
  if (k > 32) {
    gs::set_error("gs_sample_csr: k=%d > 32 not supported (one lane per draw)", k);
    return GS_ERR_UNSUPPORTED;
  }
  int64_t blocks = (n + 7) / 8;
  int64_t cap = (int64_t)gs::sm_count() * 8;
  if (blocks > cap) blocks = cap;
  gs::sample_csr_kernel<<<(unsigned)blocks, 256, 0, (cudaStream_t)stream>>>(indptr, indices, n_nodes, ids, n, k,
                                                                            replace_if_short, seed, counter, counter_dev,
                                                                            pad_id, out);
  return gs::launch_check("sample_csr_kernel");
}

}
```

### graphsage_b200/csrc/tc_common.cuh

```cuda
#pragma once
#include <cuda_bf16.h>

#include "common.cuh"

namespace gs {

constexpr int TC_BM = 128;
constexpr int TC_BN = 128;
constexpr int TC_TILE_BYTES = TC_BM * 128;

__device__ __forceinline__ void tmem_alloc(uint32_t* smem_dst, uint32_t ncols) {
  asm volatile("tcgen05.alloc.cta_group::1.sync.aligned.shared::cta.b32 [%0], %1;" ::"r"(smem_u32(smem_dst)), "r"(ncols)
               : "memory");
}
__device__ __forceinline__ void tmem_relinquish() {
  asm volatile("tcgen05.relinquish_alloc_permit.cta_group::1.sync.aligned;" ::: "memory");
}
__device__ __forceinline__ void tmem_dealloc(uint32_t taddr, uint32_t ncols) {
  asm volatile("tcgen05.dealloc.cta_group::1.sync.aligned.b32 %0, %1;" ::"r"(taddr), "r"(ncols) : "memory");
}
__device__ __forceinline__ void tc_fence_before() { asm volatile("tcgen05.fence::before_thread_sync;" ::: "memory"); }
__device__ __forceinline__ void tc_fence_after() { asm volatile("tcgen05.fence::after_thread_sync;" ::: "memory"); }

__device__ __forceinline__ void umma_commit(uint64_t* bar) {
  asm volatile("tcgen05.commit.cta_group::1.mbarrier::arrive::one.shared::cluster.b64 [%0];" ::"r"(smem_u32(bar))
               : "memory");
}

template <bool kBf16>
__device__ __forceinline__ void umma_ss(uint32_t tmem_d, uint64_t adesc, uint64_t bdesc, uint32_t idesc, uint32_t accumulate) {
  if constexpr (kBf16) {
    asm volatile(
        "{\n\t.reg .pred p;\n\tsetp.ne.b32 p, %4, 0;\n\t"
        "tcgen05.mma.cta_group::1.kind::f16 [%0], %1, %2, %3, p;\n\t}" ::"r"(tmem_d),
        "l"(adesc), "l"(bdesc), "r"(idesc), "r"(accumulate)
        : "memory");
  } else {
    asm volatile(
        "{\n\t.reg .pred p;\n\tsetp.ne.b32 p, %4, 0;\n\t"
        "tcgen05.mma.cta_group::1.kind::tf32 [%0], %1, %2, %3, p;\n\t}" ::"r"(tmem_d),
        "l"(adesc), "l"(bdesc), "r"(idesc), "r"(accumulate)
        : "memory");
  }
}


template <bool kBf16>
__device__ __forceinline__ void umma_ss_elect(uint32_t tmem_d, uint64_t adesc, uint64_t bdesc, uint32_t idesc,
                                              uint32_t accumulate) {
  if constexpr (kBf16) {
    asm volatile(
        "{\n\t.reg .pred p, q;\n\telect.sync _|q, 0xffffffff;\n\tsetp.ne.b32 p, %4, 0;\n\t"
        "@q tcgen05.mma.cta_group::1.kind::f16 [%0], %1, %2, %3, p;\n\t}" ::"r"(tmem_d),
        "l"(adesc), "l"(bdesc), "r"(idesc), "r"(accumulate)
        : "memory");
  } else {
    asm volatile(
        "{\n\t.reg .pred p, q;\n\telect.sync _|q, 0xffffffff;\n\tsetp.ne.b32 p, %4, 0;\n\t"
        "@q tcgen05.mma.cta_group::1.kind::tf32 [%0], %1, %2, %3, p;\n\t}" ::"r"(tmem_d),
        "l"(adesc), "l"(bdesc), "r"(idesc), "r"(accumulate)
        : "memory");
  }
}
__device__ __forceinline__ void umma_commit_elect(uint64_t* bar) {
  asm volatile(
      "{\n\t.reg .pred q;\n\telect.sync _|q, 0xffffffff;\n\t"
      "@q tcgen05.commit.cta_group::1.mbarrier::arrive::one.shared::cluster.b64 [%0];\n\t}" ::"r"(smem_u32(bar))
      : "memory");
}

__device__ __forceinline__ void umma_commit_elect_multicast(uint64_t* bar, uint16_t cta_mask) {
  asm volatile(
      "{\n\t.reg .pred q;\n\telect.sync _|q, 0xffffffff;\n\t"
      "@q tcgen05.commit.cta_group::1.mbarrier::arrive::one.shared::cluster.multicast::cluster.b64 [%0], %1;\n\t}" ::"r"(
          smem_u32(bar)),
      "h"(cta_mask)
      : "memory");
}

__device__ __forceinline__ void tmem_ld_32x32(uint32_t taddr, uint32_t (&r)[32]) {
  asm volatile(
      "tcgen05.ld.sync.aligned.32x32b.x32.b32 "
      "{%0,%1,%2,%3,%4,%5,%6,%7,%8,%9,%10,%11,%12,%13,%14,%15,"
      "%16,%17,%18,%19,%20,%21,%22,%23,%24,%25,%26,%27,%28,%29,%30,%31}, [%32];"
      : "=r"(r[0]), "=r"(r[1]), "=r"(r[2]), "=r"(r[3]), "=r"(r[4]), "=r"(r[5]), "=r"(r[6]), "=r"(r[7]), "=r"(r[8]),
        "=r"(r[9]), "=r"(r[10]), "=r"(r[11]), "=r"(r[12]), "=r"(r[13]), "=r"(r[14]), "=r"(r[15]), "=r"(r[16]),
        "=r"(r[17]), "=r"(r[18]), "=r"(r[19]), "=r"(r[20]), "=r"(r[21]), "=r"(r[22]), "=r"(r[23]), "=r"(r[24]),
        "=r"(r[25]), "=r"(r[26]), "=r"(r[27]), "=r"(r[28]), "=r"(r[29]), "=r"(r[30]), "=r"(r[31])
      : "r"(taddr)
      : "memory");
}
#define GS_TMEM_LD_N(NAME, XN, NREG, OUTS, INIDX)                                                            \
  __device__ __forceinline__ void NAME(uint32_t taddr, uint32_t (&r)[NREG]) {                                 \
    asm volatile("tcgen05.ld.sync.aligned.32x32b." XN ".b32 " OUTS ", [%" INIDX "];" : GS_TMEM_OUT_##NREG(r) : "r"(taddr) : "memory"); \
  }
#define GS_TMEM_OUT_1(r) "=r"(r[0])
#define GS_TMEM_OUT_2(r) "=r"(r[0]), "=r"(r[1])
#define GS_TMEM_OUT_4(r) "=r"(r[0]), "=r"(r[1]), "=r"(r[2]), "=r"(r[3])
#define GS_TMEM_OUT_8(r) GS_TMEM_OUT_4(r), "=r"(r[4]), "=r"(r[5]), "=r"(r[6]), "=r"(r[7])
#define GS_TMEM_OUT_16(r) GS_TMEM_OUT_8(r), "=r"(r[8]), "=r"(r[9]), "=r"(r[10]), "=r"(r[11]), "=r"(r[12]), "=r"(r[13]), "=r"(r[14]), "=r"(r[15])
GS_TMEM_LD_N(tmem_ld_32x1, "x1", 1, "{%0}", "1")
GS_TMEM_LD_N(tmem_ld_32x2, "x2", 2, "{%0,%1}", "2")
GS_TMEM_LD_N(tmem_ld_32x4, "x4", 4, "{%0,%1,%2,%3}", "4")
GS_TMEM_LD_N(tmem_ld_32x8, "x8", 8, "{%0,%1,%2,%3,%4,%5,%6,%7}", "8")
GS_TMEM_LD_N(tmem_ld_32x16, "x16", 16, "{%0,%1,%2,%3,%4,%5,%6,%7,%8,%9,%10,%11,%12,%13,%14,%15}", "16")
__device__ __forceinline__ void umma_ts_elect_bf16(uint32_t tmem_d, uint32_t tmem_a, uint64_t bdesc, uint32_t idesc,
                                                   uint32_t accumulate) {
  asm volatile(
      "{\n\t.reg .pred p, q;\n\telect.sync _|q, 0xffffffff;\n\tsetp.ne.b32 p, %4, 0;\n\t"
      "@q tcgen05.mma.cta_group::1.kind::f16 [%0], [%1], %2, %3, p;\n\t}" ::"r"(tmem_d),
      "r"(tmem_a), "l"(bdesc), "r"(idesc), "r"(accumulate)
      : "memory");
}

__device__ __forceinline__ void tmem_st_32x32(uint32_t taddr, const uint32_t (&r)[32]) {
  asm volatile(
      "tcgen05.st.sync.aligned.32x32b.x32.b32 [%0], "
      "{%1,%2,%3,%4,%5,%6,%7,%8,%9,%10,%11,%12,%13,%14,%15,%16,"
      "%17,%18,%19,%20,%21,%22,%23,%24,%25,%26,%27,%28,%29,%30,%31,%32};" ::"r"(taddr),
      "r"(r[0]), "r"(r[1]), "r"(r[2]), "r"(r[3]), "r"(r[4]), "r"(r[5]), "r"(r[6]), "r"(r[7]), "r"(r[8]), "r"(r[9]), "r"(r[10]),
      "r"(r[11]), "r"(r[12]), "r"(r[13]), "r"(r[14]), "r"(r[15]), "r"(r[16]), "r"(r[17]), "r"(r[18]), "r"(r[19]), "r"(r[20]),
      "r"(r[21]), "r"(r[22]), "r"(r[23]), "r"(r[24]), "r"(r[25]), "r"(r[26]), "r"(r[27]), "r"(r[28]), "r"(r[29]), "r"(r[30]),
      "r"(r[31])
      : "memory");
}
__device__ __forceinline__ void tmem_st_wait() { asm volatile("tcgen05.wait::st.sync.aligned;" ::: "memory"); }

__device__ __forceinline__ void mbar_wait_uniform(uint64_t* bar, uint32_t parity) {
  while (!__all_sync(0xffffffffu, mbar_try_wait(bar, parity))) {
  }
}
__device__ __forceinline__ void tmem_ld_wait() { asm volatile("tcgen05.wait::ld.sync.aligned;" ::: "memory"); }

__device__ __forceinline__ uint64_t make_smem_desc(uint32_t saddr) {
  uint64_t d = 0;
  d |= (uint64_t)((saddr & 0x3FFFFu) >> 4);
  d |= (uint64_t)1 << 16;
  d |= (uint64_t)(1024 >> 4) << 32;
  d |= (uint64_t)1 << 46;
  d |= (uint64_t)2 << 61;
  return d;
}

__host__ __device__ constexpr uint32_t make_idesc(uint32_t fmt, uint32_t M, uint32_t N) {
  return (1u << 4) | (fmt << 7) | (fmt << 10) | ((N >> 3) << 17) | ((M >> 4) << 24);
}

__device__ __forceinline__ uint32_t tf32_mask(float x) { return __float_as_uint(x) & 0xFFFFE000u; }

__host__ __device__ __forceinline__ uint32_t sw128_off(int r, int c) {
  return (uint32_t)(r * 128 + ((c ^ (r & 7)) << 4));
}


__device__ __forceinline__ void cp_async16(void* smem_dst, const void* gsrc, int src_bytes) {
  asm volatile("cp.async.cg.shared.global [%0], [%1], 16, %2;" ::"r"(smem_u32(smem_dst)), "l"(gsrc), "r"(src_bytes) : "memory");
}
__device__ __forceinline__ void cp_async_mbar_arrive_noinc(uint64_t* bar) {
  asm volatile("cp.async.mbarrier.arrive.noinc.shared::cta.b64 [%0];" ::"r"(smem_u32(bar)) : "memory");
}
__device__ __forceinline__ void cp_async_wait_all() { asm volatile("cp.async.wait_all;" ::: "memory"); }
__device__ __forceinline__ void cp_async_commit() { asm volatile("cp.async.commit_group;" ::: "memory"); }
template <int N>
__device__ __forceinline__ void cp_async_wait() { asm volatile("cp.async.wait_group %0;" ::"n"(N) : "memory"); }

__device__ __forceinline__ void named_bar_sync(int id, int nthreads) {
  asm volatile("bar.sync %0, %1;" ::"r"(id), "r"(nthreads) : "memory");
}

}
```

### include/graphsage_b200.h

```cpp
#ifndef GRAPHSAGE_B200_H_
#define GRAPHSAGE_B200_H_

#include <stdint.h>

#ifdef __cplusplus
extern "C" {
#endif

#define GS_ABI_VERSION 2

typedef enum {
  GS_OK = 0,
  GS_ERR_INVALID_ARG = -1,
  GS_ERR_CUDA = -2,
  GS_ERR_UNSUPPORTED = -3
} gs_status;

typedef enum { GS_F32 = 0, GS_BF16 = 1 } gs_dtype;
typedef enum { GS_ACT_NONE = 0, GS_ACT_RELU = 1 } gs_act;
typedef enum {
  GS_COMBINE_ADD = 0,
  GS_COMBINE_CONCAT = 1
} gs_combine;
typedef enum {
  GS_MATH_FP32_SIMT = 0,
  GS_MATH_TF32X3 = 1,
  GS_MATH_TF32 = 2,
  GS_MATH_BF16 = 3
} gs_math;

int32_t gs_version(void);
const char* gs_last_error_string(void);
int32_t gs_set_tuning(const char* key, int32_t value);

int32_t gs_sample_padded(const int32_t* adj, int64_t n_rows, int32_t max_deg,
                         const int32_t* ids, int64_t n, int32_t k,
                         const int32_t* col_perm, uint64_t seed, uint64_t counter,
                         const uint64_t* counter_dev, int32_t* out, void* stream);

#define GS_MAX_HOPS 4
int32_t gs_sample_padded_khop(const int32_t* adj, int64_t n_rows, int32_t max_deg,
                              const int32_t* seeds, int64_t n_seeds, const int32_t* fanout_host,
                              int32_t n_hops, uint64_t seed, uint64_t counter,
                              const uint64_t* counter_dev, int32_t* const* out_host, void* stream);

int32_t gs_sample_csr(const int64_t* indptr, const int32_t* indices, int64_t n_nodes,
                      const int32_t* ids, int64_t n, int32_t k, int32_t replace_if_short,
                      uint64_t seed, uint64_t counter, const uint64_t* counter_dev,
                      int32_t pad_id, int32_t* out, void* stream);

int32_t gs_sample_unigram(const double* cdf, int64_t n, int32_t num_sampled, uint64_t seed, uint64_t counter,
                          const uint64_t* counter_dev, int32_t* out, void* stream);

int32_t gs_build_padded_adj(const int64_t* indptr, const int32_t* indices, int64_t n_nodes, int32_t max_deg,
                            const uint8_t* skip, uint64_t seed, uint64_t counter, int32_t* adj, float* deg,
                            void* stream);

int32_t gs_perm_prefix_host(uint64_t seed, uint64_t counter, int32_t max_deg, int32_t k,
                            int32_t* out_host);

int32_t gs_gather_rows(const void* feats, int32_t dtype, int64_t n_rows, int32_t F,
                       int64_t pitch, const int32_t* ids, int64_t n, void* out,
                       int64_t out_pitch, void* stream);

#define GS_MAX_SEGMENTS 4
typedef struct {
  const int32_t* self_ids;
  const int32_t* neigh_ids;
  int64_t self_row0;
  int64_t neigh_row0;
  int64_t n;
  int32_t k;
  int32_t _pad;
  int64_t out_row0;
} gs_segment;

int32_t gs_gather_mean(const void* src, int32_t dtype, int64_t n_src_rows, int32_t F, int64_t pitch,
                       const gs_segment* segments_host, int32_t n_segments, int32_t include_self,
                       void* out_self, void* out_mean, int64_t out_pitch, void* stream);

#define GS_MAX_SHARDS 16
typedef struct {
  const void* base[GS_MAX_SHARDS];
  int64_t row_start[GS_MAX_SHARDS + 1];
  int32_t n_shards;
  int32_t my_shard;
  int64_t n_global_rows;
  int64_t zero_row;
  const int32_t* remap;
} gs_sharded_table;

int32_t gs_gather_mean_sharded(const gs_sharded_table* table_host, int32_t dtype, int32_t F, int64_t pitch,
                               const gs_segment* segments_host, int32_t n_segments, int32_t include_self,
                               int32_t ids_are_locators, const void* staging, void* out_self, void* out_mean,
                               int64_t out_pitch, void* stream);
int32_t gs_halo_begin(int32_t* claim, int64_t n_global_rows, int32_t* count, void* stream);
int32_t gs_halo_claim(const gs_sharded_table* table_host, const int32_t* ids, int64_t n, int32_t* claim, int32_t* count,
                      int32_t* stage_ids, int64_t capacity, void* stream);
int32_t gs_halo_fetch(const gs_sharded_table* table_host, int32_t F, int64_t pitch, const int32_t* stage_ids,
                      const int32_t* count, int64_t capacity, float* staging, int64_t staging_pitch, void* stream);
int32_t gs_halo_translate(const gs_sharded_table* table_host, const int32_t* ids, int64_t n, const int32_t* claim,
                          int32_t* out, void* stream);
int32_t gs_translate_ids(const gs_sharded_table* table_host, const int32_t* ids, int64_t n, int32_t* out, void* stream);
int32_t gs_gather_rows_sharded(const gs_sharded_table* table_host, int32_t dtype, int32_t F, int64_t pitch,
                               const int32_t* ids, int64_t n, void* out, int64_t out_pitch, void* stream);

int32_t gs_shard_alloc(int64_t bytes, void** dev_ptr_out);
int32_t gs_shard_free(void* dev_ptr);
int32_t gs_ipc_export(const void* dev_ptr, uint8_t* handle64_out_host);
int32_t gs_ipc_import(const uint8_t* handle64_host, void** dev_ptr_out);
int32_t gs_ipc_close(void* dev_ptr);

int32_t gs_gather_rows_f32(const void* feats, int32_t dtype, int64_t n_rows, int32_t F, int64_t pitch,
                           const int32_t* ids, int64_t row0, int64_t n, float* out, int64_t out_pitch,
                           void* stream);
int32_t gs_cast_rows_bf16(const float* x, int64_t n, int32_t F, int64_t ldx, void* out_bf16, int64_t out_pitch,
                          void* stream);

int32_t gs_rmat_degrees(int32_t scale, int64_t n_nodes, double edge_factor, double a, double b, double c, double d,
                        uint64_t seed, uint64_t mul, uint64_t mul_inv, uint64_t add, int32_t* deg_out, void* stream);
int32_t gs_rmat_fill(int32_t scale, int64_t n_nodes, double a, double b, double c, double d, uint64_t seed, uint64_t mul,
                     uint64_t mul_inv, uint64_t add, const int64_t* indptr, int32_t* indices, const int64_t* long_rows,
                     int64_t n_long, int64_t long_threshold, void* stream);

int32_t gs_segment_max(const float* x, int64_t n, int32_t k, int32_t C, int64_t ldx,
                       float* out, int64_t ldo, void* stream);

typedef struct {
  const float* A; int64_t lda; int32_t K;
  const float* B; int64_t ldb; int32_t N;
} gs_gemm_part;

int64_t gs_sage_gemm_workspace_bytes(int64_t M, const gs_gemm_part* parts_host, int32_t n_parts,
                                     int32_t math);
int32_t gs_sage_gemm(int64_t M, const gs_gemm_part* parts_host, int32_t n_parts, int32_t combine,
                     const float* bias, int32_t act, int32_t math, float* out, int64_t ldo,
                     void* workspace, void* stream);

int32_t gs_sage_gemm_pack(const gs_gemm_part* parts_host, int32_t n_parts, int32_t math, void* workspace,
                          void* stream);
int32_t gs_sage_gemm_prepacked(int64_t M, const gs_gemm_part* parts_host, int32_t n_parts, int32_t combine,
                               const float* bias, int32_t act, int32_t math, float* out, int64_t ldo,
                               const void* workspace, void* stream);

int64_t gs_gather_mean_img_bytes(int64_t rows, int32_t F, int32_t want_self);
int32_t gs_gather_mean_img(const void* src, int64_t n_src_rows, const gs_sharded_table* table_host, int32_t ids_are_locators,
                           const void* staging, int32_t F, int64_t pitch, const gs_segment* segments_host,
                           int32_t n_segments, int32_t include_self, int32_t want_self, void* images, void* stream);
int32_t gs_sage_gemm_img(int64_t M, const gs_gemm_part* parts_host, int32_t n_parts, int32_t combine, const float* bias,
                         int32_t act, float* out, int64_t ldo, const void* workspace, const void* a_images,
                         int32_t a_part0, void* stream);

int32_t gs_sage_layer_small(const float* src, int64_t n_src_rows, int32_t F, int64_t pitch,
                            const gs_segment* segment_host, int32_t include_self,
                            const gs_gemm_part* parts_host, int32_t n_parts, int32_t combine,
                            const float* bias, int32_t act, int32_t l2_normalize,
                            float* out, int64_t ldo, uint64_t* counter_dev, uint64_t counter_inc,
                            void* stream);

int64_t gs_maxpool_mlp_workspace_bytes(int32_t K, int32_t hidden);
int32_t gs_maxpool_mlp_pack(const float* Wm, int64_t ldw, int32_t K, int32_t hidden, void* workspace,
                            void* stream);
int32_t gs_maxpool_mlp_fused(const void* table_bf16, int64_t n_rows, int32_t K, int64_t pitch,
                             const int32_t* row_ids, int64_t row0, int64_t n_groups, int32_t k,
                             const void* packed_weights, const float* bias, int32_t hidden,
                             float* out, int64_t ldo, void* stream);
int32_t gs_meanpool_mlp_fused(const void* table_bf16, int64_t n_rows, int32_t K, int64_t pitch,
                              const int32_t* row_ids, int64_t row0, int64_t n_groups, int32_t k,
                              const void* packed_weights, const float* bias, int32_t hidden,
                              float* out, int64_t ldo, void* stream);

int32_t gs_row_used(const void* x, int32_t dtype, int64_t n_rows, int32_t F, int64_t pitch, uint8_t* used, void* stream);
int32_t gs_lstm_seq(const float* P, int64_t ldp, const float* Wh, int32_t H, const uint8_t* used, const int32_t* row_ids,
                    int64_t row0, int64_t n, int32_t k, float* out, int64_t ldo, float* keep_h, float* keep_c,
                    int32_t* lengths, void* stream);

int32_t gs_pipeline_step(const void* ids_host, void* ids_dev, int64_t ids_bytes, void* const* graph_execs_host,
                         int32_t n_graphs, const void* out_dev, void* out_host, int64_t out_bytes,
                         void* h2d_stream, void* compute_stream, void* copy_stream, void* ev_ids, void* ev_done,
                         void* ev_drained);

int32_t gs_bump_counter(uint64_t* counter_dev, uint64_t inc, void* stream);

int32_t gs_l2_normalize_rows(float* x, int64_t n, int32_t C, int64_t ldx, void* stream);

#ifdef __cplusplus
}
#endif
#endif
```

Before: 6.572 million.

## Switch TF32x3 GEMM tiles to 64-byte swizzle with deeper smem rings

Moves the TF32x3 (mode 0) GEMM operand images from 128-byte-swizzled 32-column K blocks to 64-byte-swizzled 16-column K blocks. The gather kernel's image writer, the B packer, the producer loops and the descriptors are updated to match. Halving the per-stage footprint lets the image GEMM double its A/B ring depth to 6 stages, which aims for more load/MMA overlap. The gather kernel is also templated on whether it writes images, so the non-image path drops that branch. A footprint query API is added as well. The cost is twice as many K iterations and barrier handoffs per tile.

```diff
diff --git a/graphsage_b200/_lib.py b/graphsage_b200/_lib.py
--- a/graphsage_b200/_lib.py
+++ b/graphsage_b200/_lib.py
@@ -37,6 +37,7 @@
     "gs_version": (c_i32, []),
     "gs_last_error_string": (ctypes.c_char_p, []),
     "gs_set_tuning": (c_i32, [ctypes.c_char_p, c_i32]),
+    "gs_step_kernel_footprint": (c_i32, [c_i32, c_vp]),
     "gs_sample_padded": (c_i32, [c_vp, c_i64, c_i32, c_vp, c_i64, c_i32, c_vp, c_u64, c_u64, c_vp, c_vp, c_vp]),
     "gs_sample_padded_khop": (c_i32, [c_vp, c_i64, c_i32, c_vp, c_i64, ctypes.POINTER(c_i32), c_i32, c_u64, c_u64, c_vp,
                                       ctypes.POINTER(c_vp), c_vp]),
diff --git a/graphsage_b200/csrc/api.cu b/graphsage_b200/csrc/api.cu
--- a/graphsage_b200/csrc/api.cu
+++ b/graphsage_b200/csrc/api.cu
@@ -66,6 +66,25 @@
 
 int32_t gs_version(void) { return GS_ABI_VERSION; }
 
+int32_t gs_step_kernel_footprint(int32_t which, int32_t* out) {
+  GS_REQUIRE(out != nullptr, "gs_step_kernel_footprint: out is NULL");
+  int32_t dyn = -1;
+  const void* fn = which == 0 ? gs::step_kernel_gather(&dyn) : which == 1 ? gs::step_kernel_sampler(&dyn)
+                 : which == 2 ? gs::step_kernel_gemm(&dyn) : which == 3 ? gs::step_kernel_small_layer(&dyn) : nullptr;
+  GS_REQUIRE(fn != nullptr, "gs_step_kernel_footprint: which=%d (0..3)", which);
+  cudaFuncAttributes a;
+  GS_CUDA(cudaFuncGetAttributes(&a, fn));
+  out[0] = a.numRegs;
+  out[1] = (int32_t)a.sharedSizeBytes;
+  out[2] = a.maxThreadsPerBlock;
+  out[3] = dyn;
+  int dev = 0, reserved = 0;
+  GS_CUDA(cudaGetDevice(&dev));
+  GS_CUDA(cudaDeviceGetAttribute(&reserved, cudaDevAttrReservedSharedMemoryPerBlock, dev));
+  out[4] = reserved;
+  return GS_OK;
+}
+
 const char* gs_last_error_string(void) { return gs::g_err; }
 
 int32_t gs_set_tuning(const char* key, int32_t value) {
diff --git a/graphsage_b200/csrc/common.cuh b/graphsage_b200/csrc/common.cuh
--- a/graphsage_b200/csrc/common.cuh
+++ b/graphsage_b200/csrc/common.cuh
@@ -12,6 +12,10 @@
 int32_t cuda_fail(cudaError_t e, const char* what);
 int32_t tuning(const char* key, int32_t dflt);
 int32_t ensure_dyn_smem(const void* kernel, int bytes);
+const void* step_kernel_gather(int32_t* dyn_smem);
+const void* step_kernel_sampler(int32_t* dyn_smem);
+const void* step_kernel_gemm(int32_t* dyn_smem);
+const void* step_kernel_small_layer(int32_t* dyn_smem);
 
 #define GS_REQUIRE(cond, ...)            \
   do {                                   \
diff --git a/graphsage_b200/csrc/gather.cu b/graphsage_b200/csrc/gather.cu
--- a/graphsage_b200/csrc/gather.cu
+++ b/graphsage_b200/csrc/gather.cu
@@ -218,21 +218,21 @@
 };
 
 __device__ __forceinline__ void gather_img_store(const GatherImg& im, int part, int64_t orow, int c, float4 v) {
-  const int kb = c >> 3, chunk = c & 7;
+  const int kb = c >> 2, chunk = c & 3;
   const int64_t mt = orow >> 7;
   const int r = (int)(orow & 127);
-  unsigned char* dst = im.base + ((((int64_t)part * im.n_mtiles + mt) * im.kblocks + kb) * 2) * 16384 +
-                       (uint32_t)(r * 128 + ((chunk ^ (r & 7)) << 4));
+  unsigned char* dst = im.base + ((((int64_t)part * im.n_mtiles + mt) * im.kblocks + kb) * 2) * 8192 +
+                       (uint32_t)(r * 64 + ((chunk ^ ((r >> 1) & 3)) << 4));
   uint4 hi, lo;
   hi.x = __float_as_uint(v.x) & 0xFFFFE000u; hi.y = __float_as_uint(v.y) & 0xFFFFE000u;
   hi.z = __float_as_uint(v.z) & 0xFFFFE000u; hi.w = __float_as_uint(v.w) & 0xFFFFE000u;
   lo.x = __float_as_uint(v.x - __uint_as_float(hi.x)) & 0xFFFFE000u; lo.y = __float_as_uint(v.y - __uint_as_float(hi.y)) & 0xFFFFE000u;
   lo.z = __float_as_uint(v.z - __uint_as_float(hi.z)) & 0xFFFFE000u; lo.w = __float_as_uint(v.w - __uint_as_float(hi.w)) & 0xFFFFE000u;
   *reinterpret_cast<uint4*>(dst) = hi;
-  *reinterpret_cast<uint4*>(dst + 16384) = lo;
-}
-
-template <class Rows>
+  *reinterpret_cast<uint4*>(dst + 8192) = lo;
+}
+
+template <class Rows, bool kImg>
 __global__ void __launch_bounds__(192) gather_mean_tma2_kernel(const __grid_constant__ Rows rows_of, int F,
                                                                const __grid_constant__ SegTable tab,
                                                                int include_self, float* __restrict__ out_self,
@@ -309,7 +309,7 @@
     }
     if (last) {
       const int64_t orow = sg.out_row0 + i;
-      const int ncol_img = img.base ? img.kblocks * 8 : 0;
+      const int ncol_img = kImg ? img.kblocks * 4 : 0;
 #pragma unroll
       for (int q = 0; q < 2; ++q) {
         const int c = threadIdx.x + q * blockDim.x;
@@ -328,7 +328,7 @@
             if (out_mean) reinterpret_cast<float4*>(out_mean + orow * out_pitch)[c] = a;
             if (out_self) reinterpret_cast<float4*>(out_self + orow * out_pitch)[c] = sv;
           }
-          if (c < ncol_img) {
+          if (kImg && c < ncol_img) {
             if (img.want_self) gather_img_store(img, 0, orow, c, sv);
             gather_img_store(img, img.want_self ? 1 : 0, orow, c, a);
           }
@@ -768,7 +768,8 @@
 template <class Rows>
 static int32_t launch_gather_tma2(const Rows& rows_of, int F, const SegTable& tab, int include_self, float* out_self, float* out_mean,
                                   int64_t out_pitch, const GatherImg& img, cudaStream_t st) {
-  const int32_t rc_attr = ensure_dyn_smem((const void*)gather_mean_tma2_kernel<Rows>, 200 * 1024);
+  const void* fn = img.base ? (const void*)gather_mean_tma2_kernel<Rows, true> : (const void*)gather_mean_tma2_kernel<Rows, false>;
+  const int32_t rc_attr = ensure_dyn_smem(fn, 200 * 1024);
   if (rc_attr != GS_OK) return rc_attr;
   const int ncol4 = (int)(out_pitch / 4);
   const int row_bytes = ((F + 3) / 4) * 16;
@@ -783,9 +784,18 @@
   int64_t blocks = tab.total_rows;
   int64_t cap = (int64_t)sm_count() * per_sm;
   if (blocks > cap) blocks = cap;
-  gather_mean_tma2_kernel<Rows><<<(unsigned)blocks, threads, smem2, st>>>(rows_of, F, tab, include_self, out_self, out_mean,
-                                                                          out_pitch, row_bytes, img);
+  if (img.base)
+    gather_mean_tma2_kernel<Rows, true><<<(unsigned)blocks, threads, smem2, st>>>(rows_of, F, tab, include_self, out_self,
+                                                                                out_mean, out_pitch, row_bytes, img);
+  else
+    gather_mean_tma2_kernel<Rows, false><<<(unsigned)blocks, threads, smem2, st>>>(rows_of, F, tab, include_self, out_self,
+                                                                                 out_mean, out_pitch, row_bytes, img);
   return launch_check("gather_mean_tma2_kernel");
+}
+
+const void* step_kernel_gather(int32_t* dyn_smem) {
+  *dyn_smem = -1;
+  return (const void*)gather_mean_tma2_kernel<DenseRows, false>;
 }
 }
 
@@ -1046,8 +1056,8 @@
 
 int64_t gs_gather_mean_img_bytes(int64_t rows, int32_t F, int32_t want_self) {
   if (rows < 0 || F < 1) return -1;
-  const int64_t n_mtiles = (rows + 127) / 128, kblocks = (F + 31) / 32;
-  return (want_self ? 2 : 1) * n_mtiles * kblocks * 2 * 16384;
+  const int64_t n_mtiles = (rows + 127) / 128, kblocks = (F + 15) / 16;
+  return (want_self ? 2 : 1) * n_mtiles * kblocks * 2 * 8192;
 }
 
 int32_t gs_gather_mean_img(const void* src, int64_t n_src_rows, const gs_sharded_table* table_host, int32_t ids_are_locators,
@@ -1077,7 +1087,7 @@
   }
   gs::GatherImg img;
   img.base = (unsigned char*)images;
-  img.kblocks = (F + 31) / 32;
+  img.kblocks = (F + 15) / 16;
   img.n_mtiles = (int32_t)((rows + 127) / 128);
   img.want_self = want_self ? 1 : 0;
   if (src) {
diff --git a/graphsage_b200/csrc/gemm_tc.cu b/graphsage_b200/csrc/gemm_tc.cu
--- a/graphsage_b200/csrc/gemm_tc.cu
+++ b/graphsage_b200/csrc/gemm_tc.cu
@@ -33,11 +33,33 @@
   int32_t a_part0;
 };
 
+template <int MODE, bool ASYNC = false>
+struct TcCfg {
+  static constexpr bool SW64 = MODE == 0;
+  static constexpr int ROW_BYTES = SW64 ? 64 : 128;
+  static constexpr int BK = ROW_BYTES / (MODE == 2 ? 2 : 4);
+  static constexpr int CPR = ROW_BYTES / 16;
+  static constexpr int UK = MODE == 2 ? 16 : 8;
+  static constexpr int NIMG = MODE == 0 ? 2 : 1;
+  static constexpr int TILE_BYTES = TC_BM * ROW_BYTES;
+  static constexpr int IMG_BYTES = NIMG * TILE_BYTES;
+  static constexpr int SA = MODE == 0 ? 2 : 3;
+  static constexpr int NB = ASYNC ? (MODE == 0 ? 2 : 4) : (MODE == 0 ? 4 : 8);
+  static constexpr int RAW_BYTES = TC_BM * BK * 4;
+  static constexpr int RAW_SLOTS = ASYNC ? (MODE == 2 ? 3 : 4) : 0;
+  static constexpr int B_OFF = SA * IMG_BYTES;
+  static constexpr int RAW_OFF = B_OFF + NB * IMG_BYTES;
+  static constexpr int SMEM_BYTES = RAW_OFF + RAW_SLOTS * RAW_BYTES + 1024;
+
+  static __host__ __device__ __forceinline__ uint32_t chunk_off(int r, int c) { return SW64 ? sw64_off(r, c) : sw128_off(r, c); }
+  static __device__ __forceinline__ uint64_t desc(uint32_t saddr) { return SW64 ? make_smem_desc64(saddr) : make_smem_desc(saddr); }
+};
+
 template <int MODE>
 __global__ void __launch_bounds__(256) pack_b_kernel(TcParams prm, unsigned char* __restrict__ ws) {
-  constexpr int BK = MODE == 2 ? 64 : 32;
+  using C = TcCfg<MODE>;
+  constexpr int BK = C::BK;
   constexpr int EPC = MODE == 2 ? 8 : 4;
-  constexpr int NIMG = MODE == 0 ? 2 : 1;
   int unit = blockIdx.x;
   int pi = 0;
   if (prm.n_parts == 2 && unit >= prm.p[0].ntiles * prm.p[0].kblocks) {
@@ -46,15 +68,15 @@
   }
   const TcPart& P = prm.p[pi];
   const int nt = unit / P.kblocks, kb = unit % P.kblocks;
-  unsigned char* img = ws + P.img_off + ((int64_t)(nt * P.kblocks + kb) * NIMG) * TC_TILE_BYTES;
-  for (int q = threadIdx.x; q < 128 * 8; q += blockDim.x) {
+  unsigned char* img = ws + P.img_off + (int64_t)(nt * P.kblocks + kb) * C::IMG_BYTES;
+  for (int q = threadIdx.x; q < 128 * C::CPR; q += blockDim.x) {
     const int c = q >> 7, n = q & 127;
     const int gn = nt * TC_BN + n;
     const int k0 = kb * BK + c * EPC;
     float w[EPC];
 #pragma unroll
     for (int e = 0; e < EPC; ++e) w[e] = (gn < P.N && k0 + e < P.K) ? P.B[(int64_t)(k0 + e) * P.ldb + gn] : 0.f;
-    const uint32_t off = sw128_off(n, c);
+    const uint32_t off = C::chunk_off(n, c);
     if constexpr (MODE == 2) {
       __nv_bfloat162 h[4];
 #pragma unroll
@@ -68,7 +90,7 @@
         uint4 lo;
         lo.x = tf32_mask(w[0] - __uint_as_float(hi.x)); lo.y = tf32_mask(w[1] - __uint_as_float(hi.y));
         lo.z = tf32_mask(w[2] - __uint_as_float(hi.z)); lo.w = tf32_mask(w[3] - __uint_as_float(hi.w));
-        *reinterpret_cast<uint4*>(img + TC_TILE_BYTES + off) = lo;
+        *reinterpret_cast<uint4*>(img + C::TILE_BYTES + off) = lo;
       }
     }
   }
@@ -83,20 +105,6 @@
   }
 }
 
-template <int MODE, bool ASYNC = false>
-struct TcCfg {
-  static constexpr int BK = MODE == 2 ? 64 : 32;
-  static constexpr int UK = MODE == 2 ? 16 : 8;
-  static constexpr int NIMG = MODE == 0 ? 2 : 1;
-  static constexpr int IMG_BYTES = NIMG * TC_TILE_BYTES;
-  static constexpr int SA = MODE == 0 ? 2 : 3;
-  static constexpr int NB = ASYNC ? (MODE == 0 ? 2 : 4) : (MODE == 0 ? 4 : 8);
-  static constexpr int RAW_BYTES = TC_BM * BK * 4;
-  static constexpr int RAW_SLOTS = ASYNC ? (MODE == 2 ? 3 : 4) : 0;
-  static constexpr int B_OFF = SA * IMG_BYTES;
-  static constexpr int RAW_OFF = B_OFF + NB * IMG_BYTES;
-  static constexpr int SMEM_BYTES = RAW_OFF + RAW_SLOTS * RAW_BYTES + 1024;
-};
 
 
 template <int MODE>
@@ -122,7 +130,7 @@
 
 template <int MODE>
 __device__ __forceinline__ void store_a_chunk(unsigned char* a_img, int row, int c, const float (&v)[8]) {
-  const uint32_t off = sw128_off(row, c);
+  const uint32_t off = TcCfg<MODE>::chunk_off(row, c);
   if constexpr (MODE == 2) {
     __nv_bfloat162 h[4];
 #pragma unroll
@@ -136,7 +144,7 @@
       uint4 lo;
       lo.x = tf32_mask(v[0] - __uint_as_float(hi.x)); lo.y = tf32_mask(v[1] - __uint_as_float(hi.y));
       lo.z = tf32_mask(v[2] - __uint_as_float(hi.z)); lo.w = tf32_mask(v[3] - __uint_as_float(hi.w));
-      *reinterpret_cast<uint4*>(a_img + TC_TILE_BYTES + off) = lo;
+      *reinterpret_cast<uint4*>(a_img + TcCfg<MODE>::TILE_BYTES + off) = lo;
     }
   }
 }
@@ -188,7 +196,7 @@
   if (warp < TC_PRODUCER_WARPS) {
     if constexpr (ASYNC) {
       constexpr int EPC = MODE == 2 ? 8 : 4;
-      constexpr int CPT = 4;
+      constexpr int CPT = TC_BM * C::CPR / 256;
       constexpr int RAW_PER_CHUNK = EPC / 4;
       unsigned char* raw = smem + C::RAW_OFF;
       const int tid = threadIdx.x;
@@ -205,7 +213,7 @@
 #pragma unroll
           for (int i = 0; i < CPT; ++i) {
             const int q = tid + 256 * i;
-            const int row = q >> 3, c = q & 7;
+            const int row = q / C::CPR, c = q % C::CPR;
             const int64_t grow = m0 + row;
 #pragma unroll
             for (int h = 0; h < RAW_PER_CHUNK; ++h) {
@@ -242,42 +250,43 @@
 #pragma unroll
         for (int i = 0; i < CPT; ++i) {
           const int q = tid + 256 * i;
-          store_a_chunk<MODE>(a_img, q >> 3, q & 7, v[i]);
+          store_a_chunk<MODE>(a_img, q / C::CPR, q % C::CPR, v[i]);
         }
         fence_proxy_async();
         __syncwarp();
         if (lane == 0) mbar_arrive(&full_a[s]);
       }
     } else {
+    constexpr int NCH = C::CPR, RSTEP = 128 / C::CPR;
     const int group = warp >> 2;
     const int tg = threadIdx.x & 127;
-    const int c = tg & 7, r0 = tg >> 3;
-    float cur[8][8];
+    const int c = tg % NCH, r0 = tg / NCH;
+    float cur[NCH][8];
     auto locate = [&](int it, int& pi, int& kb) {
       pi = part_lo; kb = it;
       while (kb >= prm.p[pi].kblocks) { kb -= prm.p[pi].kblocks; ++pi; }
     };
-    auto fetch = [&](int it, float (&dst)[8][8]) {
+    auto fetch = [&](int it, float (&dst)[NCH][8]) {
       int pi, kb;
       locate(it, pi, kb);
       const TcPart& P = prm.p[pi];
       const bool vec = ((P.lda & 3) == 0) && ((reinterpret_cast<uintptr_t>(P.A) & 15u) == 0);
       const int gcol = kb * C::BK + c * (MODE == 2 ? 8 : 4);
 #pragma unroll
-      for (int i = 0; i < 8; ++i) load_a_chunk<MODE>(P, prm.M, m0 + r0 + 16 * i, gcol, vec, dst[i]);
+      for (int i = 0; i < NCH; ++i) load_a_chunk<MODE>(P, prm.M, m0 + r0 + RSTEP * i, gcol, vec, dst[i]);
     };
     int it = group;
     if (it < total_it) fetch(it, cur);
     for (; it < total_it; it += 2) {
       const int s = it % C::SA;
       const uint32_t ph = (uint32_t)(it / C::SA) & 1u;
-      float nxt[8][8];
+      float nxt[NCH][8];
       const bool more = it + 2 < total_it;
       if (more) fetch(it + 2, nxt);
       mbar_wait(&empty_a[s], ph ^ 1u);
       unsigned char* a_img = smem + (size_t)s * C::IMG_BYTES;
 #pragma unroll
-      for (int i = 0; i < 8; ++i) store_a_chunk<MODE>(a_img, r0 + 16 * i, c, cur[i]);
+      for (int i = 0; i < NCH; ++i) store_a_chunk<MODE>(a_img, r0 + RSTEP * i, c, cur[i]);
       fence_proxy_async();
       __syncwarp();
       if (lane == 0) mbar_arrive(&full_a[s]);
@@ -285,7 +294,7 @@
       if (threadIdx.x == 0 && it + 2 >= total_it) dbg_stamp(3);
       if (more) {
 #pragma unroll
-        for (int i = 0; i < 8; ++i)
+        for (int i = 0; i < NCH; ++i)
 #pragma unroll
           for (int e = 0; e < 8; ++e) cur[i][e] = nxt[i][e];
       }
@@ -343,7 +352,7 @@
       if (lane == 0 && it == total_it - 1) dbg_stamp(12);
       const uint32_t a_base = smem_u32(smem + (size_t)s * C::IMG_BYTES);
       const uint32_t b_base = smem_u32(smem + C::B_OFF + (size_t)sb * C::IMG_BYTES);
-      const uint64_t a_hi = make_smem_desc(a_base), b_hi = make_smem_desc(b_base);
+      const uint64_t a_hi = C::desc(a_base), b_hi = C::desc(b_base);
       if (prm.issue_elect) {
 #pragma unroll
         for (int k = 0; k < C::BK / C::UK; ++k) {
@@ -351,7 +360,7 @@
           const uint32_t acc = (it > 0 || k > 0) ? 1u : 0u;
           umma_ss_elect<MODE == 2>(tmem_acc, a_hi + koff, b_hi + koff, idesc, acc);
           if constexpr (MODE == 0) {
-            const uint64_t a_lo = make_smem_desc(a_base + TC_TILE_BYTES), b_lo = make_smem_desc(b_base + TC_TILE_BYTES);
+            const uint64_t a_lo = C::desc(a_base + C::TILE_BYTES), b_lo = C::desc(b_base + C::TILE_BYTES);
             umma_ss_elect<false>(tmem_acc, a_hi + koff, b_lo + koff, idesc, 1u);
             umma_ss_elect<false>(tmem_acc, a_lo + koff, b_hi + koff, idesc, 1u);
           }
@@ -367,7 +376,7 @@
           const uint32_t acc = (it > 0 || k > 0) ? 1u : 0u;
           umma_ss<MODE == 2>(tmem_acc, a_hi + koff, b_hi + koff, idesc, acc);
           if constexpr (MODE == 0) {
-            const uint64_t a_lo = make_smem_desc(a_base + TC_TILE_BYTES), b_lo = make_smem_desc(b_base + TC_TILE_BYTES);
+            const uint64_t a_lo = C::desc(a_base + C::TILE_BYTES), b_lo = C::desc(b_base + C::TILE_BYTES);
             umma_ss<false>(tmem_acc, a_hi + koff, b_lo + koff, idesc, 1u);
             umma_ss<false>(tmem_acc, a_lo + koff, b_hi + koff, idesc, 1u);
           }
@@ -384,7 +393,7 @@
       int it = 0;
       for (int pi = part_lo; pi < part_hi; ++pi) {
         const TcPart& P = prm.p[pi];
-        const unsigned char* base = ws + P.img_off + (int64_t)ntile * P.kblocks * C::NIMG * TC_TILE_BYTES;
+        const unsigned char* base = ws + P.img_off + (int64_t)ntile * P.kblocks * C::IMG_BYTES;
         for (int kb = 0; kb < P.kblocks; ++kb, ++it) {
           const int sb = it % C::NB;
           const uint32_t ph = (uint32_t)(it / C::NB) & 1u;
@@ -406,8 +415,8 @@
 }
 
 constexpr int TCI_THREADS = 256;
-constexpr int TCI_IMG = 2 * TC_TILE_BYTES;
-constexpr int TCI_SA = 3, TCI_NB = 3;
+constexpr int TCI_IMG = TcCfg<0>::IMG_BYTES;
+constexpr int TCI_SA = 6, TCI_NB = 6;
 constexpr int TCI_SMEM = (TCI_SA + TCI_NB) * TCI_IMG + 1024;
 
 __global__ void __launch_bounds__(TCI_THREADS, 1) sage_gemm_tc_img_kernel(const __grid_constant__ TcParams prm,
@@ -483,10 +492,11 @@
       mbar_wait_uniform(&full_b[sb], (uint32_t)(it / TCI_NB) & 1u);
       tc_fence_after();
       const uint32_t a_base = smem_u32(a_ring + (size_t)sa * TCI_IMG), b_base = smem_u32(b_ring + (size_t)sb * TCI_IMG);
-      const uint64_t a_hi = make_smem_desc(a_base), b_hi = make_smem_desc(b_base);
-      const uint64_t a_lo = make_smem_desc(a_base + TC_TILE_BYTES), b_lo = make_smem_desc(b_base + TC_TILE_BYTES);
-#pragma unroll
-      for (int k = 0; k < 4; ++k) {
+      using C = TcCfg<0>;
+      const uint64_t a_hi = C::desc(a_base), b_hi = C::desc(b_base);
+      const uint64_t a_lo = C::desc(a_base + C::TILE_BYTES), b_lo = C::desc(b_base + C::TILE_BYTES);
+#pragma unroll
+      for (int k = 0; k < C::BK / C::UK; ++k) {
         const uint64_t koff = (uint64_t)((k * 32) >> 4);
         umma_ss_elect<false>(tmem_acc, a_hi + koff, b_hi + koff, idesc, (it > 0 || k > 0) ? 1u : 0u);
         umma_ss_elect<false>(tmem_acc, a_hi + koff, b_lo + koff, idesc, 1u);
@@ -542,8 +552,8 @@
 static int mode_of(int32_t math) { return math == GS_MATH_TF32X3 ? 0 : math == GS_MATH_TF32 ? 1 : 2; }
 
 static void fill_parts(TcParams& prm, int64_t M, const gs_gemm_part* parts, int32_t n_parts, int mode) {
-  const int BK = mode == 2 ? 64 : 32;
-  const int nimg = mode == 0 ? 2 : 1;
+  const int BK = mode == 0 ? TcCfg<0>::BK : mode == 1 ? TcCfg<1>::BK : TcCfg<2>::BK;
+  const int img_bytes = mode == 0 ? TcCfg<0>::IMG_BYTES : mode == 1 ? TcCfg<1>::IMG_BYTES : TcCfg<2>::IMG_BYTES;
   memset(&prm, 0, sizeof(prm));
   prm.n_parts = n_parts;
   prm.M = M;
@@ -555,7 +565,7 @@
     P.kblocks = (P.K + BK - 1) / BK;
     P.ntiles = (P.N + TC_BN - 1) / TC_BN;
     P.img_off = off;
-    off += (int64_t)P.kblocks * P.ntiles * nimg * TC_TILE_BYTES;
+    off += (int64_t)P.kblocks * P.ntiles * img_bytes;
   }
   prm.tiles_n0 = prm.p[0].ntiles;
   prm.issue_elect = tuning("mma_issue", 1) != 0;
@@ -565,8 +575,9 @@
   TcParams prm;
   fill_parts(prm, M, parts, n_parts, mode_of(math));
   const TcPart& L = prm.p[n_parts - 1];
-  const int nimg = mode_of(math) == 0 ? 2 : 1;
-  return L.img_off + (int64_t)L.kblocks * L.ntiles * nimg * TC_TILE_BYTES;
+  const int mode = mode_of(math);
+  const int img_bytes = mode == 0 ? TcCfg<0>::IMG_BYTES : mode == 1 ? TcCfg<1>::IMG_BYTES : TcCfg<2>::IMG_BYTES;
+  return L.img_off + (int64_t)L.kblocks * L.ntiles * img_bytes;
 }
 
 template <int MODE>
@@ -597,6 +608,11 @@
     aligned = aligned && (prm.p[i].lda % 4 == 0) && ((reinterpret_cast<uintptr_t>(prm.p[i].A) & 15u) == 0);
   if (aligned && tuning("gemm_async", 0)) return launch_tc_impl<MODE, true>(prm, ws, st);
   return launch_tc_impl<MODE, false>(prm, ws, st);
+}
+
+const void* step_kernel_gemm(int32_t* dyn_smem) {
+  *dyn_smem = TcCfg<0>::SMEM_BYTES;
+  return (const void*)sage_gemm_tc_kernel<0, false>;
 }
 
 int32_t tc_debug_read(unsigned long long* out_host, int n) {
diff --git a/graphsage_b200/csrc/layer_small.cu b/graphsage_b200/csrc/layer_small.cu
--- a/graphsage_b200/csrc/layer_small.cu
+++ b/graphsage_b200/csrc/layer_small.cu
@@ -242,6 +242,11 @@
       if (row0 + r < sg.n) prm.out[(sg.out_row0 + row0 + r) * prm.ldo + col] = part[r * ncolp + col] * inv[r];
   }
   if (prm.counter_dev != nullptr && blockIdx.x == 0 && threadIdx.x == 0) *prm.counter_dev += prm.counter_inc;
+}
+
+const void* step_kernel_small_layer(int32_t* dyn_smem) {
+  *dyn_smem = -1;
+  return (const void*)sage_layer_small_kernel;
 }
 
 }
diff --git a/graphsage_b200/csrc/maxpool_tc.cu b/graphsage_b200/csrc/maxpool_tc.cu
--- a/graphsage_b200/csrc/maxpool_tc.cu
+++ b/graphsage_b200/csrc/maxpool_tc.cu
@@ -34,18 +34,6 @@
   const uint32_t* wrows;
   int32_t dbg;
 };
-
-__host__ __device__ __forceinline__ uint32_t sw64_off(int r, int c) { return (uint32_t)(r * 64 + ((c ^ ((r >> 1) & 3)) << 4)); }
-
-__device__ __forceinline__ uint64_t make_smem_desc64(uint32_t saddr) {
-  uint64_t d = 0;
-  d |= (uint64_t)((saddr & 0x3FFFFu) >> 4);
-  d |= (uint64_t)1 << 16;
-  d |= (uint64_t)(512 >> 4) << 32;
-  d |= (uint64_t)1 << 46;
-  d |= (uint64_t)4 << 61;
-  return d;
-}
 
 __global__ void __launch_bounds__(256) maxpool_pack_kernel(const float* __restrict__ W, int64_t ldw, int K, int hidden,
                                                            int kblocks, unsigned char* __restrict__ img) {
diff --git a/graphsage_b200/csrc/sampler.cu b/graphsage_b200/csrc/sampler.cu
--- a/graphsage_b200/csrc/sampler.cu
+++ b/graphsage_b200/csrc/sampler.cu
@@ -206,6 +206,11 @@
   }
 }
 
+const void* step_kernel_sampler(int32_t* dyn_smem) {
+  *dyn_smem = 0;
+  return (const void*)sample_padded_khop_kernel;
+}
+
 }
 
 extern "C" {
diff --git a/graphsage_b200/csrc/tc_common.cuh b/graphsage_b200/csrc/tc_common.cuh
--- a/graphsage_b200/csrc/tc_common.cuh
+++ b/graphsage_b200/csrc/tc_common.cuh
@@ -142,6 +142,16 @@
   return d;
 }
 
+__device__ __forceinline__ uint64_t make_smem_desc64(uint32_t saddr) {
+  uint64_t d = 0;
+  d |= (uint64_t)((saddr & 0x3FFFFu) >> 4);
+  d |= (uint64_t)1 << 16;
+  d |= (uint64_t)(512 >> 4) << 32;
+  d |= (uint64_t)1 << 46;
+  d |= (uint64_t)4 << 61;
+  return d;
+}
+
 __host__ __device__ constexpr uint32_t make_idesc(uint32_t fmt, uint32_t M, uint32_t N) {
   return (1u << 4) | (fmt << 7) | (fmt << 10) | ((N >> 3) << 17) | ((M >> 4) << 24);
 }
@@ -151,6 +161,8 @@
 __host__ __device__ __forceinline__ uint32_t sw128_off(int r, int c) {
   return (uint32_t)(r * 128 + ((c ^ (r & 7)) << 4));
 }
+
+__host__ __device__ __forceinline__ uint32_t sw64_off(int r, int c) { return (uint32_t)(r * 64 + ((c ^ ((r >> 1) & 3)) << 4)); }
 
 
 __device__ __forceinline__ void cp_async16(void* smem_dst, const void* gsrc, int src_bytes) {
diff --git a/include/graphsage_b200.h b/include/graphsage_b200.h
--- a/include/graphsage_b200.h
+++ b/include/graphsage_b200.h
@@ -32,6 +32,7 @@
 int32_t gs_version(void);
 const char* gs_last_error_string(void);
 int32_t gs_set_tuning(const char* key, int32_t value);
+int32_t gs_step_kernel_footprint(int32_t which, int32_t* out);
 
 int32_t gs_sample_padded(const int32_t* adj, int64_t n_rows, int32_t max_deg,
                          const int32_t* ids, int64_t n, int32_t k,
```

After: 6.831 million (median of 6 runs). 1.04x the previous value.
